# mj129/Tramba

Measured on AMD Instinct MI355X. Metric: images/sec fwd Tramba-V 384x384, higher is better.
Workload: dtype bf16; 1 GPU; Tramba-V (VMamba-B encoder) 384x384 bf16 inference, batch 4 per GPU, random-init weights (seed 1026), randn images; global_batch=4, launch=hipGraph replay, decoder guide branches on a side stream

## Files before the change

### include/tramba_hip.h

```cpp
#ifndef TRAMBA_HIP_H
#define TRAMBA_HIP_H

#include <stddef.h>
#include <stdint.h>

#ifdef __cplusplus
extern "C" {
#endif

typedef enum { TRAMBA_F32 = 0, TRAMBA_F16 = 1, TRAMBA_BF16 = 2 } tramba_dtype;

typedef enum {
    TRAMBA_SCAN_RASTER = 0,
    TRAMBA_SCAN_LINE = 1,
    TRAMBA_SCAN_HELIX = 2,
    TRAMBA_SCAN_WINDOW = 3,
    TRAMBA_SCAN_DILATION = 4
} tramba_scan_family;

typedef enum { TRAMBA_ACT_NONE = 0, TRAMBA_ACT_SILU = 1, TRAMBA_ACT_GELU = 2,
               TRAMBA_ACT_SIGMOID_GATE = 3 ,
               TRAMBA_ACT_GELU_GRAD_MUL = 4
             } tramba_act;

// ... 82 lines not shown
#define TRAMBA_SCAN_BWD_A_LOG 1
#define TRAMBA_SCAN_BWD_BC_PARTIALS 2
int tramba_ss2d_bwd_prep_cl(const float *xdbl, const int32_t *table, const float *bpart, const float *cpart, void *ranks,
                            float *gseq, int batch, int l, int k, int r, int ctiles, int dtype, void *stream);
int tramba_ss2d_bwd_assemble_cl(const float *gseq, const int32_t *inv_ptr, const int32_t *inv_idx, void *out, int batch,
                                int l, int k, int r, int dtype, void *stream);
size_t tramba_ss2d_scan_n_bwd_workspace(int batch, int l, int d, int k, int n, int dtype);
int tramba_ss2d_scan_n_bwd_plan(int batch, int l, int d, int k, int n, int *tiles_per_segment, int *nseg);
int tramba_ss2d_scan_n_bwd_cl(const void *x, const float *xdbl, const int32_t *table, const float *dt_w,
                              const float *dt_bias, const float *A, const float *Ds, const void *gym, void *gu,
                              void *graw, float *bpart, float *cpart, float *gpar, void *workspace,
                              size_t workspace_bytes, int batch, int l, int d, int k, int r, int n, int dtype,
                              int gym_dtype, void *stream);
int tramba_ss2d_bwd_prep_n_cl(const float *xdbl, const int32_t *table, const float *bpart, const float *cpart, void *ranks,
                              float *gseq, int batch, int l, int k, int r, int n, int ctiles, int dtype, void *stream);
int tramba_ss2d_bwd_assemble_n_cl(const float *gseq, const int32_t *inv_ptr, const int32_t *inv_idx, void *out, int batch,
                                  int l, int k, int r, int n, int dtype, void *stream);
int tramba_ss2d_merge_norm_cl(const void *ys, const int32_t *inv_ptr, const int32_t *inv_idx,
                              const float *ln_w, const float *ln_b, void *y, int batch, int l, int d,
                              int k, float eps, int act, int ys_dtype, int dtype, void *stream);
int tramba_ss2d_merge_grad_cl(const void *ys, const int32_t *inv_ptr, const int32_t *inv_idx, const float *ln_w,
                              const float *ln_b, void *y, const void *addend, const void *zpre, int batch, int l, int d,
                              int k, float eps, int act, int ys_dtype, int dtype, void *stream);

int tramba_layernorm_cl(const void *x, const float *w, const float *b, void *y, int64_t rows, int c,
                        float eps, int act, int dtype, void *stream);
int64_t tramba_layernorm_bwd_parts(int64_t rows, int c, int dtype);
int tramba_layernorm_bwd_cl(const void *x, const void *dy, const float *w, void *dx, float *part, int64_t rows,
                            int c, float eps, int dtype, void *stream);
int tramba_layernorm_bwd_res_cl(const void *x, const void *dy, const float *w, void *dx, float *part, const void *gres,
                                const float *mask, int64_t rows_per_sample, void *dxm, int64_t rows, int c, float eps,
                                int dtype, void *stream);
int tramba_layernorm_bwd_any_cl(const void *x, const void *dy, const float *w, void *dx, float *part, const void *gres,
                                const float *mask, int64_t rows_per_sample, void *dxm, int64_t rows, int c, float eps, int P,
                                int H, int W, int dtype, void *stream);
int tramba_shuffle_norm_bwd_cl(const void *x, const void *dy, const float *w, void *dx, float *part, int batch, int h,
                               int wd, int c, int p, float eps, int dtype, void *stream);
int tramba_add_layernorm_cl(const void *x, const void *y, const float *mask, int64_t rows_per_sample, const float *w,
                            const float *b, void *xsum, void *n, void *n_act, int64_t rows, int c, float eps, int act,
                            int dtype, void *stream);
int tramba_shuffle_norm_cl(const void *x, const float *w, const float *b, void *y, int batch, int h,
                           int wd, int c, int p, float eps, int dtype, void *stream);
int tramba_shuffle_norm_head_cl(const void *x, const float *w, const float *b, const float *head_w, float head_b,
                                float *y, int batch, int h, int wd, int c, int p, float eps, int dtype,
                                void *stream);
int64_t tramba_shuffle_norm_head_bwd_parts(int batch, int h, int wd, int c, int p, int dtype);
int tramba_shuffle_norm_head_bwd_cl(const void *x, const float *g, const float *ln_w, const float *head_w, void *dx,
                                    float *part, int batch, int h, int wd, int c, int p, float eps, int dtype, void *stream);
int tramba_rowdot_cl(const void *x, const float *w, float bias, float *y, int64_t rows, int c, int dtype,
                     void *stream);
int64_t tramba_rowdot_bwd_parts(int64_t rows, int c, int dtype);
int tramba_rowdot_bwd_cl(const void *x, const float *gy, const float *w, void *gx, float *part, int64_t rows, int c,
                         int dtype, void *stream);
int tramba_dw_pack(const float *w, const float *bias, const float *w3, const float *b3, const float *w5,
                   const float *b5, float *wt, float *bt, int c, int ks, void *stream);
int tramba_dw_pack_multi(const float *const *w, const float *const *bias, const float *const *w3, const float *const *b3,
                         const float *const *w5, const float *const *b5, float *const *wt, float *const *bt, const int *c,
                         const int *ks, int count, void *stream);
int tramba_im2col3x3_cl(const void *x, void *cols, int batch, int h, int wd, int c, int stride, int pad, int ckp,
                        int dtype, void *stream);
int tramba_col2im3x3_cl(const void *gcols, void *gx, int batch, int h, int wd, int c, int stride, int pad, int ckp,
                        int dtype, void *stream);
int tramba_upsample_bilinear_bwd(const float *gout, float *gin, int planes, int h, int w, int hout, int wout,
                                 void *stream);
int tramba_dwconv_cl(const void *x, const float *wt, const float *bt, void *y, int batch, int h,
                     int wd, int c, int ks, int act, int dtype, void *stream);
int tramba_dwconv_dual_cl(const void *x, const float *wt, const float *bt, void *y_pre, void *y, int batch, int h, int wd,
                          int c, int ks, int act, int flip_taps, int dtype, void *stream);
int tramba_dw_unpack_grad(const float *gwt, float *g7, float *g5, float *g3, float *gb, int nb, int c, int ks,
                          void *stream);
int tramba_dw_unpack_grad_multi(const float *const *gwt, float *const *g7, float *const *g5, float *const *g3,
                                float *const *gb, const int *nb, const int *c, const int *ks, int count, void *stream);
int64_t tramba_dwconv_wgrad_parts(int batch, int h, int wd, int c, int ks);
int tramba_dwconv_wgrad_cl(const void *x, const void *gy, float *part, int batch, int h, int wd, int c, int ks,
                           int dtype, void *stream);
int tramba_dct_split_cl(const void *x, const float *wx, const float *wy, float *tmp, void *high,
                        void *low, int batch, int n, int c, int dtype, void *stream);
int tramba_linear_cl(const void *x, const void *w, const float *bias, const void *residual, void *y,
                     int64_t m, int n, int k, int act, int dtype, int out_dtype, void *stream);
int tramba_linear_ln_cl(const void *x, const void *w_folded, const float *colsum, const float *bias, const void *residual,
                        void *y, int64_t m, int n, int k, float eps, int act, int dtype, int out_dtype, void *stream);
int tramba_linear2_cl(const void *x1, const void *x2, int k1, const void *w, const float *bias, const void *residual,
                      void *y, int64_t m, int n, int k, int act, int dtype, int out_dtype, void *stream);

int tramba_linear_dual_cl(const void *x, const void *w, const float *bias, void *y_pre, void *y_act, int64_t m, int n,
                          int k, int act, int dtype, void *stream);
size_t tramba_wgrad_workspace(int64_t m, int n, int k, int groups, int nbatch);
int tramba_wgrad_cl(const void *gy, const void *x, float *out, void *workspace, size_t workspace_bytes, int64_t m, int n,
                    int k, int groups, int nbatch, int64_t gy_bs, int64_t gy_gs, int gy_ld, int64_t x_bs, int64_t x_gs,
                    int x_ld, int want_bias, int dtype, void *stream);
int tramba_wgrad_parts_cl(const void *gy, const void *x, float *out, void *workspace, size_t workspace_bytes, int64_t m,
                          int n, int k, int groups, int nbatch, int64_t gy_bs, int64_t gy_gs, int gy_ld, int64_t x_bs,
                          int64_t x_gs, int x_ld, int want_bias, int dtype, void *stream, int *nslab);
int tramba_rows_gemm_cl(const void *x, const void *w, float *y, int nz, int64_t m, int n, int k, int groups, int ldy,
                        int dtype, void *stream);
int tramba_shadow_cast_multi(const void *table, int ntensors, int64_t total_tiles, int dtype, void *stream);
int tramba_slab_sum(const float *part, float *out, int64_t n, int nslab, void *stream);
int tramba_multi_sum_strided(const float *const *parts, float *const *outs, const int64_t *n, const int64_t *stride,
                             const int *nslab, int count, void *stream);
int tramba_multi_sum(const float *const *parts, float *const *outs, const int64_t *n, const int *nslab, int count,
                     void *stream);

int tramba_expand_norm_head_cl(const void *x, const void *w, const float *ln_w, const float *ln_b,
                               const float *head_w, float head_b, float *y, int batch, int h, int wd, int cin, int p,
                               float eps, int dtype, void *stream);

int tramba_conv3x3s2_cl(const void *x, const void *w, const float *bias, void *y, int batch, int hin,
                        int win, int cin, int cout, int dtype, void *stream);
int tramba_stem_conv_ln_gelu(const void *img, const float *w, const float *bias, const float *ln_w,
                             const float *ln_b, void *y, int batch, int h, int wd, float eps,
                             int img_dtype, int dtype, void *stream);

#define TRAMBA_EVAL_NINT 520
#define TRAMBA_EVAL_NDBL 48
int tramba_saliency_stats(const float *pred, const unsigned char *gt, long long *ints, double *dbl, int batch, int h,
                          int w, void *stream);
#define TRAMBA_WFM_MAX_DIM 4096
int tramba_feature_transform(const unsigned char *gt, int *idx, int *dist2, int batch, int h, int w, void *stream);
size_t tramba_weighted_f_workspace(int batch, int h, int w);
int tramba_weighted_f_sums(const float *pred, const unsigned char *gt, const int *idx, const int *dist2, const double *gauss,
                           double *sums, void *workspace, size_t workspace_bytes, int batch, int h, int w, void *stream);

#define TRAMBA_FRAME_MAX_DIM 16384
#define TRAMBA_FRAME_MAX_OUT 2048
size_t tramba_resize_table_words(int in_h, int in_w, int out_h, int out_w);
int tramba_resize_table(int in_h, int in_w, int out_h, int out_w, const double *mean, const double *std, int *table,
                        size_t words);
int tramba_frames_to_input(const unsigned char *frames, const int *table, float *out, int batch, int h, int w, int out_h,
                           int out_w, int bgr, void *stream);
int tramba_logits_to_u8(const void *logits, unsigned char *out, int batch, int in_h, int in_w, int h, int w, int dtype,
                        void *stream);
#define TRAMBA_FRAMES_DESC_WORDS 16
#define TRAMBA_RAGGED_IN 1
#define TRAMBA_RAGGED_OUT 2
int tramba_frames_ragged_check(const int64_t *desc_host, int batch, int size, size_t packed_bytes, size_t out_capacity,
                               int parts);
int tramba_frames_to_input_ragged(const unsigned char *packed, const int64_t *desc_host, size_t packed_bytes, float *out,
                                  int batch, int size, int bgr, void *stream);
int tramba_logits_to_u8_ragged(const void *logits, const unsigned char *packed, const int64_t *desc_host, unsigned char *out,
                               size_t out_capacity, int batch, int size, int dtype, void *stream);

#define TRAMBA_AUG_DESC_WORDS 32
#define TRAMBA_AUG_CONTRAST 0
#define TRAMBA_AUG_BRIGHTNESS 1
#define TRAMBA_AUG_SHARPNESS 2
size_t tramba_augment_source_table_words(int h, int w, int size);
int tramba_augment_source_table(int h, int w, int size, int *table, size_t words);
size_t tramba_augment_size_table_words(int size);
int tramba_augment_size_table(int size, const double *mean, const double *std, int *table, size_t words);
int tramba_augment_scale_taps(int size, int r);
int tramba_augment_rotation(int size, int degrees, int *coef);
size_t tramba_augment_workspace(int batch, int size);
int tramba_augment_batch(const unsigned char *packed, const int64_t *desc_host, size_t packed_bytes, const int *size_table,
                         float *image, float *label, void *workspace, size_t workspace_bytes, int batch, int size,
                         void *stream);

int tramba_sod_loss_sums(const float *logits, const float *label, float *part, int planes, int h, int w, int hout, int wout,
                         int nblk, void *stream);
int tramba_sod_loss_finish(const float *const *parts, const int *nblk, const float *weights, float *const *coefs, int nout,
                           int planes, int64_t npix, float *loss, void *stream);
size_t tramba_sod_loss_grad_workspace(int planes, int h, int w, int hout, int wout);
int tramba_sod_loss_grad(const float *logits, const float *label, const float *coef, const float *gscale, float *glogits,
                         void *workspace, size_t workspace_bytes, int planes, int h, int w, int hout, int wout, void *stream);
int tramba_loss_weight_map(const float *label, float *weit, int planes, int h, int w, int k, void *stream);
int tramba_sod_wloss_sums(const float *logits, const float *label, const float *wmap, float *part, int planes, int h, int w,
                          int hout, int wout, int nblk, float eps, int weight_is_raw, void *stream);
// ... 80 lines not shown
```

### tramba_amd/csrc/linear.hip

```cpp
#include <stdlib.h>
#include <string.h>

#include <type_traits>

#include "common.h"

namespace tramba {

typedef __attribute__((ext_vector_type(8))) short frag8_t;
typedef __attribute__((ext_vector_type(8))) _Float16 frag8h_t;
typedef __attribute__((ext_vector_type(16))) float acc16_t;

template <typename T> struct Mfma;
template <> struct Mfma<__hip_bfloat16> {
    static constexpr int KSTEP = 16;
    using frag = frag8_t;
    static __device__ __forceinline__ acc16_t run(frag a, frag b, acc16_t c)
    {
        typedef __attribute__((ext_vector_type(8))) __bf16 bf8;
        return __builtin_amdgcn_mfma_f32_32x32x16_bf16(__builtin_bit_cast(bf8, a), __builtin_bit_cast(bf8, b), c, 0, 0, 0);
    }
};
template <> struct Mfma<__half> {
    static constexpr int KSTEP = 16;
// ... 31 lines not shown
    if (col >= N) return;
    const float bv = bias ? bias[col] : 0.f;
#pragma unroll
    for (int r = 0; r < 16; ++r) {
        const long row = m0 + (r & 3) + 8 * (r >> 2) + 4 * (lane >> 5);
        if (row < M) {
            float v = apply_act(acc[r] + bv, act);
            if (res) v = combine_residual(v, Cvt<T>::to_f(res[row * N + col]), act);
            y[row * N + col] = Cvt<TO>::from_f(v);
        }
    }
}

template <typename T, typename TO>
__global__ __launch_bounds__(256) void linear16_kernel(const T *__restrict__ x, const T *__restrict__ w,
                                                      const float *__restrict__ bias, const T *__restrict__ res,
                                                      TO *__restrict__ y, long M, int N, int K, int act, int vec)
{
    const int lane = threadIdx.x & 63, wave = threadIdx.x >> 6;
    const long m0 = (long)blockIdx.y * 128 + (wave >> 1) * 64;
    const int n0 = blockIdx.x * 128 + (wave & 1) * 64;
    if (m0 >= M || n0 >= N) return;
    acc16_t acc[2][2];
#pragma unroll
    for (int i = 0; i < 2; ++i)
#pragma unroll
        for (int j = 0; j < 2; ++j)
#pragma unroll
            for (int r = 0; r < 16; ++r) acc[i][j][r] = 0.f;
    const int r32 = lane & 31, kh = (lane >> 5) * 8;
    for (int k0 = 0; k0 < K; k0 += 16) {
        frag8_t a[2], b[2];
#pragma unroll
        for (int i = 0; i < 2; ++i) a[i] = load_frag16<T>(x, m0 + i * 32 + r32, M, k0 + kh, K, vec);
#pragma unroll
        for (int j = 0; j < 2; ++j) b[j] = load_frag16<T>(w, n0 + j * 32 + r32, N, k0 + kh, K, vec);
#pragma unroll
        for (int i = 0; i < 2; ++i)
#pragma unroll
            for (int j = 0; j < 2; ++j) acc[i][j] = Mfma<T>::run(a[i], b[j], acc[i][j]);
    }
#pragma unroll
    for (int i = 0; i < 2; ++i)
#pragma unroll
        for (int j = 0; j < 2; ++j)
            store_tile<T, TO>(acc[i][j], y, bias, res, m0 + i * 32, n0 + j * 32, M, N, act, lane);
}


constexpr int kBK = 64;

__device__ __forceinline__ int swz_chunk(int row, int chunk) { return chunk ^ ((row >> 1) & 7); }

struct ConvGeom {
    int hin, win, cin, hout, wout;
};

template <int BM, int BN>
struct WaveLayout {
    static constexpr int WM = BM / 2, WN = BN / 2, TM = WM / 32, TN = WN / 32;
    static_assert(WM % 32 == 0 && WN % 32 == 0, "wave tiles are whole 32x32 MFMA tiles");
};

template <int BM, int BN, typename ACC>
__device__ __forceinline__ void acc_to_lds(ACC &acc, float *ep)
{
    using WL = WaveLayout<BM, BN>;
    constexpr int TM = WL::TM, TN = WL::TN, WM = WL::WM, WN = WL::WN, LDE = BN + 4;
    const int lane = threadIdx.x & 63, wave = threadIdx.x >> 6;
    if (wave >= 4) return;
    const int wm = wave / 2, wn = wave % 2;
    const int r32 = lane & 31, hi = lane >> 5;
#pragma unroll
    for (int i = 0; i < TM; ++i)
#pragma unroll
        for (int j = 0; j < TN; ++j)
#pragma unroll
            for (int g = 0; g < 4; ++g) {
                float *dst = ep + (wm * WM + i * 32 + r32) * LDE + wn * WN + j * 32 + 8 * g + 4 * hi;
                *reinterpret_cast<float4 *>(dst) = make_float4(acc[i][j][4 * g], acc[i][j][4 * g + 1], acc[i][j][4 * g + 2], acc[i][j][4 * g + 3]);
            }
}

template <typename T, typename TO, int BM, int BN, int NT = 256, typename ACC>
__device__ __forceinline__ void tile_epilogue(ACC &acc, unsigned char *lds,
                                              const float *__restrict__ bias, const T *__restrict__ res,
                                              TO *__restrict__ y, long M, int N, int act, long m0, int n0,
                                              const float *__restrict__ colsum = nullptr,
                                              const float2 *__restrict__ rowstat = nullptr,
                                              TO *__restrict__ y_pre = nullptr)
{
    const int tid = threadIdx.x;
    constexpr int LDE = BN + 4;
    float *ep = reinterpret_cast<float *>(lds);
    acc_to_lds<BM, BN>(acc, ep);
    __syncthreads();
    constexpr int CPL = 8;
    constexpr int LPRW = BN / CPL;
    constexpr int RPI = NT / LPRW;
    const int cl = (tid % LPRW) * CPL, rl = tid / LPRW;
    const int gcol = n0 + cl;
#pragma unroll
    for (int it = 0; it < (BM + RPI - 1) / RPI; ++it) {
        const int row = it * RPI + rl;
        const long grow = m0 + row;
        if (grow >= M || gcol >= N) continue;
        float o[CPL];
        {
            const float4 v0 = *reinterpret_cast<const float4 *>(ep + row * LDE + cl);
            const float4 v1 = *reinterpret_cast<const float4 *>(ep + row * LDE + cl + 4);
            o[0] = v0.x; o[1] = v0.y; o[2] = v0.z; o[3] = v0.w; o[4] = v1.x; o[5] = v1.y; o[6] = v1.z; o[7] = v1.w;
        }
        if (gcol + CPL <= N && (N & 7) == 0) {
            if (colsum) {
                const float2 st = rowstat[row];
                float cs[CPL];
                load_pack<float, CPL>(colsum + gcol, cs);
#pragma unroll
                for (int q = 0; q < CPL; ++q) o[q] = st.y * fmaf(-st.x, cs[q], o[q]);
            }
            if (bias) {
                float bv[CPL];
                load_pack<float, CPL>(bias + gcol, bv);
#pragma unroll
                for (int q = 0; q < CPL; ++q) o[q] += bv[q];
            }
            if (y_pre) store_pack<TO, CPL>(y_pre + grow * N + gcol, o);
#pragma unroll
            for (int q = 0; q < CPL; ++q) o[q] = apply_act(o[q], act);
            if (res) {
                float rv[CPL];
                load_pack<T, CPL>(res + grow * N + gcol, rv);
#pragma unroll
                for (int q = 0; q < CPL; ++q) o[q] = combine_residual(o[q], rv[q], act);
            }
            store_pack<TO, CPL>(y + grow * N + gcol, o);
        } else {
#pragma unroll
            for (int q = 0; q < CPL; ++q) {
                if (gcol + q < N) {
                    if (colsum) o[q] = rowstat[row].y * fmaf(-rowstat[row].x, colsum[gcol + q], o[q]);
                    const float pre = o[q] + (bias ? bias[gcol + q] : 0.f);
                    if (y_pre) y_pre[grow * N + gcol + q] = Cvt<TO>::from_f(pre);
                    float t = apply_act(pre, act);
                    if (res) {
                        const float rv = Cvt<T>::to_f(res[grow * N + gcol + q]);
                        t = combine_residual(t, rv, act);
                    }
                    y[grow * N + gcol + q] = Cvt<TO>::from_f(t);
                }
            }
        }
    }
}

template <typename T, typename TO, int BM, int BN, int PF, bool CONV>
__global__ __launch_bounds__(256) void linear_tiled_kernel(const T *__restrict__ x, const T *__restrict__ w,
                                                          const float *__restrict__ bias,
                                                          const T *__restrict__ res, TO *__restrict__ y, long M,
                                                          int N, int K, int act, ConvGeom cg)
{
    constexpr int TM = BM / 64, TN = BN / 64;
    constexpr int A_CHUNKS = BM * (kBK / 8), B_CHUNKS = BN * (kBK / 8);
    constexpr int A_PER_T = A_CHUNKS / 256, B_PER_T = B_CHUNKS / 256;
    constexpr int TILE_BYTES = (BM + BN) * kBK * 2;
    constexpr int EPI_BYTES = BM * (BN + 4) * 4;
    constexpr int LDS_BYTES = 2 * TILE_BYTES > EPI_BYTES ? 2 * TILE_BYTES : EPI_BYTES;
    __shared__ __attribute__((aligned(16))) unsigned char lds[LDS_BYTES];

    const int tid = threadIdx.x, lane = tid & 63, wave = tid >> 6;
    const int wm = wave >> 1, wn = wave & 1;
    long m0;
    int n0;
    {
        const unsigned nblk = gridDim.x * gridDim.y, lin = blockIdx.y * gridDim.x + blockIdx.x;
        const unsigned q = nblk >> 3, r = nblk & 7, xcd = lin & 7, slot = lin >> 3;
        const unsigned t = xcd * q + (xcd < r ? xcd : r) + slot;
        m0 = (long)(t / gridDim.x) * BM;
        n0 = (int)(t % gridDim.x) * BN;
    }
    const int nk = (K + kBK - 1) / kBK;

    acc16_t acc[TM][TN];
#pragma unroll
    for (int i = 0; i < TM; ++i)
#pragma unroll
        for (int j = 0; j < TN; ++j)
#pragma unroll
            for (int r = 0; r < 16; ++r) acc[i][j][r] = 0.f;

    struct Stage { frag8_t a[A_PER_T], b[B_PER_T]; };
    const int kmax = ((K - 1) / 8) * 8;
    int cb[A_PER_T], chi[A_PER_T], cwi[A_PER_T];
    if (CONV) {
#pragma unroll
        for (int i = 0; i < A_PER_T; ++i) {
            const int row = (tid + i * 256) >> 3;
            const long gr = m0 + row < M ? m0 + row : M - 1;
            const int wo = (int)(gr % cg.wout);
            const long t = gr / cg.wout;
            chi[i] = 2 * (int)(t % cg.hout) - 1;
            cwi[i] = 2 * wo - 1;
            cb[i] = (int)(t / cg.hout);
        }
    }
    auto conv_src = [&](int kt, int i, bool &inside) -> long {
        const int k0 = kt * kBK;
        const int tap = k0 / cg.cin, ci = k0 - tap * cg.cin;
        const int hy = chi[i] + tap / 3, wx = cwi[i] + tap % 3;
        inside = hy >= 0 && hy < cg.hin && wx >= 0 && wx < cg.win;
        const int hc = hy < 0 ? 0 : (hy >= cg.hin ? cg.hin - 1 : hy), wc = wx < 0 ? 0 : (wx >= cg.win ? cg.win - 1 : wx);
        return (((long)cb[i] * cg.hin + hc) * cg.win + wc) * cg.cin + ci;
    };
    auto gload = [&](int kt, Stage &st) {
        const int ktc = kt < nk ? kt : nk - 1;
        const int k0 = ktc * kBK;
#pragma unroll
        for (int i = 0; i < A_PER_T; ++i) {
            const int q = tid + i * 256, row = q >> 3, c = q & 7;
            if (CONV) {
                bool inside;
                st.a[i] = *reinterpret_cast<const frag8_t *>(x + conv_src(ktc, i, inside) + c * 8);
            } else {
                const long gr = m0 + row < M ? m0 + row : M - 1;
                const int kc = k0 + c * 8 <= kmax ? k0 + c * 8 : kmax;
                st.a[i] = *reinterpret_cast<const frag8_t *>(x + gr * K + kc);
            }
        }
#pragma unroll
        for (int i = 0; i < B_PER_T; ++i) {
            const int q = tid + i * 256, row = q >> 3, c = q & 7;
            const int gn = n0 + row < N ? n0 + row : N - 1;
            const int kc = k0 + c * 8 <= kmax ? k0 + c * 8 : kmax;
            st.b[i] = *reinterpret_cast<const frag8_t *>(w + (long)gn * K + kc);
        }
    };
    auto lstore = [&](int kt, const Stage &st) {
        const int buf = kt & 1, k0 = kt * kBK;
        unsigned char *As = lds + buf * TILE_BYTES, *Bs = As + BM * kBK * 2;
        const frag8_t zero = {0, 0, 0, 0, 0, 0, 0, 0};
#pragma unroll
        for (int i = 0; i < A_PER_T; ++i) {
            const int q = tid + i * 256, row = q >> 3, c = q & 7;
            bool ok = m0 + row < M && k0 + c * 8 < K;
            if (CONV) {
                bool inside;
                conv_src(kt, i, inside);
                ok = ok && inside;
            }
            *reinterpret_cast<frag8_t *>(As + row * 128 + swz_chunk(row, c) * 16) = ok ? st.a[i] : zero;
        }
#pragma unroll
        for (int i = 0; i < B_PER_T; ++i) {
            const int q = tid + i * 256, row = q >> 3, c = q & 7;
            const bool ok = n0 + row < N && k0 + c * 8 < K;
            *reinterpret_cast<frag8_t *>(Bs + row * 128 + swz_chunk(row, c) * 16) = ok ? st.b[i] : zero;
        }
    };

    constexpr int NS = PF + 1;
    Stage pipe[NS];
    gload(0, pipe[0]);
    lstore(0, pipe[0]);
#pragma unroll
    for (int i = 1; i < NS; ++i) gload(i, pipe[i]);
    __syncthreads();
    const int r32 = lane & 31, hi = lane >> 5;
    auto kstep = [&](int kt, Stage &load_into, const Stage &store_from) {
        gload(kt + NS, load_into);
        const unsigned char *As = lds + (kt & 1) * TILE_BYTES, *Bs = As + BM * kBK * 2;
#pragma unroll
        for (int kk = 0; kk < kBK / 16; ++kk) {
            frag8_t a[TM], b[TN];
            const int c = kk * 2 + hi;
#pragma unroll
            for (int i = 0; i < TM; ++i) {
                const int row = wm * (BM / 2) + i * 32 + r32;
                a[i] = *reinterpret_cast<const frag8_t *>(As + row * 128 + swz_chunk(row, c) * 16);
            }
#pragma unroll
            for (int j = 0; j < TN; ++j) {
                const int row = wn * (BN / 2) + j * 32 + r32;
                b[j] = *reinterpret_cast<const frag8_t *>(Bs + row * 128 + swz_chunk(row, c) * 16);
            }
#pragma unroll
            for (int i = 0; i < TM; ++i)
#pragma unroll
                for (int j = 0; j < TN; ++j) acc[i][j] = Mfma<T>::run(b[j], a[i], acc[i][j]);
        }
        lstore(kt + 1, store_from);
        __syncthreads();
    };
    const int nkp = (nk + NS - 1) / NS * NS;
    constexpr int UNR = 4 * NS;
    int kt0 = 0;
    for (; kt0 + UNR <= nkp; kt0 += UNR) {
#pragma unroll
        for (int ui = 0; ui < UNR; ++ui) kstep(kt0 + ui, pipe[ui % NS], pipe[(ui + 1) % NS]);
    }
    for (; kt0 < nkp; kt0 += NS) {
#pragma unroll
        for (int ui = 0; ui < NS; ++ui) kstep(kt0 + ui, pipe[ui % NS], pipe[(ui + 1) % NS]);
    }

    tile_epilogue<T, TO, BM, BN>(acc, lds, bias, res, y, M, N, act, m0, n0);
}

struct LnIn {
    const float *colsum;
    float eps;
};

struct LnHead {
    const float *ln_w, *ln_b, *head_w;
    float head_b, eps;
    int H, W, P;
    float *out;
};

template <typename T, int BM>
__device__ __forceinline__ void tile_epilogue_ln_head(acc16_t (&acc)[BM / 64][2], unsigned char *lds, const LnHead hd,
                                                      long M, long m0, int n0)
{
    constexpr int BN = 128, TM = BM / 64, TN = 2, WM = BM / 2, WN = BN / 2;
    const int tid = threadIdx.x, lane = tid & 63, wave = tid >> 6;
    const int wm = wave >> 1, wn = wave & 1;
    const int r32 = lane & 31, hi = lane >> 5;
    constexpr int LDE = BN + 4;
    float *ep = reinterpret_cast<float *>(lds);
    acc_to_lds<BM, BN>(acc, ep);
    __syncthreads();
    const int sub = tid & 3;
    float gam[32], bet[32], hw[32];
#pragma unroll
    for (int j = 0; j < 8; ++j) {
        const int c = 16 * j + 4 * sub;
        const float4 a = *reinterpret_cast<const float4 *>(hd.ln_w + c);
        const float4 b = *reinterpret_cast<const float4 *>(hd.ln_b + c);
        const float4 h = *reinterpret_cast<const float4 *>(hd.head_w + c);
        gam[4 * j] = a.x; gam[4 * j + 1] = a.y; gam[4 * j + 2] = a.z; gam[4 * j + 3] = a.w;
        bet[4 * j] = b.x; bet[4 * j + 1] = b.y; bet[4 * j + 2] = b.z; bet[4 * j + 3] = b.w;
        hw[4 * j] = h.x; hw[4 * j + 1] = h.y; hw[4 * j + 2] = h.z; hw[4 * j + 3] = h.w;
    }
    const int g = n0 / BN;
#pragma unroll
    for (int it = 0; it < BM / 64; ++it) {
        const int row = it * 64 + (tid >> 2);
        const long grow = m0 + row;
        float v[32];
#pragma unroll
        for (int j = 0; j < 8; ++j) {
            const float4 t = *reinterpret_cast<const float4 *>(ep + row * LDE + 16 * j + 4 * sub);
            v[4 * j] = t.x; v[4 * j + 1] = t.y; v[4 * j + 2] = t.z; v[4 * j + 3] = t.w;
        }
        float s1 = 0.f;
#pragma unroll
        for (int q = 0; q < 32; ++q) s1 += v[q];
        s1 += __shfl_xor(s1, 1, 64);
        s1 += __shfl_xor(s1, 2, 64);
        const float mean = s1 * (1.f / 128.f);
        float s2 = 0.f;
#pragma unroll
        for (int q = 0; q < 32; ++q) {
            const float d = v[q] - mean;
            s2 = fmaf(d, d, s2);
        }
        s2 += __shfl_xor(s2, 1, 64);
        s2 += __shfl_xor(s2, 2, 64);
        const float rstd = rsqrtf(s2 * (1.f / 128.f) + hd.eps);
        float dot = 0.f;
#pragma unroll
        for (int q = 0; q < 32; ++q) {
            const float yn = (v[q] - mean) * rstd * gam[q] + bet[q];
            dot = fmaf(yn, hw[q], dot);
        }
        dot += __shfl_xor(dot, 1, 64);
        dot += __shfl_xor(dot, 2, 64);
        if (sub == 0 && grow < M) {
            const unsigned pix = (unsigned)grow;
            const unsigned wi = pix % (unsigned)hd.W, bh = pix / (unsigned)hd.W;
            const unsigned hh = bh % (unsigned)hd.H, bb = bh / (unsigned)hd.H;
            const long o = ((long)bb * (hd.H * hd.P) + (hh * hd.P + g / hd.P)) * (long)(hd.W * hd.P) + (wi * hd.P + g % hd.P);
            hd.out[o] = dot + hd.head_b;
        }
    }
}

typedef unsigned v4u_t __attribute__((ext_vector_type(4)));

template <typename T> __device__ __forceinline__ float dot2_ones(unsigned v, float acc);
template <typename T> __device__ __forceinline__ float dot2_self(unsigned v, float acc);
typedef __bf16 bf2_t __attribute__((ext_vector_type(2)));
typedef _Float16 hf2_t __attribute__((ext_vector_type(2)));
template <> __device__ __forceinline__ float dot2_ones<__hip_bfloat16>(unsigned v, float acc)
{
    return __builtin_amdgcn_fdot2_f32_bf16(__builtin_bit_cast(bf2_t, v), __builtin_bit_cast(bf2_t, 0x3f803f80u), acc, false);
}
template <> __device__ __forceinline__ float dot2_self<__hip_bfloat16>(unsigned v, float acc)
{
    return __builtin_amdgcn_fdot2_f32_bf16(__builtin_bit_cast(bf2_t, v), __builtin_bit_cast(bf2_t, v), acc, false);
}
template <> __device__ __forceinline__ float dot2_ones<__half>(unsigned v, float acc)
{
    return __builtin_amdgcn_fdot2(__builtin_bit_cast(hf2_t, v), __builtin_bit_cast(hf2_t, 0x3c003c00u), acc, false);
}
template <> __device__ __forceinline__ float dot2_self<__half>(unsigned v, float acc)
{
    return __builtin_amdgcn_fdot2(__builtin_bit_cast(hf2_t, v), __builtin_bit_cast(hf2_t, v), acc, false);
}
template <> __device__ __forceinline__ float dot2_ones<float>(unsigned, float acc) { return acc; }
template <> __device__ __forceinline__ float dot2_self<float>(unsigned, float acc) { return acc; }

template <typename T, typename TO, int BM, int BN, int PF, bool LNHEAD = false>
__global__ __launch_bounds__(256) void linear_lean_kernel(const T *__restrict__ x, const T *__restrict__ w,
                                                         const float *__restrict__ bias,
                                                         const T *__restrict__ res, TO *__restrict__ y, long M,
                                                         int N, int K, int act, const T *__restrict__ x2, int K1,
                                                         LnHead hd = LnHead{})
{
    using WL = WaveLayout<BM, BN>;
    constexpr int TM = WL::TM, TN = WL::TN;
    constexpr int A_PER_T = BM * (kBK / 8) / 256, B_PER_T = BN * (kBK / 8) / 256;
    constexpr int TILE_BYTES = (BM + BN) * kBK * 2;
    constexpr int EPI_BYTES = BM * (BN + 4) * 4;
    static_assert((BM * (kBK / 8)) % 256 == 0 && (BN * (kBK / 8)) % 256 == 0, "whole 16-byte chunks per thread");
    constexpr int LDS_BYTES = 2 * TILE_BYTES > EPI_BYTES ? 2 * TILE_BYTES : EPI_BYTES;
    constexpr int NS = PF + 1;
    static_assert(NS % 2 == 0, "the LDS buffer parity must be a compile-time constant");
    __shared__ __attribute__((aligned(16))) unsigned char lds[LDS_BYTES];

    const int tid = threadIdx.x, lane = tid & 63, wave = tid >> 6;
    const int wm = wave < 4 ? wave / 2 : 0, wn = wave % 2;
    const int r32 = lane & 31, hi = lane >> 5;
    long m0;
    int n0;
    {
        const unsigned nblk = gridDim.x * gridDim.y, lin = blockIdx.y * gridDim.x + blockIdx.x;
        const unsigned q = nblk >> 3, r = nblk & 7, xcd = lin & 7, slot = lin >> 3;
        const unsigned t = xcd * q + (xcd < r ? xcd : r) + slot;
        m0 = (long)(t / gridDim.x) * BM;
        n0 = (int)(t % gridDim.x) * BN;
    }
    const int nk = K / kBK;
    const unsigned rowb = (unsigned)K * 2u;
    const long mrows = M - m0 < BM ? M - m0 : BM;
    const int nrows = N - n0 < BN ? N - n0 : BN;
    const int ka = x2 ? K1 : K;
    const unsigned rowa = (unsigned)ka * 2u, rowa2 = (unsigned)(K - ka) * 2u;
    const int nk1 = ka / kBK;
    const __amdgpu_buffer_rsrc_t ra = make_rsrc(x + m0 * ka, (unsigned)mrows * rowa);
    const __amdgpu_buffer_rsrc_t ra2 = make_rsrc(x2 ? x2 + m0 * (K - ka) : x, x2 ? (unsigned)mrows * rowa2 : 0u);
    const __amdgpu_buffer_rsrc_t rb = make_rsrc(w + (long)n0 * K, (unsigned)nrows * rowb);

    unsigned ag[A_PER_T], ag2[A_PER_T], bg[B_PER_T], al[A_PER_T], bl[B_PER_T];
#pragma unroll
    for (int i = 0; i < A_PER_T; ++i) {
        const int q = tid + i * 256, row = q >> 3, c = q & 7;
        ag[i] = (unsigned)row * rowa + (unsigned)c * 16u;
        ag2[i] = (unsigned)row * rowa2 + (unsigned)c * 16u;
        al[i] = (unsigned)(row * 128 + swz_chunk(row, c) * 16);
    }
#pragma unroll
    for (int i = 0; i < B_PER_T; ++i) {
        const int q = tid + i * 256, row = q >> 3, c = q & 7;
        bg[i] = (unsigned)row * rowb + (unsigned)c * 16u;
        bl[i] = (unsigned)(BM * kBK * 2 + row * 128 + swz_chunk(row, c) * 16);
    }
    unsigned ard[TM], brd[TN];
#pragma unroll
    for (int i = 0; i < TM; ++i) {
        const int row = wm * WL::WM + i * 32 + r32;
        ard[i] = (unsigned)(row * 128 + swz_chunk(row, hi) * 16);
    }
#pragma unroll
    for (int j = 0; j < TN; ++j) {
        const int row = wn * WL::WN + j * 32 + r32;
        brd[j] = (unsigned)(BM * kBK * 2 + row * 128 + swz_chunk(row, hi) * 16);
    }

    acc16_t acc[TM][TN];
#pragma unroll
    for (int i = 0; i < TM; ++i)
#pragma unroll
        for (int j = 0; j < TN; ++j)
#pragma unroll
            for (int r = 0; r < 16; ++r) acc[i][j][r] = 0.f;

    struct Stage { v4u_t a[A_PER_T], b[B_PER_T]; };
    auto gload = [&](int kt, Stage &st) {
        const unsigned so = (unsigned)kt * (kBK * 2);
        const bool first = kt < nk1;
        const __amdgpu_buffer_rsrc_t rsel = first ? ra : ra2;
        const unsigned soa = first ? so : so - (unsigned)nk1 * (kBK * 2);
#pragma unroll
        for (int i = 0; i < A_PER_T; ++i)
            st.a[i] = __builtin_amdgcn_raw_buffer_load_b128(rsel, first ? ag[i] : ag2[i], soa, 0);
#pragma unroll
        for (int i = 0; i < B_PER_T; ++i) st.b[i] = __builtin_amdgcn_raw_buffer_load_b128(rb, bg[i], so, 0);
    };
    auto lstore = [&](int par, const Stage &st) {
        unsigned char *base = lds + par * TILE_BYTES;
#pragma unroll
        for (int i = 0; i < A_PER_T; ++i) *reinterpret_cast<v4u_t *>(base + al[i]) = st.a[i];
#pragma unroll
        for (int i = 0; i < B_PER_T; ++i) *reinterpret_cast<v4u_t *>(base + bl[i]) = st.b[i];
    };

    Stage pipe[NS];
    gload(0, pipe[0]);
    lstore(0, pipe[0]);
#pragma unroll
    for (int i = 1; i < NS; ++i) gload(i, pipe[i]);
    __syncthreads();
    auto kstep = [&](int kt, int par, Stage &load_into, const Stage &store_from) {
        gload(kt + NS, load_into);
        const unsigned char *base = lds + par * TILE_BYTES;
#pragma unroll
        for (int kk = 0; kk < kBK / 16; ++kk) {
            frag8_t a[TM], b[TN];
#pragma unroll
            for (int i = 0; i < TM; ++i) a[i] = *reinterpret_cast<const frag8_t *>(base + (ard[i] ^ (unsigned)(kk * 32)));
#pragma unroll
            for (int j = 0; j < TN; ++j) b[j] = *reinterpret_cast<const frag8_t *>(base + (brd[j] ^ (unsigned)(kk * 32)));
#pragma unroll
            for (int i = 0; i < TM; ++i)
#pragma unroll
                for (int j = 0; j < TN; ++j) acc[i][j] = Mfma<T>::run(b[j], a[i], acc[i][j]);
        }
        lstore(par ^ 1, store_from);
        __syncthreads();
    };
    constexpr int UNR = 4 * NS;
    int kt0 = 0;
    for (; kt0 + UNR <= nk; kt0 += UNR) {
#pragma unroll
        for (int ui = 0; ui < UNR; ++ui) kstep(kt0 + ui, ui & 1, pipe[ui % NS], pipe[(ui + 1) % NS]);
    }
    for (; kt0 + NS <= nk; kt0 += NS) {
#pragma unroll
        for (int ui = 0; ui < NS; ++ui) kstep(kt0 + ui, ui & 1, pipe[ui % NS], pipe[(ui + 1) % NS]);
    }
#pragma unroll
    for (int ui = 0; ui < NS - 1; ++ui)
        if (kt0 + ui < nk) kstep(kt0 + ui, ui & 1, pipe[ui % NS], pipe[(ui + 1) % NS]);

    if constexpr (LNHEAD) {
        static_assert(BN == 128, "one tile = whole 128-channel groups");
        tile_epilogue_ln_head<T, BM>(acc, lds, hd, M, m0, n0);
    } else {
        tile_epilogue<T, TO, BM, BN>(acc, lds, bias, res, y, M, N, act, m0, n0);
    }
}

#define TRAMBA_DSR128_(OUT, ADDR, OFF) asm volatile("ds_read_b128 %0, %1 offset:" #OFF : "=v"(OUT) : "v"(ADDR) : "memory")

template <typename T, typename TO, int NSTG, bool LNIN = false, bool DUAL = false>
__global__ __launch_bounds__(256) void linear_dma_kernel(const T *__restrict__ x, const T *__restrict__ w,
                                                        const float *__restrict__ bias, const T *__restrict__ res,
                                                        TO *__restrict__ y, long M, int N, int K, int act,
                                                        LnIn li = LnIn{nullptr, 0.f}, TO *__restrict__ y_pre = nullptr)
{
#if defined(__HIP_DEVICE_COMPILE__)
    constexpr int BM = 64, BN = 64;
    constexpr int TILE_BYTES = (BM + BN) * kBK * 2;
    constexpr int EPI_BYTES = BM * (BN + 4) * 4;
    constexpr int LDS_BYTES = NSTG * TILE_BYTES > EPI_BYTES ? NSTG * TILE_BYTES : EPI_BYTES;
    static_assert(NSTG == 2 || NSTG == 3 || NSTG == 4, "stage index = kt % NSTG with the loop unrolled by NSTG (up to 8 stages are coded)");
    __shared__ __attribute__((aligned(1024))) unsigned char lds[LDS_BYTES + (LNIN ? BM * 8 : 0)];
    typedef __attribute__((address_space(3))) void lds_void;

    const int tid = threadIdx.x, lane = tid & 63;
    const int wave = __builtin_amdgcn_readfirstlane(tid >> 6);
    const int wm = wave >> 1, wn = wave & 1;
    const int r32 = lane & 31, hi = lane >> 5;
    long m0;
    int n0;
    {
        const unsigned nblk = gridDim.x * gridDim.y, lin = blockIdx.y * gridDim.x + blockIdx.x;
        const unsigned q = nblk >> 3, r = nblk & 7, xcd = lin & 7, slot = lin >> 3;
        const unsigned t = xcd * q + (xcd < r ? xcd : r) + slot;
        m0 = (long)(t / gridDim.x) * BM;
        n0 = (int)(t % gridDim.x) * BN;
    }
    const int nk = K / kBK;
    const unsigned rowb = (unsigned)K * 2u;
    const long mrows = M - m0 < BM ? M - m0 : BM;
    const int nrows = N - n0 < BN ? N - n0 : BN;
    const bool stage_b = wave >= 2;
    const __amdgpu_buffer_rsrc_t rs = stage_b ? make_rsrc(w + (long)n0 * K, (unsigned)nrows * rowb)
                                              : make_rsrc(x + m0 * K, (unsigned)mrows * rowb);
    unsigned voff[4];
#pragma unroll
    for (int j = 0; j < 4; ++j) {
        const int row = ((wave & 1) * 4 + j) * 8 + (lane >> 3);
        const int c = (lane & 7) ^ ((row >> 1) & 7);
        voff[j] = (unsigned)row * rowb + (unsigned)c * 16u;
    }
    unsigned char *mine = lds + (stage_b ? BM * kBK * 2 : 0) + (wave & 1) * 4096;
    auto issue = [&](int kt, int stg) {
        const unsigned so = (unsigned)kt * (kBK * 2);
#pragma unroll
        for (int j = 0; j < 4; ++j)
            __builtin_amdgcn_raw_ptr_buffer_load_lds(rs, (lds_void *)(mine + stg * TILE_BYTES + j * 1024), 16, voff[j], so, 0,
                                                     0);
    };
    const unsigned lbase = (unsigned)(size_t)(__attribute__((address_space(3))) unsigned char *)lds;
    unsigned aad[4], bad[4];
    {
        const int ra_ = wm * 32 + r32, rb_ = wn * 32 + r32;
        const unsigned a0 = lbase + (unsigned)(ra_ * 128 + ((hi ^ ((ra_ >> 1) & 7)) * 16));
        const unsigned b0 = lbase + (unsigned)(BM * kBK * 2 + rb_ * 128 + ((hi ^ ((rb_ >> 1) & 7)) * 16));
#pragma unroll
        for (int kk = 0; kk < 4; ++kk) {
            aad[kk] = a0 ^ (unsigned)(kk * 32);
            bad[kk] = b0 ^ (unsigned)(kk * 32);
        }
    }
    acc16_t acc[1][1];
#pragma unroll
    for (int r = 0; r < 16; ++r) acc[0][0][r] = 0.f;
    float rs1[2] = {0.f, 0.f}, rs2[2] = {0.f, 0.f};
    const unsigned sad = lbase + (unsigned)((tid >> 3) * 128 + (tid & 7) * 16);

    constexpr int DEPTH = NSTG - 1;
#pragma unroll
    for (int t = 0; t < DEPTH; ++t)
        if (t < nk) issue(t, t);
    unsigned aad_hi[4], bad_hi[4];
#pragma unroll
    for (int kk = 0; kk < 4; ++kk) {
        aad_hi[kk] = aad[kk] + 65536u;
        bad_hi[kk] = bad[kk] + 65536u;
    }
    const unsigned sad_hi = sad + 65536u;
    auto kstep = [&](int kt, auto stg_c) {
        constexpr int STG = decltype(stg_c)::value;
        const int later = nk - 1 - kt;
        if (later >= DEPTH - 1) {
            if constexpr (DEPTH == 1) asm volatile("s_waitcnt vmcnt(0)" ::: "memory");
            else if constexpr (DEPTH == 2) asm volatile("s_waitcnt vmcnt(4)" ::: "memory");
            else if constexpr (DEPTH == 3) asm volatile("s_waitcnt vmcnt(8)" ::: "memory");
            else asm volatile("s_waitcnt vmcnt(24)" ::: "memory");
        } else {
            switch (later) {
            case 0: asm volatile("s_waitcnt vmcnt(0)" ::: "memory"); break;
            case 1: asm volatile("s_waitcnt vmcnt(4)" ::: "memory"); break;
            case 2: asm volatile("s_waitcnt vmcnt(8)" ::: "memory"); break;
            case 3: asm volatile("s_waitcnt vmcnt(12)" ::: "memory"); break;
            case 4: asm volatile("s_waitcnt vmcnt(16)" ::: "memory"); break;
            default: asm volatile("s_waitcnt vmcnt(20)" ::: "memory"); break;
            }
        }
        __builtin_amdgcn_s_barrier();
        asm volatile("" ::: "memory");
        if (kt + DEPTH < nk) issue(kt + DEPTH, (STG + DEPTH) % NSTG);
        frag8_t a[4], b[4];
        v4u_t sv[2];
        const unsigned *aa = STG < 4 ? aad : aad_hi, *ba = STG < 4 ? bad : bad_hi;
        const unsigned sa = STG < 4 ? sad : sad_hi;
#define TRAMBA_RD_STG_(S, S2)                                                                       \
    if constexpr (LNIN) { TRAMBA_DSR128_(sv[0], sa, S); TRAMBA_DSR128_(sv[1], sa, S2); }             \
    TRAMBA_DSR128_(a[0], aa[0], S); TRAMBA_DSR128_(b[0], ba[0], S); TRAMBA_DSR128_(a[1], aa[1], S);  \
    TRAMBA_DSR128_(b[1], ba[1], S); TRAMBA_DSR128_(a[2], aa[2], S); TRAMBA_DSR128_(b[2], ba[2], S);  \
    TRAMBA_DSR128_(a[3], aa[3], S); TRAMBA_DSR128_(b[3], ba[3], S)
        if constexpr ((STG & 3) == 0) { TRAMBA_RD_STG_(0, 4096); }
        else if constexpr ((STG & 3) == 1) { TRAMBA_RD_STG_(16384, 20480); }
        else if constexpr ((STG & 3) == 2) { TRAMBA_RD_STG_(32768, 36864); }
        else { TRAMBA_RD_STG_(49152, 53248); }
#undef TRAMBA_RD_STG_
        if constexpr (LNIN) {
            asm volatile("s_waitcnt lgkmcnt(8)" : "+v"(sv[0]), "+v"(sv[1]) : : "memory");
#pragma unroll
            for (int i = 0; i < 2; ++i)
#pragma unroll
                for (int e = 0; e < 4; ++e) {
                    rs1[i] = dot2_ones<T>(sv[i][e], rs1[i]);
                    rs2[i] = dot2_self<T>(sv[i][e], rs2[i]);
                }
        }
        asm volatile("s_waitcnt lgkmcnt(6)" : "+v"(a[0]), "+v"(b[0]) : : "memory");
        acc[0][0] = Mfma<T>::run(b[0], a[0], acc[0][0]);
        asm volatile("s_waitcnt lgkmcnt(4)" : "+v"(a[1]), "+v"(b[1]) : : "memory");
        acc[0][0] = Mfma<T>::run(b[1], a[1], acc[0][0]);
        asm volatile("s_waitcnt lgkmcnt(2)" : "+v"(a[2]), "+v"(b[2]) : : "memory");
        acc[0][0] = Mfma<T>::run(b[2], a[2], acc[0][0]);
        asm volatile("s_waitcnt lgkmcnt(0)" : "+v"(a[3]), "+v"(b[3]) : : "memory");
        acc[0][0] = Mfma<T>::run(b[3], a[3], acc[0][0]);
    };
    int kt0 = 0;
    for (; kt0 + NSTG <= nk; kt0 += NSTG) {
        kstep(kt0, std::integral_constant<int, 0>{});
        kstep(kt0 + 1, std::integral_constant<int, 1>{});
        if constexpr (NSTG > 2) kstep(kt0 + 2, std::integral_constant<int, 2>{});
        if constexpr (NSTG > 3) kstep(kt0 + 3, std::integral_constant<int, 3>{});
        if constexpr (NSTG > 4) {
            kstep(kt0 + 4, std::integral_constant<int, 4>{});
            kstep(kt0 + 5, std::integral_constant<int, 5>{});
            kstep(kt0 + 6, std::integral_constant<int, 6>{});
            kstep(kt0 + 7, std::integral_constant<int, 7>{});
        }
    }
    if (kt0 < nk) kstep(kt0, std::integral_constant<int, 0>{});
    if constexpr (NSTG > 2) {
        if (kt0 + 1 < nk) kstep(kt0 + 1, std::integral_constant<int, 1>{});
    }
    if constexpr (NSTG > 3) {
        if (kt0 + 2 < nk) kstep(kt0 + 2, std::integral_constant<int, 2>{});
    }
    if constexpr (NSTG > 4) {
        if (kt0 + 3 < nk) kstep(kt0 + 3, std::integral_constant<int, 3>{});
        if (kt0 + 4 < nk) kstep(kt0 + 4, std::integral_constant<int, 4>{});
        if (kt0 + 5 < nk) kstep(kt0 + 5, std::integral_constant<int, 5>{});
        if (kt0 + 6 < nk) kstep(kt0 + 6, std::integral_constant<int, 6>{});
    }
    __syncthreads();
    if constexpr (LNIN) {
        float2 *rowstat = reinterpret_cast<float2 *>(lds + LDS_BYTES);
#pragma unroll
        for (int i = 0; i < 2; ++i) {
            float s1 = rs1[i], s2 = rs2[i];
#pragma unroll
            for (int m = 1; m < 8; m <<= 1) {
                s1 += __shfl_xor(s1, m, 64);
                s2 += __shfl_xor(s2, m, 64);
            }
            const float mean = s1 / (float)K;
            const float var = fmaxf(s2 / (float)K - mean * mean, 0.f);
            if ((tid & 7) == 0) rowstat[(tid >> 3) + 32 * i] = make_float2(mean, rsqrtf(var + li.eps));
        }
        tile_epilogue<T, TO, BM, BN>(acc, lds, bias, res, y, M, N, act, m0, n0, li.colsum,
                                     reinterpret_cast<const float2 *>(lds + LDS_BYTES));
    } else {
        tile_epilogue<T, TO, BM, BN>(acc, lds, bias, res, y, M, N, act, m0, n0, nullptr, nullptr, DUAL ? y_pre : nullptr);
    }
#endif
}

enum { A_PLAIN = 0, A_TWO = 1, A_CONV = 2 };
struct ASrc {
    const void *x2;
    int k1;
    ConvGeom cg;
    unsigned abytes;
};

#define TRAMBA_DSR128_(OUT, ADDR, OFF) asm volatile("ds_read_b128 %0, %1 offset:" #OFF : "=v"(OUT) : "v"(ADDR) : "memory")
template <typename T, typename TO, int NSTG, bool LNIN = false, bool DUAL = false, int ASRC = A_PLAIN>
__global__ __launch_bounds__(512, ASRC == A_CONV && NSTG == 3 ? 6 : 1) void linear_pc_kernel(const T *__restrict__ x, const T *__restrict__ w,
                                                       const float *__restrict__ bias, const T *__restrict__ res,
                                                       TO *__restrict__ y, long M, int N, int K, int act,
                                                       LnIn li = LnIn{nullptr, 0.f}, TO *__restrict__ y_pre = nullptr,
                                                       ASrc as = ASrc{nullptr, 0, ConvGeom{0, 0, 0, 0, 0}, 0u})
{
#if defined(__HIP_DEVICE_COMPILE__)
    constexpr int BM = 64, BN = 64;
    constexpr int TILE_BYTES = (BM + BN) * kBK * 2;
    constexpr int EPI_BYTES = BM * (BN + 4) * 4;
    constexpr int LDS_BYTES = NSTG * TILE_BYTES > EPI_BYTES ? NSTG * TILE_BYTES : EPI_BYTES;
    static_assert(NSTG == 3 || NSTG == 4, "stage index = kt % NSTG with the loop unrolled by NSTG");
    __shared__ __attribute__((aligned(1024))) unsigned char lds[LDS_BYTES + (LNIN ? BM * 8 : 0)];
    typedef __attribute__((address_space(3))) void lds_void;

    const int tid = threadIdx.x, lane = tid & 63;
    const int wave = __builtin_amdgcn_readfirstlane(tid >> 6);
    const bool loader = wave >= 4;
    const int cw = wave & 3;
    const int wm = cw >> 1, wn = cw & 1;
    const int r32 = lane & 31, hi = lane >> 5;
    long m0;
    int n0;
    {
        const unsigned nblk = gridDim.x * gridDim.y, lin = blockIdx.y * gridDim.x + blockIdx.x;
        const unsigned q = nblk >> 3, r = nblk & 7, xcd = lin & 7, slot = lin >> 3;
        const unsigned t = xcd * q + (xcd < r ? xcd : r) + slot;
        m0 = (long)(t / gridDim.x) * BM;
        n0 = (int)(t % gridDim.x) * BN;
    }
    const int nk = K / kBK;
    const unsigned rowb = (unsigned)K * 2u;
    const long mrows = M - m0 < BM ? M - m0 : BM;
    const int nrows = N - n0 < BN ? N - n0 : BN;
    const bool stage_b = cw >= 2;
    __amdgpu_buffer_rsrc_t rs, rsx;
    unsigned voff[4];
    unsigned lx[4] = {0u, 0u, 0u, 0u}, ly[4] = {0u, 0u, 0u, 0u};
    unsigned(&voff2)[4] = lx;
    unsigned(&chy)[4] = lx, (&cwx)[4] = ly;
    int nsw = nk;
    unsigned hlim = 0xffffffffu, wlim = 0xffffffffu;
    int ccs = 0, cdy = 0, cdx = 0;
    if constexpr (ASRC == A_TWO) {
        const int ka = as.k1;
        const unsigned rowa = (unsigned)ka * 2u, rowa2 = (unsigned)(K - ka) * 2u;
        rs = stage_b ? make_rsrc(w + (long)n0 * K, (unsigned)nrows * rowb) : make_rsrc(x + m0 * ka, (unsigned)mrows * rowa);
        rsx = stage_b ? rs : make_rsrc((const T *)as.x2 + m0 * (K - ka), (unsigned)mrows * rowa2);
        if (!stage_b) nsw = ka / kBK;
#pragma unroll
        for (int j = 0; j < 4; ++j) {
            const int row = ((cw & 1) * 4 + j) * 8 + (lane >> 3);
            const int c = (lane & 7) ^ ((row >> 1) & 7);
            voff[j] = (unsigned)row * (stage_b ? rowb : rowa) + (unsigned)c * 16u;
            voff2[j] = (unsigned)row * (stage_b ? rowb : rowa2) + (unsigned)c * 16u;
        }
    } else if constexpr (ASRC == A_CONV) {
        rs = stage_b ? make_rsrc(w + (long)n0 * K, (unsigned)nrows * rowb) : make_rsrc(x, as.abytes);
        if (!stage_b) {
            hlim = (unsigned)as.cg.hin;
            wlim = (unsigned)as.cg.win;
        }
#pragma unroll
        for (int j = 0; j < 4; ++j) {
            const int row = ((cw & 1) * 4 + j) * 8 + (lane >> 3);
            const int c = (lane & 7) ^ ((row >> 1) & 7);
            if (stage_b) {
                voff[j] = (unsigned)row * rowb + (unsigned)c * 16u;
                chy[j] = cwx[j] = 0u;
            } else {
                const long gr = m0 + row;
                const bool ok = gr < M;
                const unsigned pix = ok ? (unsigned)gr : 0u;
                const unsigned wo = pix % (unsigned)as.cg.wout, t = pix / (unsigned)as.cg.wout;
                const unsigned ho = t % (unsigned)as.cg.hout, b = t / (unsigned)as.cg.hout;
                chy[j] = (unsigned)(ok ? 2 * (int)ho - 1 : -4);
                cwx[j] = (unsigned)(2 * (int)wo - 1);
                voff[j] = ((b * (unsigned)as.cg.hin + chy[j]) * (unsigned)as.cg.win + cwx[j]) * ((unsigned)as.cg.cin * 2u) +
                          (unsigned)c * 16u;
            }
        }
    } else {
        rs = stage_b ? make_rsrc(w + (long)n0 * K, (unsigned)nrows * rowb) : make_rsrc(x + m0 * K, (unsigned)mrows * rowb);
#pragma unroll
        for (int j = 0; j < 4; ++j) {
            const int row = ((cw & 1) * 4 + j) * 8 + (lane >> 3);
            const int c = (lane & 7) ^ ((row >> 1) & 7);
            voff[j] = (unsigned)row * rowb + (unsigned)c * 16u;
        }
    }
    unsigned char *mine = lds + (stage_b ? BM * kBK * 2 : 0) + (cw & 1) * 4096;
    auto issue = [&](int kt, int stg) {
        if constexpr (ASRC == A_TWO) {
            const bool first = kt < nsw;
            const __amdgpu_buffer_rsrc_t rsel = first ? rs : rsx;
            const unsigned so = (unsigned)(first ? kt : kt - nsw) * (kBK * 2);
#pragma unroll
            for (int j = 0; j < 4; ++j)
                __builtin_amdgcn_raw_ptr_buffer_load_lds(rsel, (lds_void *)(mine + stg * TILE_BYTES + j * 1024), 16,
                                                         first ? voff[j] : voff2[j], so, 0, 0);
        } else if constexpr (ASRC == A_CONV) {
            const unsigned so = stage_b ? (unsigned)kt * (kBK * 2)
                                        : (unsigned)((cdy * as.cg.win + cdx) * as.cg.cin + ccs * kBK) * 2u;
#pragma unroll
            for (int j = 0; j < 4; ++j) {
                const unsigned hy = chy[j] + (unsigned)cdy, wx = cwx[j] + (unsigned)cdx;
                unsigned out = (hy < hlim && wx < wlim) ? 0u : 1u;
                asm volatile("" : "+v"(out));
                __builtin_amdgcn_raw_ptr_buffer_load_lds(rs, (lds_void *)(mine + stg * TILE_BYTES + j * 1024), 16,
                                                         (voff[j] + so) | (out << 31), 0, 0, 0);
            }
            if (++ccs == as.cg.cin / kBK) {
                ccs = 0;
                if (++cdx == 3) { cdx = 0; ++cdy; }
            }
        } else {
            const unsigned so = (unsigned)kt * (kBK * 2);
#pragma unroll
            for (int j = 0; j < 4; ++j)
                __builtin_amdgcn_raw_ptr_buffer_load_lds(rs, (lds_void *)(mine + stg * TILE_BYTES + j * 1024), 16, voff[j], so,
                                                         0, 0);
        }
    };
    const unsigned lbase = (unsigned)(size_t)(__attribute__((address_space(3))) unsigned char *)lds;
    unsigned(&aad)[4] = lx, (&bad)[4] = ly;
    if (ASRC == A_PLAIN || !loader) {
        const int ra_ = wm * 32 + r32, rb_ = wn * 32 + r32;
        const unsigned a0 = lbase + (unsigned)(ra_ * 128 + ((hi ^ ((ra_ >> 1) & 7)) * 16));
        const unsigned b0 = lbase + (unsigned)(BM * kBK * 2 + rb_ * 128 + ((hi ^ ((rb_ >> 1) & 7)) * 16));
#pragma unroll
        for (int kk = 0; kk < 4; ++kk) {
            aad[kk] = a0 ^ (unsigned)(kk * 32);
            bad[kk] = b0 ^ (unsigned)(kk * 32);
        }
    }
    acc16_t acc[1][1];
#pragma unroll
    for (int r = 0; r < 16; ++r) acc[0][0][r] = 0.f;
    const int lt = tid & 255;
    float rs1[2] = {0.f, 0.f}, rs2[2] = {0.f, 0.f};
    const unsigned sad = lbase + (unsigned)((lt >> 3) * 128 + (lt & 7) * 16);

    constexpr int DEPTH = NSTG - 1;
    if (loader) {
#pragma unroll
        for (int t = 0; t < DEPTH; ++t)
            if (t < nk) issue(t, t);
    }
    auto kstep = [&](int kt, auto stg_c) {
        constexpr int STG = decltype(stg_c)::value;
        if (loader) {
            const int later = nk - 1 - kt;
            if (later >= DEPTH - 1) {
                if constexpr (DEPTH == 2) asm volatile("s_waitcnt vmcnt(4)" ::: "memory");
                else asm volatile("s_waitcnt vmcnt(8)" ::: "memory");
            } else {
                switch (later) {
                case 0: asm volatile("s_waitcnt vmcnt(0)" ::: "memory"); break;
                default: asm volatile("s_waitcnt vmcnt(4)" ::: "memory"); break;
                }
            }
        }
        __builtin_amdgcn_s_barrier();
        asm volatile("" ::: "memory");
        if (loader) {
            if (kt + DEPTH < nk) issue(kt + DEPTH, (STG + DEPTH) % NSTG);
        } else {
            frag8_t a[4], b[4];
            v4u_t sv[2];
            if constexpr (LNIN) {
                if constexpr (STG == 0) { TRAMBA_DSR128_(sv[0], sad, 0); TRAMBA_DSR128_(sv[1], sad, 4096); }
                else if constexpr (STG == 1) { TRAMBA_DSR128_(sv[0], sad, 16384); TRAMBA_DSR128_(sv[1], sad, 20480); }
                else if constexpr (STG == 2) { TRAMBA_DSR128_(sv[0], sad, 32768); TRAMBA_DSR128_(sv[1], sad, 36864); }
                else { TRAMBA_DSR128_(sv[0], sad, 49152); TRAMBA_DSR128_(sv[1], sad, 53248); }
            }
#define TRAMBA_RD_STG_(S)                                                                            \
    TRAMBA_DSR128_(a[0], aad[0], S); TRAMBA_DSR128_(b[0], bad[0], S); TRAMBA_DSR128_(a[1], aad[1], S); \
    TRAMBA_DSR128_(b[1], bad[1], S); TRAMBA_DSR128_(a[2], aad[2], S); TRAMBA_DSR128_(b[2], bad[2], S); \
    TRAMBA_DSR128_(a[3], aad[3], S); TRAMBA_DSR128_(b[3], bad[3], S)
            if constexpr (STG == 0) { TRAMBA_RD_STG_(0); }
            else if constexpr (STG == 1) { TRAMBA_RD_STG_(16384); }
            else if constexpr (STG == 2) { TRAMBA_RD_STG_(32768); }
            else { TRAMBA_RD_STG_(49152); }
#undef TRAMBA_RD_STG_
            if constexpr (LNIN) {
                asm volatile("s_waitcnt lgkmcnt(8)" : "+v"(sv[0]), "+v"(sv[1]) : : "memory");
#pragma unroll
                for (int i = 0; i < 2; ++i)
#pragma unroll
                    for (int e = 0; e < 4; ++e) {
                        rs1[i] = dot2_ones<T>(sv[i][e], rs1[i]);
                        rs2[i] = dot2_self<T>(sv[i][e], rs2[i]);
                    }
            }
            asm volatile("s_waitcnt lgkmcnt(6)" : "+v"(a[0]), "+v"(b[0]) : : "memory");
            acc[0][0] = Mfma<T>::run(b[0], a[0], acc[0][0]);
            __builtin_amdgcn_sched_barrier(0);
            asm volatile("s_waitcnt lgkmcnt(4)" : "+v"(a[1]), "+v"(b[1]) : : "memory");
            acc[0][0] = Mfma<T>::run(b[1], a[1], acc[0][0]);
            __builtin_amdgcn_sched_barrier(0);
            asm volatile("s_waitcnt lgkmcnt(2)" : "+v"(a[2]), "+v"(b[2]) : : "memory");
            acc[0][0] = Mfma<T>::run(b[2], a[2], acc[0][0]);
            __builtin_amdgcn_sched_barrier(0);
            asm volatile("s_waitcnt lgkmcnt(0)" : "+v"(a[3]), "+v"(b[3]) : : "memory");
            acc[0][0] = Mfma<T>::run(b[3], a[3], acc[0][0]);
        }
    };
    int kt0 = 0;
    for (; kt0 + NSTG <= nk; kt0 += NSTG) {
        kstep(kt0, std::integral_constant<int, 0>{});
        kstep(kt0 + 1, std::integral_constant<int, 1>{});
        kstep(kt0 + 2, std::integral_constant<int, 2>{});
        if constexpr (NSTG > 3) kstep(kt0 + 3, std::integral_constant<int, 3>{});
    }
    if (kt0 < nk) kstep(kt0, std::integral_constant<int, 0>{});
    if (kt0 + 1 < nk) kstep(kt0 + 1, std::integral_constant<int, 1>{});
    if constexpr (NSTG > 3) {
        if (kt0 + 2 < nk) kstep(kt0 + 2, std::integral_constant<int, 2>{});
    }
    __syncthreads();
    if constexpr (LNIN) {
        float2 *rowstat = reinterpret_cast<float2 *>(lds + LDS_BYTES);
        if (!loader) {
#pragma unroll
            for (int i = 0; i < 2; ++i) {
                float s1 = rs1[i], s2 = rs2[i];
#pragma unroll
                for (int m = 1; m < 8; m <<= 1) {
                    s1 += __shfl_xor(s1, m, 64);
                    s2 += __shfl_xor(s2, m, 64);
                }
                const float mean = s1 / (float)K;
                const float var = fmaxf(s2 / (float)K - mean * mean, 0.f);
                if ((lt & 7) == 0) rowstat[(lt >> 3) + 32 * i] = make_float2(mean, rsqrtf(var + li.eps));
            }
        }
        tile_epilogue<T, TO, BM, BN, 512>(acc, lds, bias, res, y, M, N, act, m0, n0, li.colsum,
                                          reinterpret_cast<const float2 *>(lds + LDS_BYTES));
    } else {
        tile_epilogue<T, TO, BM, BN, 512>(acc, lds, bias, res, y, M, N, act, m0, n0, nullptr, nullptr, DUAL ? y_pre : nullptr);
    }
#endif
}
#undef TRAMBA_DSR128_

template <typename T> __device__ __forceinline__ unsigned pack2_(float a, float b);
template <> __device__ __forceinline__ unsigned pack2_<__hip_bfloat16>(float a, float b)
{
    unsigned pk = 0u;
#if defined(__HIP_DEVICE_COMPILE__)
    asm("v_cvt_pk_bf16_f32 %0, %1, %2" : "=v"(pk) : "v"(a), "v"(b));
#endif
    return pk;
}
template <> __device__ __forceinline__ unsigned pack2_<__half>(float a, float b)
{
    unsigned pk = 0u;
#if defined(__HIP_DEVICE_COMPILE__)
    asm("v_cvt_pk_f16_f32 %0, %1, %2" : "=v"(pk) : "v"(a), "v"(b));
#endif
    return pk;
}
template <typename T> __device__ __forceinline__ float unpack_lo_(unsigned v);
template <typename T> __device__ __forceinline__ float unpack_hi_(unsigned v);
template <> __device__ __forceinline__ float unpack_lo_<__hip_bfloat16>(unsigned v) { return __builtin_bit_cast(float, v << 16); }
template <> __device__ __forceinline__ float unpack_hi_<__hip_bfloat16>(unsigned v) { return __builtin_bit_cast(float, v & 0xffff0000u); }
template <> __device__ __forceinline__ float unpack_lo_<__half>(unsigned v) { return (float)__builtin_bit_cast(_Float16, (unsigned short)(v & 0xffffu)); }
template <> __device__ __forceinline__ float unpack_hi_<__half>(unsigned v) { return (float)__builtin_bit_cast(_Float16, (unsigned short)(v >> 16)); }

typedef unsigned v2u_t __attribute__((ext_vector_type(2)));

#define TRAMBA_DSR128I_(OUT, ADDR, OFF) asm volatile("ds_read_b128 %0, %1 offset:%2" : "=v"(OUT) : "v"(ADDR), "i"(OFF) : "memory")
#define TRAMBA_VMCNT_(N) asm volatile("s_waitcnt vmcnt(%0)" ::"n"(N) : "memory")

template <typename T, int K, int NCW, bool LNIN, bool DUAL, bool RES>
__global__ __launch_bounds__(256, 2) void linear_ws_kernel(const T *__restrict__ x, const T *__restrict__ w,
                                                          const float *__restrict__ bias, const T *__restrict__ res,
                                                          T *__restrict__ y, long M, int N, int act, LnIn li,
                                                          T *__restrict__ y_pre, int npanel, int gt)
{
#if defined(__HIP_DEVICE_COMPILE__)
    static_assert(K == 128 || K == 256, "row = one or two 256-byte bank rows");
    static_assert(NCW * K <= 512, "the wave's B fragments stay in <= 128 registers");
    static_assert((((K == 128 && NCW <= 2) ? 6 : 4) - 1) * 32 * K * 2 + 512 <= 65535, "the last ring stage inside ds_read's 16-bit offset");
    static_assert((((K == 128 && NCW <= 2) ? 6 : 4) - 1) * (NCW * 2 * (DUAL ? 2 : 1)) +
                          (((K == 128 && NCW <= 2) ? 6 : 4) - 2) * ((RES ? NCW * 4 : 0) + K / 64) <= 63,
                  "the counted vmcnt fits its 6-bit field");
    static_assert(!(DUAL && RES), "a dual-output launch has no residual");
    static_assert(!RES || NCW <= 2, "residual rows are prefetched into registers");
    constexpr int KB = K / 16;
    constexpr int RB = K * 2;
    constexpr int TILE_BYTES = 32 * RB;
    constexpr int NSTG = (K == 128 && NCW <= 2) ? 6 : 4;
    constexpr int PPW = K / 64;
    constexpr int PANEL = 128 * NCW;
    constexpr int S = NCW * 2 * (DUAL ? 2 : 1);
    constexpr int RL = RES ? NCW * 4 : 0;
    __shared__ __attribute__((aligned(1024))) unsigned char lds[NSTG * TILE_BYTES + PANEL * 8];
    typedef __attribute__((address_space(3))) void lds_void;
    float *lbias = reinterpret_cast<float *>(lds + NSTG * TILE_BYTES);
    float *lcs = lbias + PANEL;

    const int tid = threadIdx.x, lane = tid & 63;
    const int wv = __builtin_amdgcn_readfirstlane(tid >> 6);
    const int r32 = lane & 31, hi = lane >> 5;
    const int pn = blockIdx.x % npanel, g0 = blockIdx.x / npanel;
    const int n0 = pn * PANEL, n0w = n0 + wv * (NCW * 32);
    const long T32 = (M + 31) / 32;
    const int nt = g0 < T32 ? (int)((T32 - g0 + gt - 1) / gt) : 0;

    frag8_t bf[NCW][KB];
#pragma unroll
    for (int cb = 0; cb < NCW; ++cb)
#pragma unroll
        for (int kb = 0; kb < KB; ++kb)
            bf[cb][kb] = *reinterpret_cast<const frag8_t *>(w + (long)(n0w + cb * 32 + r32) * K + kb * 16 + hi * 8);
    for (int i = tid; i < PANEL; i += 256) {
        lbias[i] = bias ? bias[n0 + i] : 0.f;
        lcs[i] = LNIN ? li.colsum[n0 + i] : 0.f;
    }
    __syncthreads();

    const __amdgpu_buffer_rsrc_t rsx = make_rsrc(x, (unsigned)(M * RB));
// ... 133 lines not shown
                v4f_t cf4 = {0.f, 0.f, 0.f, 0.f};
                if constexpr (LNIN) cf4 = __builtin_bit_cast(v4f_t, cq[g]);
#pragma unroll
                for (int q = 0; q < 4; ++q) {
                    float v = acc[cb][4 * g + q];
                    if constexpr (LNIN) v = rstd * fmaf(-mean, cf4[q], v);
                    o[4 * g + q] = v + bf4[q];
                }
            }
            if constexpr (DUAL) {
#pragma unroll
                for (int g = 0; g < 4; ++g) {
                    pp[g][0] = pack2_<T>(o[4 * g], o[4 * g + 1]);
                    pp[g][1] = pack2_<T>(o[4 * g + 2], o[4 * g + 3]);
                }
            }
            if (act == TRAMBA_ACT_GELU) {
#pragma unroll
                for (int e = 0; e < 16; ++e) o[e] = geluf_(o[e]);
            } else if (act == TRAMBA_ACT_SILU) {
#pragma unroll
                for (int e = 0; e < 16; ++e) o[e] = siluf_(o[e]);
            }
#pragma unroll
            for (int g = 0; g < 4; ++g) {
                if constexpr (RES) {
                    const v2u_t r2 = rv[cb * 4 + g];
                    o[4 * g + 0] += unpack_lo_<T>(r2[0]);
                    o[4 * g + 1] += unpack_hi_<T>(r2[0]);
                    o[4 * g + 2] += unpack_lo_<T>(r2[1]);
                    o[4 * g + 3] += unpack_hi_<T>(r2[1]);
                }
                pk[g][0] = pack2_<T>(o[4 * g], o[4 * g + 1]);
                pk[g][1] = pack2_<T>(o[4 * g + 2], o[4 * g + 3]);
            }
#pragma unroll
            for (int pr = 0; pr < 2; ++pr) {
                const auto w0 = __builtin_amdgcn_permlane32_swap(pk[2 * pr][0], pk[2 * pr + 1][0], false, false);
                const auto w1 = __builtin_amdgcn_permlane32_swap(pk[2 * pr][1], pk[2 * pr + 1][1], false, false);
                const unsigned a0 = w0[0], b0 = w0[1], a1 = w1[0], b1 = w1[1];
                const v4u_t out = {a0, a1, b0, b1};
                __builtin_amdgcn_raw_buffer_store_b128(out, rsy, yoff + (unsigned)((cb * 32 + pr * 16) * 2), so_y, 0);
                if constexpr (DUAL) {
                    const auto u0 = __builtin_amdgcn_permlane32_swap(pp[2 * pr][0], pp[2 * pr + 1][0], false, false);
                    const auto u1 = __builtin_amdgcn_permlane32_swap(pp[2 * pr][1], pp[2 * pr + 1][1], false, false);
                    const unsigned c0 = u0[0], d0 = u0[1], c1 = u1[0], d1 = u1[1];
                    const v4u_t outp = {c0, c1, d0, d1};
                    __builtin_amdgcn_raw_buffer_store_b128(outp, rsp, yoff + (unsigned)((cb * 32 + pr * 16) * 2), so_y, 0);
                }
            }
        }
    };
    for (int t0 = 0; t0 < nt; t0 += NSTG) {
        tile_step(t0, std::integral_constant<int, 0>{});
        if (t0 + 1 < nt) tile_step(t0 + 1, std::integral_constant<int, 1>{});
        if (t0 + 2 < nt) tile_step(t0 + 2, std::integral_constant<int, 2>{});
        if (t0 + 3 < nt) tile_step(t0 + 3, std::integral_constant<int, 3>{});
        if constexpr (NSTG > 4) {
            if (t0 + 4 < nt) tile_step(t0 + 4, std::integral_constant<int, 4>{});
            if (t0 + 5 < nt) tile_step(t0 + 5, std::integral_constant<int, 5>{});
        }
    }
    asm volatile("s_waitcnt vmcnt(0)" ::: "memory");
#endif
}
#undef TRAMBA_DSR128I_
#undef TRAMBA_VMCNT_

static bool ws_rule(long m, int n, int k, int kind )
{
    if (k != 128 || n < 256) return false;
    return kind == 1 ? m >= 16384 : m >= 65536;
}

static int pc_rule(long tiles64, int k, int kind)
{
    if (kind == 1) return tiles64 <= 320 ? 3 : 0;
    if (kind == 2) return (k <= 256 && tiles64 >= 4096) ? 0 : 3;
    if (k >= 2048 && tiles64 <= 256) return 4;
    if (k >= 2048 && tiles64 <= 320) return 0;
    return 3;
}

static int ws_ncw(long m, int n, int k)
{
    if (k != 128 && k != 256) return 0;
    if ((double)m * n * 2.0 >= 2147483648.0 || (double)(m + 32) * k * 2.0 >= 2147483648.0) return 0;
    int ncw = 256 / k;
    while (ncw >= 1 && n % (128 * ncw)) ncw >>= 1;
    return ncw;
}

template <typename T, int K, bool LNIN, bool DUAL, bool RES>
static void launch_ws(int ncw, const void *x, const void *w, const float *bias, const void *res, void *y, long m, int n, int act,
                      LnIn li, void *y_pre, hipStream_t s)
{
    const int npanel = n / (128 * ncw);
    const long t32 = (m + 31) / 32;
    const long resident = 256L * (K == 128 ? 3 : 2);
    long gt = resident / npanel;
    if (gt > t32) gt = t32;
    if (gt < 1) gt = 1;
    dim3 grid((unsigned)(gt * npanel)), block(256);
#define WS_(NCW_)                                                                                                      \
    hipLaunchKernelGGL((linear_ws_kernel<T, K, NCW_, LNIN, DUAL, RES>), grid, block, 0, s, (const T *)x, (const T *)w, bias, \
                       (const T *)res, (T *)y, m, n, act, li, (T *)y_pre, npanel, (int)gt)
    if constexpr (K == 128) {
        if (ncw == 2) { WS_(2); } else { WS_(1); }
    } else {
        WS_(1);
    }
#undef WS_
}

template <typename T, bool LNIN, bool DUAL>
static void launch_ws_k(int ncw, const void *x, const void *w, const float *bias, const void *res, void *y, long m, int n, int k,
                        int act, LnIn li, void *y_pre, hipStream_t s)
{
    if (k == 128) {
        if (res) { if constexpr (!DUAL) launch_ws<T, 128, LNIN, false, true>(ncw, x, w, bias, res, y, m, n, act, li, y_pre, s); }
        else launch_ws<T, 128, LNIN, DUAL, false>(ncw, x, w, bias, res, y, m, n, act, li, y_pre, s);
    } else {
        if (res) { if constexpr (!DUAL) launch_ws<T, 256, LNIN, false, true>(ncw, x, w, bias, res, y, m, n, act, li, y_pre, s); }
        else launch_ws<T, 256, LNIN, DUAL, false>(ncw, x, w, bias, res, y, m, n, act, li, y_pre, s);
    }
}

constexpr int DMA_SHORT_K = 256;

enum GemmKind { GEMM_PLAIN = 0, GEMM_LN = 1, GEMM_DUAL = 2, GEMM_TWO_SRC, GEMM_CONV };
enum class GemmForm {
    WS,
    PC3, PC4,
    DMA2, DMA3, DMA4,
    LEAN,
    TILED128, TILED64, TILED64_PF3
};
struct GemmPlan {
    GemmForm form;
    int ncw;
};

static GemmPlan gemm_plan(GemmKind kind, long m, int n, int k, int act, bool same_dtype, bool a_dma = true)
{
    int tune = tramba_tune_get(TRAMBA_TUNE_GEMM_TILE);
    if ((kind == GEMM_TWO_SRC || kind == GEMM_CONV) && a_dma && tune != 18 && k % 64 == 0 &&
        (double)k * 2.0 * 128.0 < 2147483648.0) {
        const long tiles64 = ((m + 63) / 64) * ((n + 63) / 64);
        return {pc_rule(tiles64, k, GEMM_PLAIN) == 4 ? GemmForm::PC4 : GemmForm::PC3, 0};
    }
    if (kind == GEMM_TWO_SRC) return {GemmForm::LEAN, 0};
    if (kind == GEMM_CONV || k % 64 != 0 || (double)k * 2.0 * 128.0 >= 2147483648.0) {
        const long big = ((m + 127) / 128) * ((n + 127) / 128);
        if (big >= 2048 && k >= 1024) return {GemmForm::TILED128, 0};
        return {k <= 128 ? GemmForm::TILED64 : GemmForm::TILED64_PF3, 0};
    }
    if (tune == 7 && kind != GEMM_PLAIN) tune = 0;
    if (tune == 0 || tune == 19) {
        const bool ws_act = act == TRAMBA_ACT_NONE || act == TRAMBA_ACT_GELU || act == TRAMBA_ACT_SILU;
        const int ncw = same_dtype && ws_act ? ws_ncw(m, n, k) : 0;
        if (ncw && (tune == 19 ? m >= 64 : ws_rule(m, n, k, kind))) return {GemmForm::WS, ncw};
    }
    switch (tune) {
    case 7: return {GemmForm::DMA4, 0};
    case 13: return {GemmForm::DMA2, 0};
    case 14: return {GemmForm::DMA3, 0};
    case 16: return {GemmForm::PC3, 0};
    case 17: return {GemmForm::PC4, 0};
    }
    const long tiles64 = ((m + 63) / 64) * ((n + 63) / 64);
    const int pc = tune == 18 ? 0 : pc_rule(tiles64, k, kind);
    if (pc) return {pc == 4 ? GemmForm::PC4 : GemmForm::PC3, 0};
    if (k <= DMA_SHORT_K && tiles64 >= 1024) return {GemmForm::DMA2, 0};
    if (kind == GEMM_PLAIN && tiles64 <= 256 && k >= 1024) return {GemmForm::DMA4, 0};
    return {GemmForm::DMA3, 0};
}

struct GemmArgs {
    const void *x, *w;
    const float *bias;
    const void *res;
    void *y;
    long m;
    int n, k, act;
    LnIn li{nullptr, 0.f};
    void *y_pre = nullptr;
    const void *x2 = nullptr;
    int k1 = 0;
    ConvGeom cg{0, 0, 0, 0, 0};
    unsigned abytes = 0;
};

template <typename T, typename TO, bool LNIN = false, bool DUAL = false, bool CONV = false>
static void launch_gemm(const GemmPlan &p, const GemmArgs &a, hipStream_t s)
{
    const T *x = (const T *)a.x, *w = (const T *)a.w, *res = (const T *)a.res;
    TO *y = (TO *)a.y, *y_pre = (TO *)a.y_pre;
    const long m = a.m;
    const int n = a.n, k = a.k, act = a.act;
    const dim3 g64((n + 63) / 64, (unsigned)((m + 63) / 64)), g128((n + 127) / 128, (unsigned)((m + 127) / 128));
    switch (p.form) {
    case GemmForm::WS:
        launch_ws_k<T, LNIN, DUAL>(p.ncw, a.x, a.w, a.bias, a.res, a.y, m, n, k, act, a.li, a.y_pre, s);
        break;
    case GemmForm::PC3:
    case GemmForm::PC4: {
        const bool four = p.form == GemmForm::PC4;
        if constexpr (CONV) {
            const ASrc as{nullptr, 0, a.cg, a.abytes};
            if (four) hipLaunchKernelGGL((linear_pc_kernel<T, TO, 4, false, false, A_CONV>), g64, dim3(512), 0, s, x, w, a.bias, res, y, m, n, k, act, a.li, y_pre, as);
            else hipLaunchKernelGGL((linear_pc_kernel<T, TO, 3, false, false, A_CONV>), g64, dim3(512), 0, s, x, w, a.bias, res, y, m, n, k, act, a.li, y_pre, as);
            break;
        }
        if constexpr (!LNIN && !DUAL) {
            if (a.x2) {
                const ASrc as{a.x2, a.k1, a.cg, 0u};
                if (four) hipLaunchKernelGGL((linear_pc_kernel<T, TO, 4, false, false, A_TWO>), g64, dim3(512), 0, s, x, w, a.bias, res, y, m, n, k, act, a.li, y_pre, as);
                else hipLaunchKernelGGL((linear_pc_kernel<T, TO, 3, false, false, A_TWO>), g64, dim3(512), 0, s, x, w, a.bias, res, y, m, n, k, act, a.li, y_pre, as);
                break;
            }
        }
        if (four) hipLaunchKernelGGL((linear_pc_kernel<T, TO, 4, LNIN, DUAL>), g64, dim3(512), 0, s, x, w, a.bias, res, y, m, n, k, act, a.li, y_pre);
        else hipLaunchKernelGGL((linear_pc_kernel<T, TO, 3, LNIN, DUAL>), g64, dim3(512), 0, s, x, w, a.bias, res, y, m, n, k, act, a.li, y_pre);
        break;
    }
    case GemmForm::DMA2:
        hipLaunchKernelGGL((linear_dma_kernel<T, TO, 2, LNIN, DUAL>), g64, dim3(256), 0, s, x, w, a.bias, res, y, m, n, k, act, a.li, y_pre);
        break;
    case GemmForm::DMA3:
        hipLaunchKernelGGL((linear_dma_kernel<T, TO, 3, LNIN, DUAL>), g64, dim3(256), 0, s, x, w, a.bias, res, y, m, n, k, act, a.li, y_pre);
        break;
    case GemmForm::DMA4:
        if constexpr (!LNIN && !DUAL)
            hipLaunchKernelGGL((linear_dma_kernel<T, TO, 4>), g64, dim3(256), 0, s, x, w, a.bias, res, y, m, n, k, act, a.li, y_pre);
        break;
    case GemmForm::LEAN:
        hipLaunchKernelGGL((linear_lean_kernel<T, TO, 64, 64, 1>), g64, dim3(256), 0, s, x, w, a.bias, res, y, m, n, k, act,
                           (const T *)a.x2, a.k1);
        break;
    case GemmForm::TILED128:
        hipLaunchKernelGGL((linear_tiled_kernel<T, TO, 128, 128, 2, CONV>), g128, dim3(256), 0, s, x, w, a.bias, res, y, m, n, k, act, a.cg);
        break;
    case GemmForm::TILED64:
        hipLaunchKernelGGL((linear_tiled_kernel<T, TO, 64, 64, 1, CONV>), g64, dim3(256), 0, s, x, w, a.bias, res, y, m, n, k, act, a.cg);
        break;
    case GemmForm::TILED64_PF3:
        hipLaunchKernelGGL((linear_tiled_kernel<T, TO, 64, 64, 3, CONV>), g64, dim3(256), 0, s, x, w, a.bias, res, y, m, n, k, act, a.cg);
        break;
    }
}

template <bool LNIN = false>
static void launch_gemm16(const GemmPlan &p, const GemmArgs &a, int dtype, int out_dtype, hipStream_t s)
{
    if (dtype == TRAMBA_BF16) {
        if (out_dtype == TRAMBA_F32) launch_gemm<__hip_bfloat16, float, LNIN>(p, a, s);
        else launch_gemm<__hip_bfloat16, __hip_bfloat16, LNIN>(p, a, s);
    } else {
        if (out_dtype == TRAMBA_F32) launch_gemm<__half, float, LNIN>(p, a, s);
        else launch_gemm<__half, __half, LNIN>(p, a, s);
    }
}

template <typename TO>
__global__ __launch_bounds__(256) void linear32_kernel(const float *__restrict__ x, const float *__restrict__ w,
                                                      const float *__restrict__ bias, const float *__restrict__ res,
                                                      TO *__restrict__ y, long M, int N, int K, int act)
{
    const int lane = threadIdx.x & 63, wave = threadIdx.x >> 6;
    const long m0 = (long)blockIdx.y * 128 + (wave >> 1) * 64;
    const int n0 = blockIdx.x * 128 + (wave & 1) * 64;
    if (m0 >= M || n0 >= N) return;
    acc16_t acc[2][2];
#pragma unroll
    for (int i = 0; i < 2; ++i)
#pragma unroll
        for (int j = 0; j < 2; ++j)
#pragma unroll
            for (int r = 0; r < 16; ++r) acc[i][j][r] = 0.f;
    const int r32 = lane & 31, kh = lane >> 5;
    for (int k0 = 0; k0 < K; k0 += 2) {
        const int k = k0 + kh;
        float a[2], b[2];
#pragma unroll
        for (int i = 0; i < 2; ++i) {
            const long row = m0 + i * 32 + r32;
            a[i] = (row < M && k < K) ? x[row * K + k] : 0.f;
        }
#pragma unroll
        for (int j = 0; j < 2; ++j) {
            const int col = n0 + j * 32 + r32;
            b[j] = (col < N && k < K) ? w[(long)col * K + k] : 0.f;
        }
#pragma unroll
        for (int i = 0; i < 2; ++i)
#pragma unroll
            for (int j = 0; j < 2; ++j)
                acc[i][j] = __builtin_amdgcn_mfma_f32_32x32x2f32(a[i], b[j], acc[i][j], 0, 0, 0);
    }
#pragma unroll
    for (int i = 0; i < 2; ++i)
#pragma unroll
        for (int j = 0; j < 2; ++j)
            store_tile<float, TO>(acc[i][j], y, bias, res, m0 + i * 32, n0 + j * 32, M, N, act, lane);
}

}

using namespace tramba;

extern "C" int tramba_linear_cl(const void *x, const void *w, const float *bias, const void *residual,
                                void *y, int64_t m, int n, int k, int act, int dtype, int out_dtype,
                                void *stream)
{
    TRAMBA_CHECK(x && w && y, "linear_cl: null tensor");
    TRAMBA_CHECK(m > 0 && n > 0 && k > 0, "linear_cl: empty shape");
    TRAMBA_CHECK(out_dtype == dtype || out_dtype == TRAMBA_F32, "linear_cl: out dtype must be dtype or f32");
    TRAMBA_CHECK(act >= TRAMBA_ACT_NONE && act <= TRAMBA_ACT_GELU_GRAD_MUL, "linear_cl: unknown activation %d", act);
    TRAMBA_CHECK(residual || (act != TRAMBA_ACT_SIGMOID_GATE && act != TRAMBA_ACT_GELU_GRAD_MUL),
                 "linear_cl: activation %d combines with a `residual` operand, none given", act);
    const long gy = (m + 127) / 128, gx = (n + 127) / 128;
    TRAMBA_CHECK(gy <= 65535, "linear_cl: M=%ld exceeds grid limits", (long)m);
    hipStream_t s = (hipStream_t)stream;
    ProfScope prof(TRAMBA_PROF_GEMM, s, 2.0 * (double)m * n * k);
    dim3 grid((unsigned)gx, (unsigned)gy), block(256);
    const int vec = (k % 8 == 0) && aligned16(x) && aligned16(w);
    const bool tiled = vec && dtype != TRAMBA_F32 && aligned16(y) && (residual == nullptr || aligned16(residual)) &&
                       (m + 63) / 64 <= 65535;
    if (tiled) {
        launch_gemm16(gemm_plan(GEMM_PLAIN, m, n, k, act, out_dtype == dtype), GemmArgs{x, w, bias, residual, y, m, n, k, act},
                      dtype, out_dtype, s);
        TRAMBA_LAUNCH_CHECK();
        return TRAMBA_OK;
    }
    if (dtype == TRAMBA_F32) {
        hipLaunchKernelGGL(linear32_kernel<float>, grid, block, 0, s, (const float *)x, (const float *)w, bias,
                           (const float *)residual, (float *)y, (long)m, n, k, act);
    } else if (dtype == TRAMBA_BF16) {
        using T = __hip_bfloat16;
        if (out_dtype == TRAMBA_F32)
            hipLaunchKernelGGL((linear16_kernel<T, float>), grid, block, 0, s, (const T *)x, (const T *)w, bias,
                               (const T *)residual, (float *)y, (long)m, n, k, act, vec);
        else
            hipLaunchKernelGGL((linear16_kernel<T, T>), grid, block, 0, s, (const T *)x, (const T *)w, bias,
                               (const T *)residual, (T *)y, (long)m, n, k, act, vec);
    } else if (dtype == TRAMBA_F16) {
        using T = __half;
        if (out_dtype == TRAMBA_F32)
            hipLaunchKernelGGL((linear16_kernel<T, float>), grid, block, 0, s, (const T *)x, (const T *)w, bias,
                               (const T *)residual, (float *)y, (long)m, n, k, act, vec);
        else
            hipLaunchKernelGGL((linear16_kernel<T, T>), grid, block, 0, s, (const T *)x, (const T *)w, bias,
                               (const T *)residual, (T *)y, (long)m, n, k, act, vec);
    } else {
        set_error("linear_cl: bad dtype %d", dtype);
        return TRAMBA_ERR_ARG;
    }
    TRAMBA_LAUNCH_CHECK();
    return TRAMBA_OK;
}

extern "C" int tramba_linear_ln_cl(const void *x, const void *w_folded, const float *colsum, const float *bias,
                                   const void *residual, void *y, int64_t m, int n, int k, float eps, int act, int dtype,
                                   int out_dtype, void *stream)
{
    TRAMBA_CHECK(x && w_folded && colsum && y, "linear_ln_cl: null tensor");
    TRAMBA_CHECK(m > 0 && n > 0 && k > 0, "linear_ln_cl: empty shape");
    TRAMBA_CHECK(dtype == TRAMBA_BF16 || dtype == TRAMBA_F16, "linear_ln_cl: 16-bit activations only");
    TRAMBA_CHECK(out_dtype == dtype || out_dtype == TRAMBA_F32, "linear_ln_cl: output must be the input dtype or f32");
    TRAMBA_CHECK(k % 64 == 0 && k <= 2048 && n % 8 == 0, "linear_ln_cl: needs K %% 64 == 0, K <= 2048, N %% 8 == 0");
    TRAMBA_CHECK(aligned16(x) && aligned16(w_folded) && aligned16(y) && aligned16(colsum) && (!bias || aligned16(bias)) &&
                     (!residual || aligned16(residual)),
                 "linear_ln_cl: tensors must be 16-byte aligned");
    hipStream_t s = (hipStream_t)stream;
    ProfScope prof(TRAMBA_PROF_GEMM, s, 2.0 * (double)m * n * k);
    GemmArgs a{x, w_folded, bias, residual, y, m, n, k, act};
    a.li = LnIn{colsum, eps};
    launch_gemm16<true>(gemm_plan(GEMM_LN, m, n, k, act, out_dtype == dtype), a, dtype, out_dtype, s);
    TRAMBA_LAUNCH_CHECK();
    return TRAMBA_OK;
}

extern "C" int tramba_linear2_cl(const void *x1, const void *x2, int k1, const void *w, const float *bias,
                                 const void *residual, void *y, int64_t m, int n, int k, int act, int dtype,
                                 int out_dtype, void *stream)
{
    TRAMBA_CHECK(x1 && x2 && w && y, "linear2_cl: null tensor");
    TRAMBA_CHECK(m > 0 && n > 0 && k > 0 && k1 > 0 && k1 < k, "linear2_cl: empty shape");
    TRAMBA_CHECK(dtype == TRAMBA_BF16 || dtype == TRAMBA_F16, "linear2_cl: 16-bit dtypes only");
    TRAMBA_CHECK(out_dtype == dtype || out_dtype == TRAMBA_F32, "linear2_cl: out dtype must be dtype or f32");
    TRAMBA_CHECK(k1 % 64 == 0 && (k - k1) % 64 == 0, "linear2_cl: both K parts must be multiples of 64 (%d + %d)", k1, k - k1);
    TRAMBA_CHECK(aligned16(x1) && aligned16(x2) && aligned16(w) && aligned16(y) && (residual == nullptr || aligned16(residual)),
                 "linear2_cl: tensors must be 16-byte aligned");
    TRAMBA_CHECK((m + 63) / 64 <= 65535 && (double)k * 2.0 * 128.0 < 2147483648.0, "linear2_cl: shape exceeds this build's limits");
    hipStream_t s = (hipStream_t)stream;
    ProfScope prof(TRAMBA_PROF_GEMM, s, 2.0 * (double)m * n * k);
    GemmArgs a{x1, w, bias, residual, y, m, n, k, act};
    a.x2 = x2;
    a.k1 = k1;
    launch_gemm16(gemm_plan(GEMM_TWO_SRC, m, n, k, act, out_dtype == dtype), a, dtype, out_dtype, s);
    TRAMBA_LAUNCH_CHECK();
    return TRAMBA_OK;
}

extern "C" int tramba_expand_norm_head_cl(const void *x, const void *w, const float *ln_w, const float *ln_b,
                                          const float *head_w, float head_b, float *y, int batch, int h, int wd, int cin,
                                          int p, float eps, int dtype, void *stream)
{
    TRAMBA_CHECK(x && w && ln_w && ln_b && head_w && y, "expand_norm_head_cl: null tensor");
    TRAMBA_CHECK(batch > 0 && h > 0 && wd > 0 && cin > 0 && p > 0, "expand_norm_head_cl: empty shape");
    TRAMBA_CHECK(dtype == TRAMBA_BF16 || dtype == TRAMBA_F16, "expand_norm_head_cl: 16-bit dtypes only");
    TRAMBA_CHECK(cin % 64 == 0, "expand_norm_head_cl: Cin=%d must be a multiple of 64", cin);
    TRAMBA_CHECK(aligned16(x) && aligned16(w), "expand_norm_head_cl: tensors must be 16-byte aligned");
    const long m = (long)batch * h * wd;
    const int n = p * p * 128;
    TRAMBA_CHECK(m < 2147483647L && (m + 63) / 64 <= 65535, "expand_norm_head_cl: too many pixels");
    hipStream_t s = (hipStream_t)stream;
    ProfScope prof(TRAMBA_PROF_GEMM, s, 2.0 * (double)m * n * cin);
    const LnHead hd{ln_w, ln_b, head_w, head_b, eps, h, wd, p, y};
    dim3 grid((unsigned)(n / 128), (unsigned)((m + 63) / 64)), block(256);
    if (dtype == TRAMBA_BF16) {
        using T = __hip_bfloat16;
        hipLaunchKernelGGL((linear_lean_kernel<T, T, 64, 128, 1, true>), grid, block, 0, s, (const T *)x, (const T *)w,
                           (const float *)nullptr, (const T *)nullptr, (T *)nullptr, m, n, cin, 0, (const T *)nullptr, 0, hd);
    } else {
        using T = __half;
        hipLaunchKernelGGL((linear_lean_kernel<T, T, 64, 128, 1, true>), grid, block, 0, s, (const T *)x, (const T *)w,
                           (const float *)nullptr, (const T *)nullptr, (T *)nullptr, m, n, cin, 0, (const T *)nullptr, 0, hd);
    }
    TRAMBA_LAUNCH_CHECK();
    return TRAMBA_OK;
}

extern "C" int tramba_conv3x3s2_cl(const void *x, const void *w, const float *bias, void *y, int batch, int hin,
                                   int win, int cin, int cout, int dtype, void *stream)
{
    TRAMBA_CHECK(x && w && y, "conv3x3s2_cl: null tensor");
    TRAMBA_CHECK(batch > 0 && hin > 0 && win > 0 && cin > 0 && cout > 0, "conv3x3s2_cl: empty shape");
    TRAMBA_CHECK(cin % 64 == 0, "conv3x3s2_cl: Cin=%d must be a multiple of 64", cin);
    TRAMBA_CHECK(dtype == TRAMBA_BF16 || dtype == TRAMBA_F16, "conv3x3s2_cl: bf16/f16 only (fp32 convs run on MIOpen)");
    TRAMBA_CHECK(aligned16(x) && aligned16(w) && aligned16(y), "conv3x3s2_cl: tensors must be 16-byte aligned");
    ConvGeom cg{hin, win, cin, (hin + 1) / 2, (win + 1) / 2};
    const long m = (long)batch * cg.hout * cg.wout;
    TRAMBA_CHECK((m + 63) / 64 <= 65535, "conv3x3s2_cl: too many output pixels");
    hipStream_t s = (hipStream_t)stream;
    const double xbytes = (double)batch * hin * win * cin * 2.0;
    const GemmPlan p = gemm_plan(GEMM_CONV, m, cout, 9 * cin, TRAMBA_ACT_NONE, true, xbytes < 2147483648.0);
    GemmArgs a{x, w, bias, nullptr, y, m, cout, 9 * cin, TRAMBA_ACT_NONE};
    a.cg = cg;
    a.abytes = (unsigned)xbytes;
    if (dtype == TRAMBA_BF16) launch_gemm<__hip_bfloat16, __hip_bfloat16, false, false, true>(p, a, s);
    else launch_gemm<__half, __half, false, false, true>(p, a, s);
    TRAMBA_LAUNCH_CHECK();
    return TRAMBA_OK;
}

extern "C" int tramba_linear_dual_cl(const void *x, const void *w, const float *bias, void *y_pre, void *y_act, int64_t m,
                                     int n, int k, int act, int dtype, void *stream)
{
    TRAMBA_CHECK(x && w && y_pre && y_act, "linear_dual_cl: null tensor");
    TRAMBA_CHECK(m > 0 && n > 0 && k > 0, "linear_dual_cl: empty shape");
    TRAMBA_CHECK(dtype == TRAMBA_BF16 || dtype == TRAMBA_F16, "linear_dual_cl: 16-bit activations only");
    TRAMBA_CHECK(act == TRAMBA_ACT_GELU || act == TRAMBA_ACT_SILU, "linear_dual_cl: act must be GELU or SiLU");
    TRAMBA_CHECK(k % 64 == 0 && n % 8 == 0 && (double)k * 2.0 * 128.0 < 2147483648.0 && (m + 63) / 64 <= 65535,
                 "linear_dual_cl: needs K %% 64 == 0, N %% 8 == 0");
    TRAMBA_CHECK(aligned16(x) && aligned16(w) && aligned16(y_pre) && aligned16(y_act), "linear_dual_cl: 16-byte alignment");
    hipStream_t s = (hipStream_t)stream;
    ProfScope prof(TRAMBA_PROF_GEMM, s, 2.0 * (double)m * n * k);
    const GemmPlan p = gemm_plan(GEMM_DUAL, m, n, k, act, true);
    GemmArgs a{x, w, bias, nullptr, y_act, m, n, k, act};
    a.y_pre = y_pre;
    if (dtype == TRAMBA_BF16) launch_gemm<__hip_bfloat16, __hip_bfloat16, false, true>(p, a, s);
    else launch_gemm<__half, __half, false, true>(p, a, s);
    TRAMBA_LAUNCH_CHECK();
    return TRAMBA_OK;
}
```

### tramba_amd/hip.py

```python
import ctypes
import os
import threading
import weakref

import numpy as np
import torch

_HERE = os.path.dirname(os.path.abspath(__file__))
LIB_PATH = os.path.join(_HERE, "_lib", "libtramba_hip.so")

F32, F16, BF16 = 0, 1, 2
ACT_NONE, ACT_SILU, ACT_GELU, ACT_SIGMOID_GATE, ACT_GELU_GRAD_MUL = 0, 1, 2, 3, 4
SCAN_RASTER, SCAN_LINE, SCAN_HELIX, SCAN_WINDOW, SCAN_DILATION = range(5)
FAMILY = {"raster": SCAN_RASTER, "line": SCAN_LINE, "helix": SCAN_HELIX, "window": SCAN_WINDOW,
          "dilation": SCAN_DILATION}
PROF_SCAN_BOUNDARY, PROF_SCAN_FUSED, PROF_GEMM, PROF_MERGE, PROF_SCAN_BWD, PROF_WGRAD, PROF_LAYERNORM, PROF_DW = 0, 1, 2, 3, 4, 5, 6, 7

_DT = {torch.float32: F32, torch.float16: F16, torch.bfloat16: BF16}

c_int, c_i64, c_f, c_vp = ctypes.c_int, ctypes.c_int64, ctypes.c_float, ctypes.c_void_p

SIGNATURES = {
    "tramba_last_error": (ctypes.c_char_p, []),
    "tramba_abi_version": (c_int, []),
# ... 2 lines not shown
    "tramba_tune_get": (c_int, [c_int]),
    "tramba_profile_enable": (c_int, [c_int, c_int]),
    "tramba_profile_read": (c_int, [c_int, ctypes.POINTER(ctypes.c_double), ctypes.POINTER(ctypes.c_double)]),
    "tramba_profile_min_units": (c_int, [c_int, ctypes.c_double]),
    "tramba_scan_family_k": (c_int, [c_int]),
    "tramba_default_window": (c_int, [c_int]),
    "tramba_scan_table": (c_int, [c_int, c_int, c_int, c_int, c_vp]),
    "tramba_scan_table_inverse": (c_int, [c_vp, c_int, c_int, c_vp, c_vp]),
    "tramba_selective_scan_nchunk": (c_int, [c_int, c_int]),
    "tramba_selective_scan_max_dstate": (c_int, []),
    "tramba_selective_scan_fwd": (c_int, [c_vp] * 9 + [c_int] * 8 + [c_vp]),
    "tramba_selective_scan_bwd": (c_int, [c_vp] * 16 + [c_int] * 8 + [c_vp]),
    "tramba_selective_scan_bwd_det_work": (c_i64, [c_int] * 6),
    "tramba_selective_scan_bwd_det": (c_int, [c_vp] * 17 + [ctypes.c_size_t] + [c_int] * 7 + [c_vp]),
    "tramba_cross_scan": (c_int, [c_vp, c_vp, c_vp, c_int, c_int, c_int, c_int, c_int, c_vp]),
    "tramba_cross_merge": (c_int, [c_vp, c_vp, c_vp, c_vp, c_int, c_int, c_int, c_int, c_int, c_vp]),
    "tramba_ss2d_group_stride": (c_int, [c_int]),
    "tramba_ss2d_scan_workspace": (ctypes.c_size_t, [c_int] * 4),
    "tramba_ss2d_scan_cl": (c_int, [c_vp] * 9 + [ctypes.c_size_t] + [c_int] * 7 + [c_vp, c_int, c_vp]),
    "tramba_ss2d_group_stride_n": (c_int, [c_int] * 2),
    "tramba_ss2d_scan_n_workspace": (ctypes.c_size_t, [c_int] * 5),
    "tramba_ss2d_scan_n_plan": (c_int, [c_int] * 5 + [c_vp] * 2),
    "tramba_ss2d_scan_n_cl": (c_int, [c_vp] * 9 + [ctypes.c_size_t] + [c_int] * 8 + [c_vp]),
    "tramba_ss2d_scan_bwd_workspace": (ctypes.c_size_t, [c_int] * 4),
    "tramba_ss2d_scan_bwd_cl": (c_int, [c_vp] * 12 + [c_int, c_vp, c_vp, ctypes.c_size_t] + [c_int] * 9 + [c_vp]),
    "tramba_ss2d_bwd_prep_cl": (c_int, [c_vp] * 6 + [c_int] * 6 + [c_vp]),
    "tramba_ss2d_bwd_assemble_cl": (c_int, [c_vp] * 4 + [c_int] * 5 + [c_vp]),
    "tramba_ss2d_scan_n_bwd_workspace": (ctypes.c_size_t, [c_int] * 6),
    "tramba_ss2d_scan_n_bwd_plan": (c_int, [c_int] * 5 + [c_vp] * 2),
    "tramba_ss2d_scan_n_bwd_cl": (c_int, [c_vp] * 14 + [ctypes.c_size_t] + [c_int] * 8 + [c_vp]),
    "tramba_ss2d_bwd_prep_n_cl": (c_int, [c_vp] * 6 + [c_int] * 7 + [c_vp]),
    "tramba_ss2d_bwd_assemble_n_cl": (c_int, [c_vp] * 4 + [c_int] * 6 + [c_vp]),
    "tramba_ss2d_merge_grad_cl": (c_int, [c_vp] * 8 + [c_int] * 4 + [c_f, c_int, c_int, c_int, c_vp]),
    "tramba_ss2d_merge_norm_cl": (c_int, [c_vp] * 6 + [c_int] * 4 + [c_f, c_int, c_int, c_int, c_vp]),
    "tramba_layernorm_cl": (c_int, [c_vp] * 4 + [c_i64, c_int, c_f, c_int, c_int, c_vp]),
    "tramba_layernorm_bwd_parts": (c_i64, [c_i64, c_int, c_int]),
    "tramba_layernorm_bwd_cl": (c_int, [c_vp] * 5 + [c_i64, c_int, c_f, c_int, c_vp]),
    "tramba_layernorm_bwd_res_cl": (c_int, [c_vp] * 7 + [c_i64, c_vp, c_i64, c_int, c_f, c_int, c_vp]),
    "tramba_layernorm_bwd_any_cl": (c_int, [c_vp] * 7 + [c_i64, c_vp, c_i64, c_int, c_f, c_int, c_int, c_int, c_int, c_vp]),
    "tramba_shuffle_norm_bwd_cl": (c_int, [c_vp] * 5 + [c_int] * 5 + [c_f, c_int, c_vp]),
    "tramba_add_layernorm_cl": (c_int, [c_vp] * 3 + [c_i64] + [c_vp] * 5 + [c_i64, c_int, c_f, c_int, c_int, c_vp]),
    "tramba_shuffle_norm_cl": (c_int, [c_vp] * 4 + [c_int] * 5 + [c_f, c_int, c_vp]),
    "tramba_shuffle_norm_head_cl": (c_int, [c_vp] * 4 + [c_f, c_vp] + [c_int] * 5 + [c_f, c_int, c_vp]),
    "tramba_shuffle_norm_head_bwd_parts": (c_i64, [c_int] * 6),
    "tramba_shuffle_norm_head_bwd_cl": (c_int, [c_vp] * 6 + [c_int] * 5 + [c_f, c_int, c_vp]),
    "tramba_rowdot_cl": (c_int, [c_vp, c_vp, c_f, c_vp, c_i64, c_int, c_int, c_vp]),
    "tramba_rowdot_bwd_parts": (c_i64, [c_i64, c_int, c_int]),
    "tramba_rowdot_bwd_cl": (c_int, [c_vp] * 5 + [c_i64, c_int, c_int, c_vp]),
    "tramba_saliency_stats": (c_int, [c_vp] * 4 + [c_int] * 3 + [c_vp]),
    "tramba_feature_transform": (c_int, [c_vp] * 3 + [c_int] * 3 + [c_vp]),
    "tramba_weighted_f_workspace": (ctypes.c_size_t, [c_int] * 3),
    "tramba_weighted_f_sums": (c_int, [c_vp] * 7 + [ctypes.c_size_t] + [c_int] * 3 + [c_vp]),
    "tramba_resize_table_words": (ctypes.c_size_t, [c_int] * 4),
    "tramba_resize_table": (c_int, [c_int] * 4 + [c_vp] * 3 + [ctypes.c_size_t]),
    "tramba_frames_to_input": (c_int, [c_vp] * 3 + [c_int] * 6 + [c_vp]),
    "tramba_logits_to_u8": (c_int, [c_vp] * 2 + [c_int] * 6 + [c_vp]),
    "tramba_frames_ragged_check": (c_int, [c_vp, c_int, c_int, ctypes.c_size_t, ctypes.c_size_t, c_int]),
    "tramba_frames_to_input_ragged": (c_int, [c_vp, c_vp, ctypes.c_size_t, c_vp, c_int, c_int, c_int, c_vp]),
    "tramba_logits_to_u8_ragged": (c_int, [c_vp] * 4 + [ctypes.c_size_t] + [c_int] * 3 + [c_vp]),
    "tramba_augment_source_table_words": (ctypes.c_size_t, [c_int] * 3),
    "tramba_augment_source_table": (c_int, [c_int] * 3 + [c_vp, ctypes.c_size_t]),
    "tramba_augment_size_table_words": (ctypes.c_size_t, [c_int]),
    "tramba_augment_size_table": (c_int, [c_int] + [c_vp] * 3 + [ctypes.c_size_t]),
    "tramba_augment_scale_taps": (c_int, [c_int] * 2),
    "tramba_augment_rotation": (c_int, [c_int] * 2 + [c_vp]),
    "tramba_augment_workspace": (ctypes.c_size_t, [c_int] * 2),
    "tramba_augment_batch": (c_int, [c_vp] * 2 + [ctypes.c_size_t] + [c_vp] * 4 + [ctypes.c_size_t] + [c_int] * 2 + [c_vp]),
    "tramba_dw_pack": (c_int, [c_vp] * 8 + [c_int] * 2 + [c_vp]),
    "tramba_dwconv_cl": (c_int, [c_vp] * 4 + [c_int] * 7 + [c_vp]),
    "tramba_dwconv_dual_cl": (c_int, [c_vp] * 5 + [c_int] * 8 + [c_vp]),
    "tramba_dw_unpack_grad": (c_int, [c_vp] * 5 + [c_int] * 3 + [c_vp]),
    "tramba_dw_pack_multi": (c_int, [c_vp] * 10 + [c_int, c_vp]),
    "tramba_dw_unpack_grad_multi": (c_int, [c_vp] * 8 + [c_int, c_vp]),
    "tramba_im2col3x3_cl": (c_int, [c_vp] * 2 + [c_int] * 8 + [c_vp]),
    "tramba_upsample_bilinear_bwd": (c_int, [c_vp] * 2 + [c_int] * 5 + [c_vp]),
    "tramba_col2im3x3_cl": (c_int, [c_vp] * 2 + [c_int] * 8 + [c_vp]),
    "tramba_dwconv_wgrad_parts": (c_i64, [c_int, c_int, c_int, c_int, c_int]),
    "tramba_dwconv_wgrad_cl": (c_int, [c_vp] * 3 + [c_int] * 6 + [c_vp]),
    "tramba_dct_split_cl": (c_int, [c_vp] * 6 + [c_int] * 4 + [c_vp]),
    "tramba_linear_cl": (c_int, [c_vp] * 5 + [c_i64, c_int, c_int, c_int, c_int, c_int, c_vp]),
    "tramba_linear_dual_cl": (c_int, [c_vp] * 5 + [c_i64, c_int, c_int, c_int, c_int, c_vp]),
    "tramba_linear_ln_cl": (c_int, [c_vp] * 6 + [c_i64, c_int, c_int, c_f, c_int, c_int, c_int, c_vp]),
    "tramba_linear2_cl": (c_int, [c_vp, c_vp, c_int] + [c_vp] * 4 + [c_i64, c_int, c_int, c_int, c_int, c_int, c_vp]),
    "tramba_wgrad_workspace": (ctypes.c_size_t, [c_i64, c_int, c_int, c_int, c_int]),
    "tramba_wgrad_cl": (c_int, [c_vp] * 4 + [ctypes.c_size_t, c_i64, c_int, c_int, c_int, c_int, c_i64, c_i64, c_int, c_i64,
                                             c_i64, c_int, c_int, c_int, c_vp]),
    "tramba_rows_gemm_cl": (c_int, [c_vp] * 3 + [c_int, c_i64, c_int, c_int, c_int, c_int, c_int, c_vp]),
    "tramba_shadow_cast_multi": (c_int, [c_vp, c_int, c_i64, c_int, c_vp]),
    "tramba_slab_sum": (c_int, [c_vp, c_vp, c_i64, c_int, c_vp]),
    "tramba_multi_sum": (c_int, [c_vp, c_vp, c_vp, c_vp, c_int, c_vp]),
    "tramba_multi_sum_strided": (c_int, [c_vp, c_vp, c_vp, c_vp, c_vp, c_int, c_vp]),
    "tramba_wgrad_parts_cl": (c_int, [c_vp] * 4 + [ctypes.c_size_t, c_i64, c_int, c_int, c_int, c_int, c_i64, c_i64, c_int, c_i64,
                                                   c_i64, c_int, c_int, c_int, c_vp, c_vp]),
    "tramba_expand_norm_head_cl": (c_int, [c_vp] * 5 + [c_f, c_vp] + [c_int] * 5 + [c_f, c_int, c_vp]),
    "tramba_conv3x3s2_cl": (c_int, [c_vp] * 4 + [c_int] * 6 + [c_vp]),
    "tramba_stem_conv_ln_gelu": (c_int, [c_vp] * 6 + [c_int] * 3 + [c_f, c_int, c_int, c_vp]),
    "tramba_sod_loss_sums": (c_int, [c_vp] * 3 + [c_int] * 6 + [c_vp]),
    "tramba_sod_loss_finish": (c_int, [c_vp] * 4 + [c_int, c_int, c_i64, c_vp, c_vp]),
    "tramba_sod_loss_grad_workspace": (ctypes.c_size_t, [c_int] * 5),
    "tramba_sod_loss_grad": (c_int, [c_vp] * 6 + [ctypes.c_size_t] + [c_int] * 5 + [c_vp]),
    "tramba_loss_weight_map": (c_int, [c_vp] * 2 + [c_int] * 4 + [c_vp]),
    "tramba_sod_wloss_sums": (c_int, [c_vp] * 4 + [c_int] * 6 + [c_f, c_int, c_vp]),
    "tramba_sod_wloss_finish": (c_int, [c_vp] * 4 + [c_int, c_int, c_i64, c_int, c_int, c_vp, c_vp]),
    "tramba_sod_wloss_grad_workspace": (ctypes.c_size_t, [c_int] * 5),
    "tramba_sod_wloss_grad": (c_int, [c_vp] * 7 + [ctypes.c_size_t] + [c_int] * 5 + [c_f, c_int, c_vp]),
    "tramba_adam_step": (c_int, [c_vp] * 6 + [c_int] + [ctypes.c_double] * 5 + [c_vp]),
    "tramba_grad_accumulate": (c_int, [c_vp] * 3 + [c_int, c_vp, c_vp]),
    "tramba_grad_norm_workspace": (ctypes.c_size_t, [c_vp, c_int]),
    "tramba_grad_norm": (c_int, [c_vp] * 2 + [c_int, ctypes.c_double, ctypes.c_double, c_int, c_vp, c_vp, ctypes.c_size_t, c_vp]),
    "tramba_adam_step_ctl": (c_int, [c_vp] * 6 + [c_int] + [ctypes.c_double] * 5 + [c_vp] * 3),
    "tramba_window_attn_cl": (c_int, [c_vp] * 3 + [c_int] * 8 + [c_vp]),
    "tramba_kv_attn_cl": (c_int, [c_vp] * 3 + [c_int, c_i64] + [c_int] * 4 + [c_vp]),
    "tramba_window_attn_bwd_work": (ctypes.c_size_t, [c_int] * 6),
    "tramba_window_attn_bwd_cl": (c_int, [c_vp] * 6 + [ctypes.c_size_t] + [c_int] * 8 + [c_vp]),
    "tramba_kv_attn_bwd_work": (ctypes.c_size_t, [c_int, c_i64, c_int, c_int, c_int]),
    "tramba_kv_attn_bwd_cl": (c_int, [c_vp] * 6 + [ctypes.c_size_t, c_int, c_i64] + [c_int] * 4 + [c_vp]),
    "tramba_patch_conv_cl": (c_int, [c_vp] * 4 + [c_int] * 7 + [c_vp]),
    "tramba_patch_conv_dgrad_cl": (c_int, [c_vp] * 3 + [c_int] * 7 + [c_vp]),
    "tramba_patch_conv_wgrad_split": (c_int, [c_int] * 6),
    "tramba_patch_conv_wgrad_work": (ctypes.c_size_t, [c_int] * 6),
    "tramba_patch_conv_wgrad_cl": (c_int, [c_vp] * 3 + [ctypes.c_size_t] + [c_int] * 8 + [c_vp]),
    "tramba_patch_embed_ln": (c_int, [c_vp] * 6 + [c_int] * 7 + [c_f, c_int, c_int, c_vp]),
    "tramba_conv_affine_cl": (c_int, [c_vp] * 6 + [c_int] * 9 + [c_vp]),
    "tramba_stem7_affine_relu_pool": (c_int, [c_vp] * 5 + [c_int] * 5 + [c_vp]),
    "tramba_conv_dgrad_cl": (c_int, [c_vp] * 3 + [c_int] * 8 + [c_vp]),
    "tramba_conv_wgrad_split": (c_int, [c_int] * 7),
    "tramba_conv_wgrad_work": (ctypes.c_size_t, [c_int] * 7),
    "tramba_conv_wgrad_cl": (c_int, [c_vp] * 3 + [ctypes.c_size_t] + [c_int] * 8 + [c_vp]),
    "tramba_bn_parts": (c_int, [c_i64, c_int]),
    "tramba_bn_work": (ctypes.c_size_t, [c_i64, c_int]),
    "tramba_bn_stats_cl": (c_int, [c_vp] * 6 + [ctypes.c_size_t, c_i64, c_int, c_f, c_f, c_int, c_vp]),
    "tramba_bn_act_cl": (c_int, [c_vp] * 7 + [c_i64, c_int, c_int, c_int, c_vp]),
    "tramba_bn_act_bwd_cl": (c_int, [c_vp] * 11 + [ctypes.c_size_t, c_i64, c_int, c_int, c_int, c_vp]),
    "tramba_maxpool3s2_cl": (c_int, [c_vp] * 2 + [c_int] * 5 + [c_vp]),
    "tramba_maxpool3s2_bwd_cl": (c_int, [c_vp] * 3 + [c_int] * 5 + [c_vp]),
}

_lib = None
_lock = threading.Lock()


def lib():
    global _lib
    if _lib is None:
        with _lock:
            if _lib is None:
                if not os.path.exists(LIB_PATH):
                    raise RuntimeError(
                        f"{LIB_PATH} is missing: build it with `python -m tramba_amd.buildlib` "
                        "(hipcc, gfx950).  tramba_amd has no CPU or PyTorch fallback.")
                l = ctypes.CDLL(LIB_PATH)
                for name, (res, args) in SIGNATURES.items():
                    fn = getattr(l, name)
                    fn.restype, fn.argtypes = res, args
                _lib = l
    return _lib


class TrambaHipError(RuntimeError):
    pass


def _check(rc, what):
    if rc < 0:
        raise TrambaHipError(f"{what}: {lib().tramba_last_error().decode()} (code {rc})")
    return rc
# ... 1064 lines not shown

def step_ctl_record(device):
    rec = torch.zeros(STEP_CTL_BYTES // 8, dtype=torch.int64, device=device)
    f, i = rec.view(torch.float32), rec.view(torch.int32)
    return rec, {"norm": f[0], "scale": f[1], "skip": i[2], "micro": i[3], "skipped_steps": rec[2]}


def grad_accumulate_raw(accs, grads, numel, n, ctl):
    _check(lib().tramba_grad_accumulate(accs, grads, numel, n, ctl.data_ptr(), _stream()), "grad_accumulate")


def grad_norm_workspace(numel, n):
    return lib().tramba_grad_norm_workspace(numel, n)


def grad_norm_raw(grads, numel, n, mean_scale, max_norm, skip_nonfinite, ctl, workspace):
    _check(lib().tramba_grad_norm(grads, numel, n, float(mean_scale), float(max_norm or 0.0), int(bool(skip_nonfinite)),
                                  ctl.data_ptr(), workspace.data_ptr(), workspace.numel() * workspace.element_size(), _stream()),
           "grad_norm")


def im2col3x3_cl(x, stride, pad, ckp):
    _dev(x)
    bb, h, wd, c = x.shape
    ho, wo = (h + 2 * pad - 3) // stride + 1, (wd + 2 * pad - 3) // stride + 1
    cols = torch.empty((bb * ho * wo, ckp), dtype=x.dtype, device=x.device)
    _check(lib().tramba_im2col3x3_cl(_ptr(x), _ptr(cols), bb, h, wd, c, stride, pad, ckp, dt(x), _stream()), "im2col3x3_cl")
    return cols


def col2im3x3_cl(gcols, shape, stride, pad):
    _dev(gcols)
    bb, h, wd, c = shape
    gx = torch.empty(shape, dtype=gcols.dtype, device=gcols.device)
    _check(lib().tramba_col2im3x3_cl(_ptr(gcols), _ptr(gx), bb, h, wd, c, stride, pad, gcols.shape[1], dt(gcols), _stream()),
           "col2im3x3_cl")
    return gx


def dwconv_wgrad_cl(x, gy, ks):
    _dev(x, gy)
    bb, h, wd, c = x.shape
    if gy.shape != x.shape or gy.dtype != x.dtype:
        raise TrambaHipError("dwconv_wgrad_cl: x / gy mismatch")
    part = torch.empty((lib().tramba_dwconv_wgrad_parts(bb, h, wd, c, ks), ks * ks + 1, c), dtype=torch.float32, device=x.device)
    _check(lib().tramba_dwconv_wgrad_cl(_ptr(x), _ptr(gy), _ptr(part), bb, h, wd, c, ks, dt(x), _stream()),
           "dwconv_wgrad_cl")
    s = slab_sum(part)
    return s[:ks * ks], s[ks * ks]


def dwconv_wgrad_table(x, gy, ks, defer=False):
    _dev(x, gy)
    bb, h, wd, c = x.shape
    if gy.shape != x.shape or gy.dtype != x.dtype:
        raise TrambaHipError("dwconv_wgrad_cl: x / gy mismatch")
    part = torch.empty((lib().tramba_dwconv_wgrad_parts(bb, h, wd, c, ks), ks * ks + 1, c), dtype=torch.float32, device=x.device)
    _check(lib().tramba_dwconv_wgrad_cl(_ptr(x), _ptr(gy), _ptr(part), bb, h, wd, c, ks, dt(x), _stream()),
           "dwconv_wgrad_cl")
    return slab_sum(part, defer=defer)


def dct_split_cl(x, wx, wy):
    _dev(x, wx, wy)
    bb, n, n2, c = x.shape
    if n != n2 or n % 2:
        raise TrambaHipError(f"dct_split_cl: need an even square map, got {n}x{n2}")
    tmp = torch.empty((bb, n, n, c), dtype=torch.float32, device=x.device)
    high = torch.empty((bb, n // 2, n // 2, c), dtype=x.dtype, device=x.device)
    low = torch.empty_like(high)
    _check(lib().tramba_dct_split_cl(_ptr(x), _ptr(wx), _ptr(wy), _ptr(tmp), _ptr(high), _ptr(low), bb, n, c,
                                     dt(x), _stream()), "dct_split_cl")
    return high, low


def _check_epilogue(what, bias, residual, dtype, m, n):
    if bias is not None and (bias.dtype != torch.float32 or bias.numel() != n):
        raise TrambaHipError(f"{what}: bias must be float32 with {n} elements, got {bias.dtype} x {bias.numel()}")
    if residual is not None and (residual.dtype != dtype or residual.numel() != m * n):
        raise TrambaHipError(f"{what}: residual must be {dtype} with {m} x {n} elements, got {residual.dtype} x "
                             f"{residual.numel()}")


def linear_cl(x, w, bias=None, residual=None, act=ACT_NONE, out_dtype=None):
    _dev(x, w, bias, residual)
    k = x.shape[-1]
    n = w.shape[0]
    m = x.numel() // k
    out_dtype = x.dtype if out_dtype is None else out_dtype
    y = torch.empty(x.shape[:-1] + (n,), dtype=out_dtype, device=x.device)
    if w.dtype != x.dtype or w.shape[1] != k:
        raise TrambaHipError("linear_cl: weight dtype/shape mismatch")
    _check_epilogue("linear_cl", bias, residual, x.dtype, m, n)
    _check(lib().tramba_linear_cl(_ptr(x), _ptr(w), _ptr(bias), _ptr(residual), _ptr(y), m, n, k, act, dt(x),
                                  dt(y), _stream()), "linear_cl")
    return y


_ATTN_DTYPES = (torch.bfloat16, torch.float16)


def window_attention_supported(dtype, h, w, c, heads, ws, shift):
    return (dtype in _ATTN_DTYPES and heads > 0 and c % heads == 0 and c // heads in (32, 64) and h > 0 and w > 0
            and 1 <= ws and ws * ws <= 256 and h % ws == 0 and w % ws == 0 and 0 <= shift < ws)


def kv_attention_supported(dtype, m, c, heads):
    return dtype in _ATTN_DTYPES and heads > 0 and c % heads == 0 and c // heads in (32, 64) and 1 <= m <= 256


def window_attention_cl(qkv, table, ws, shift, heads):
    _dev(qkv, table)
    if heads <= 0 or qkv.dim() != 4 or qkv.shape[-1] % (3 * heads):
        raise TrambaHipError(f"window_attention_cl: qkv must be (B, H, W, 3 * heads * hd), got {tuple(qkv.shape)}")
    b, h, w, c3 = qkv.shape
    if table.dtype != torch.float32 or tuple(table.shape) != ((2 * ws - 1) ** 2, heads):
        raise TrambaHipError(f"window_attention_cl: table must be float32 ({(2 * ws - 1) ** 2}, {heads}), got {table.dtype} "
                             f"{tuple(table.shape)}")
    y = torch.empty((b, h, w, c3 // 3), dtype=qkv.dtype, device=qkv.device)
    _check(lib().tramba_window_attn_cl(_ptr(qkv), _ptr(table), _ptr(y), b, h, w, heads, c3 // (3 * heads), ws, shift, dt(qkv),
                                       _stream()), "window_attention_cl")
    return y


def kv_attention_cl(q, kv, heads):
    _dev(q, kv)
    if heads <= 0 or q.dim() != 3 or kv.dim() != 3 or kv.shape[0] != q.shape[0] or kv.shape[2] != 2 * q.shape[2] or kv.dtype != q.dtype \
            or q.shape[2] % heads:
        raise TrambaHipError(f"kv_attention_cl: need q (B, N, C) and kv (B, M, 2 C) of one dtype, got {tuple(q.shape)} "
                             f"{tuple(kv.shape)}")
    b, n, c = q.shape
    y = torch.empty_like(q)
    _check(lib().tramba_kv_attn_cl(_ptr(q), _ptr(kv), _ptr(y), b, n, kv.shape[1], heads, c // heads, dt(q), _stream()),
           "kv_attention_cl")
    return y


def window_attention_train_supported(dtype, h, w, c, heads, ws, shift):
    return window_attention_supported(dtype, h, w, c, heads, ws, shift)


def kv_attention_train_supported(dtype, m, c, heads):
    return kv_attention_supported(dtype, m, c, heads)


def _attn_out(name, what, out, shape, dtype, device):
    if out is None:
        return torch.empty(shape, dtype=dtype, device=device)
    _dev(out)
    if tuple(out.shape) != tuple(shape) or out.dtype != dtype:
        raise TrambaHipError(f"{name}: {what} must be {dtype} {tuple(shape)}, got {out.dtype} {tuple(out.shape)}")
    return out


def window_attention_bwd_cl(qkv, table, dy, ws, shift, heads, need_table=True, out=None):
    _dev(qkv, table, dy)
    if heads <= 0 or qkv.dim() != 4 or qkv.shape[-1] % (3 * heads):
        raise TrambaHipError(f"window_attention_bwd_cl: qkv must be (B, H, W, 3 * heads * hd), got {tuple(qkv.shape)}")
    b, h, w, c3 = qkv.shape
    if table.dtype != torch.float32 or tuple(table.shape) != ((2 * ws - 1) ** 2, heads):
        raise TrambaHipError(f"window_attention_bwd_cl: table must be float32 ({(2 * ws - 1) ** 2}, {heads}), got "
                             f"{table.dtype} {tuple(table.shape)}")
    if dy.dtype != qkv.dtype or tuple(dy.shape) != (b, h, w, c3 // 3):
        raise TrambaHipError(f"window_attention_bwd_cl: dy must be {qkv.dtype} {(b, h, w, c3 // 3)}, got {dy.dtype} "
                             f"{tuple(dy.shape)}")
    o_qkv, o_table = out if out is not None else (None, None)
    dqkv = _attn_out("window_attention_bwd_cl", "dqkv", o_qkv, qkv.shape, qkv.dtype, qkv.device)
    dtable = _attn_out("window_attention_bwd_cl", "dtable", o_table, table.shape, torch.float32, qkv.device) if need_table else None
    hd = c3 // (3 * heads)
    nbytes = lib().tramba_window_attn_bwd_work(b, h, w, heads, hd, ws) if need_table else 0
    work = torch.empty(nbytes, dtype=torch.uint8, device=qkv.device) if nbytes else None
    _check(lib().tramba_window_attn_bwd_cl(_ptr(qkv), _ptr(table), _ptr(dy), _ptr(dqkv), _ptr(dtable), _ptr(work), nbytes, b, h,
                                           w, heads, hd, ws, shift, dt(qkv), _stream()), "window_attention_bwd_cl")
    return dqkv, dtable


def kv_attention_bwd_cl(q, kv, dy, heads, out=None):
    _dev(q, kv, dy)
    if heads <= 0 or q.dim() != 3 or kv.dim() != 3 or kv.shape[0] != q.shape[0] or kv.shape[2] != 2 * q.shape[2] or kv.dtype != q.dtype \
            or q.shape[2] % heads or dy.shape != q.shape or dy.dtype != q.dtype:
        raise TrambaHipError(f"kv_attention_bwd_cl: need q, dy (B, N, C) and kv (B, M, 2 C) of one dtype, got {tuple(q.shape)} "
                             f"{tuple(dy.shape)} {tuple(kv.shape)}")
    b, n, c = q.shape
    m = kv.shape[1]
    o_q, o_kv = out if out is not None else (None, None)
    dq = _attn_out("kv_attention_bwd_cl", "dq", o_q, q.shape, q.dtype, q.device)
    dkv = _attn_out("kv_attention_bwd_cl", "dkv", o_kv, kv.shape, q.dtype, q.device)
    nbytes = lib().tramba_kv_attn_bwd_work(b, n, m, heads, c // heads)
    work = torch.empty(max(nbytes, 16), dtype=torch.uint8, device=q.device)
    _check(lib().tramba_kv_attn_bwd_cl(_ptr(q), _ptr(kv), _ptr(dy), _ptr(dq), _ptr(dkv), _ptr(work), nbytes, b, n, m, heads,
                                       c // heads, dt(q), _stream()), "kv_attention_bwd_cl")
    return dq, dkv


def linear_dual_ok(x, w):
    return (x.is_cuda and x.dtype in (torch.bfloat16, torch.float16) and w.dtype == x.dtype and x.shape[-1] % 64 == 0
            and w.shape[0] % 8 == 0 and x.is_contiguous() and w.is_contiguous())


def linear_dual_cl(x, w, bias, act):
    _dev(x, w, bias)
    k, n = x.shape[-1], w.shape[0]
    m = x.numel() // k
    if not linear_dual_ok(x, w) or w.shape[1] != k:
        raise TrambaHipError("linear_dual_cl: needs 16-bit contiguous operands with K % 64 == 0 and N % 8 == 0")
    _check_epilogue("linear_dual_cl", bias, None, x.dtype, m, n)
    y_pre = torch.empty(x.shape[:-1] + (n,), dtype=x.dtype, device=x.device)
    y_act = torch.empty_like(y_pre)
    _check(lib().tramba_linear_dual_cl(_ptr(x), _ptr(w), _ptr(bias), _ptr(y_pre), _ptr(y_act), m, n, k, act, dt(x), _stream()),
           "linear_dual_cl")
    return y_pre, y_act


def linear_ln_cl(x, w_folded, colsum, bias, eps, residual=None, act=ACT_NONE, out_dtype=None):
    _dev(x, w_folded, colsum, bias, residual)
    k = x.shape[-1]
    n = w_folded.shape[0]
    m = x.numel() // k
    if w_folded.dtype != x.dtype or w_folded.shape[1] != k or colsum.dtype != torch.float32 or colsum.numel() != n:
        raise TrambaHipError("linear_ln_cl: operand shapes / dtypes do not match")
    _check_epilogue("linear_ln_cl", bias, residual, x.dtype, m, n)
    out_dtype = x.dtype if out_dtype is None else out_dtype
    y = torch.empty(x.shape[:-1] + (n,), dtype=out_dtype, device=x.device)
    _check(lib().tramba_linear_ln_cl(_ptr(x), _ptr(w_folded), _ptr(colsum), _ptr(bias), _ptr(residual), _ptr(y), m, n, k,
                                     float(eps), act, dt(x), dt(y), _stream()), "linear_ln_cl")
    return y


def linear2_cl(x1, x2, w, bias=None, residual=None, act=ACT_NONE, out_dtype=None):
    _dev(x1, x2, w, bias, residual)
    k1, k2 = x1.shape[-1], x2.shape[-1]
    n = w.shape[0]
    m = x1.numel() // k1
    if x2.shape[:-1] != x1.shape[:-1] or w.shape[1] != k1 + k2 or w.dtype != x1.dtype or x2.dtype != x1.dtype:
        raise TrambaHipError("linear2_cl: operand shapes / dtypes do not match")
    _check_epilogue("linear2_cl", bias, residual, x1.dtype, m, n)
    out_dtype = x1.dtype if out_dtype is None else out_dtype
    y = torch.empty(x1.shape[:-1] + (n,), dtype=out_dtype, device=x1.device)
    _check(lib().tramba_linear2_cl(_ptr(x1), _ptr(x2), k1, _ptr(w), _ptr(bias), _ptr(residual), _ptr(y), m, n, k1 + k2,
                                   act, dt(x1), dt(y), _stream()), "linear2_cl")
    return y


def wgrad_cl(gy, x, want_bias=False, defer=False):
    n, k = gy.shape[-1], x.shape[-1]
    gy2, x2 = gy.reshape(-1, n), x.reshape(-1, k)
    if gy2.stride(-1) != 1 or x2.stride(-1) != 1:
        gy2, x2 = gy2.contiguous(), x2.contiguous()
    m = gy2.shape[0]
    if x2.shape[0] != m or gy2.dtype != x2.dtype:
        raise TrambaHipError("wgrad_cl: gy / x mismatch")
    return _wgrad(gy2, x2, m, n, k, 1, 1, 0, 0, gy2.stride(0), 0, 0, x2.stride(0), want_bias, defer)


def wgrad_rows_cl(gy, x, segments, defer=False):
    _dev(gy, x)
    m, n = gy.shape
    k = x.shape[-1]
    if x.shape[0] != m or gy.dtype != x.dtype:
        raise TrambaHipError("wgrad_rows_cl: gy / x mismatch")
    if any(a < 0 or c <= 0 or a + c > n for a, c in segments):
        raise TrambaHipError("wgrad_rows_cl: a row range outside the gradient")
    total = sum(c for _, c in segments)
    if defer and _sumq.enabled:
        ws_bytes = lib().tramba_wgrad_workspace(m, n, k, 1, 1)
        ws = torch.empty(ws_bytes, dtype=torch.uint8, device=gy.device)
        full = torch.empty((1, n * k + n), dtype=torch.float32, device=gy.device)
        nslab = ctypes.c_int(0)
        _check(lib().tramba_wgrad_parts_cl(_ptr(gy), _ptr(x), _ptr(full), _ptr(ws), ws_bytes, m, n, k, 1, 1, 0, 0, n, 0, 0, k, 0,
                                           dt(gy), _stream(), ctypes.byref(nslab)), "wgrad_parts_cl")
        if nslab.value > 0:
            out = torch.empty((total, k), dtype=torch.float32, device=gy.device)
            if _sumq.poison:
                out.fill_(float("nan"))
            row = 0
            for a, c in segments:
                _enqueue_sum(_ptr(ws) + a * k * 4, _ptr(out) + row * k * 4, c * k, nslab.value, (ws, out), stride=n * k + n)
                row += c
            return out.view(total, k)
        gw = full[0, :n * k].view(n, k)
    else:
        gw = wgrad_cl(gy, x)[0]
    return torch.cat([gw[a:a + c] for a, c in segments], dim=0)


def wgrad_grouped_cl(gy, x, defer=False):
    _dev(gy, x)
    b, g, l, n = gy.shape
    k = x.shape[-1]
    if x.shape[:3] != gy.shape[:3] or gy.dtype != x.dtype:
        raise TrambaHipError("wgrad_grouped_cl: gy / x mismatch")
    out, _ = _wgrad(gy, x, l, n, k, g, b, g * l * n, l * n, n, g * l * k, l * k, k, False, defer)
    return out


def tn_shared_cl(a, x):
    _dev(a, x)
    nb = a.shape[0] if a.dim() == 3 else 1
    t, n = a.shape[-2:]
    g, t2, k = x.shape
    if t2 != t or a.dtype != x.dtype:
        raise TrambaHipError("tn_shared_cl: operand shapes / dtypes do not match")
    out, _ = _wgrad(a, x, t, n, k, g, nb, t * n, 0, n, 0, t * k, k, False)
    return out if g > 1 else out.view(1, n, k)


def _wgrad(gy, x, m, n, k, groups, nbatch, gy_bs, gy_gs, gy_ld, x_bs, x_gs, x_ld, want_bias, defer=False):
    for t in (gy, x):
        if not t.is_cuda:
            raise TrambaHipError("tramba_amd kernels need tensors on a HIP device (no CPU fallback)")
    ws_bytes = lib().tramba_wgrad_workspace(m, n, k, groups, nbatch)
    ws = torch.empty(ws_bytes, dtype=torch.uint8, device=gy.device)
    out = torch.empty((groups, n * k + n), dtype=torch.float32, device=gy.device)
    if defer and _sumq.enabled:
        nslab = ctypes.c_int(0)
        _check(lib().tramba_wgrad_parts_cl(_ptr(gy), _ptr(x), _ptr(out), _ptr(ws), ws_bytes, m, n, k, groups, nbatch, gy_bs,
                                           gy_gs, gy_ld, x_bs, x_gs, x_ld, int(want_bias), dt(gy), _stream(),
                                           ctypes.byref(nslab)), "wgrad_parts_cl")
        if nslab.value > 0:
            slab = n * k + n
            if groups > 1 and not want_bias:
# ... 466 lines not shown
```

### tramba_amd/modules.py

```python
import math
from collections import OrderedDict

import torch
import torch.nn as nn
import torch.nn.functional as F

from . import hip
from .ops import (CrossMerge, CrossMerge_Dilation, CrossMerge_Line, CrossMerge_Window, CrossScan,
                  CrossScan_Dilation, CrossScan_Line, CrossScan_Window, SelectiveScanOflex)



FOLD_LAYERNORM = True


def to_cl(x: torch.Tensor) -> torch.Tensor:
    return x.permute(0, 2, 3, 1).contiguous()


def from_cl(x: torch.Tensor) -> torch.Tensor:
    return x.permute(0, 3, 1, 2)


def _need_device(x):
    if not x.is_cuda:
        raise RuntimeError("tramba_amd runs on a HIP device only (MI355X); got a CPU tensor. "
                           "There is deliberately no CPU fallback.")


def _infer(*tensors) -> bool:
    if not torch.is_grad_enabled():
        return True
    return not any(t is not None and t.requires_grad for t in tensors)


def _f32(p):
    return hip._f32(p)


class _PackCache:

    def __init__(self):
        self._store = {}

    def get(self, name, params, builder):
        key = tuple((p._version, p.data_ptr(), p.dtype, str(p.device)) for p in params if p is not None)
        hit = self._store.get(name)
        if hit is None or hit[0] != key:
            with torch.no_grad():
                hit = (key, builder())
            self._store[name] = hit
        return hit[1]


def _cache(module) -> _PackCache:
    c = module.__dict__.get("_tramba_cache")
    if c is None:
        c = module.__dict__["_tramba_cache"] = _PackCache()
    return c


def _act_torch(x, act):
    if act == hip.ACT_GELU:
        return F.gelu(x)
    if act == hip.ACT_SILU:
        return F.silu(x)
    return x


def _split16(t):
    hi = t.to(torch.bfloat16)
    return hi, (t - hi.float()).to(torch.bfloat16)


def _wgrad(gy2, x2, want_bias=False, defer=False):
    if gy2.dtype != torch.float32:
        return hip.wgrad_cl(gy2, x2, want_bias, defer)
    gh, gl = _split16(gy2)
    xh, xl = _split16(x2)
    gw = hip.wgrad_cl(gh, xh)[0] + hip.wgrad_cl(gh, xl)[0] + hip.wgrad_cl(gl, xh)[0]
    return gw, (gy2.sum(0) if want_bias else None)


def _dgrad(gy2, wa, wa_t=None):
    return hip.linear_cl(gy2, wa.t().contiguous() if wa_t is None else wa_t)


class _ConvIm2colCL(torch.autograd.Function):

    @staticmethod
    def forward(ctx, x, w, b, stride, padding):
        bsz, h, wd, cin = x.shape
        cout, _, kh, kw = w.shape
        if (kh, kw) != (3, 3) or stride[0] != stride[1] or padding[0] != padding[1]:
            raise NotImplementedError("the training path of a dense convolution is built for 3x3 kernels with one stride / padding")
        st, pd = int(stride[0]), int(padding[0])
# ... 360 lines not shown

    @staticmethod
    def forward(ctx, x1, x2, w, b):
        wa = _lowp(w, x1.dtype).detach().contiguous()
        k1, k2 = x1.shape[-1], x2.shape[-1]
        a1, a2 = x1.reshape(-1, k1).contiguous(), x2.reshape(-1, k2).contiguous()
        ctx.save_for_backward(a1, a2, wa)
        ctx.wa_t = _lowp_t(w, x1.dtype)
        ctx.wdtype, ctx.has_bias, ctx.shapes = w.dtype, b is not None, (x1.shape, x2.shape)
        y = hip.linear2_cl(a1, a2, wa, None if b is None else b.detach().float().contiguous())
        return y.view(x1.shape[:-1] + (wa.shape[0],))

    @staticmethod
    def backward(ctx, gy):
        a1, a2, wa = ctx.saved_tensors
        k1 = a1.shape[1]
        gy2 = gy.reshape(-1, gy.shape[-1])
        gy2 = gy2 if gy2.is_contiguous() and gy2.dtype == a1.dtype else gy2.to(a1.dtype).contiguous()
        wt = wa.t().contiguous() if ctx.wa_t is None else ctx.wa_t
        g1 = hip.linear_cl(gy2, wt[:k1]).view(ctx.shapes[0]) if ctx.needs_input_grad[0] else None
        g2 = hip.linear_cl(gy2, wt[k1:]).view(ctx.shapes[1]) if ctx.needs_input_grad[1] else None
        gw = gb = None
        if ctx.needs_input_grad[2] or (ctx.has_bias and ctx.needs_input_grad[3]):
            gw1, gb = _wgrad(gy2, a1, ctx.has_bias)
            gw = torch.cat((gw1, _wgrad(gy2, a2)[0]), dim=1).to(ctx.wdtype)
        return g1, g2, gw, gb


class _ShuffleNormHeadCL(torch.autograd.Function):

    @staticmethod
    def forward(ctx, x, ln_w, ln_b, head_w, p, eps):
        x = x.contiguous()
        y = hip.shuffle_norm_head_cl(x, hip._f32(ln_w), hip._f32(ln_b), hip._f32(head_w).reshape(-1), 0.0, p, eps)
        ctx.save_for_backward(x, ln_w, ln_b, head_w)
        ctx.p, ctx.eps = p, eps
        return y

    @staticmethod
    def backward(ctx, g):
        x, ln_w, ln_b, head_w = ctx.saved_tensors
        gam, bet, hw = ln_w.detach().float(), ln_b.detach().float(), head_w.detach().float().reshape(-1)
        dx, part = hip.shuffle_norm_head_bwd_cl(x, g.contiguous().float(), gam, hw, ctx.p, ctx.eps)
        s_ = hip.slab_sum(part)
        c = gam.numel()
        a, gs = s_[:c], s_[c]
        return (dx if ctx.needs_input_grad[0] else None, (hw * a).to(ln_w.dtype), (hw * gs).to(ln_b.dtype),
                (gam * a + bet * gs).reshape(head_w.shape).to(head_w.dtype), None, None)


class _RowDotCL(torch.autograd.Function):

    @staticmethod
    def forward(ctx, x, w, b):
        x = x.contiguous()
        wf = w.detach().float().reshape(-1).contiguous()
        ctx.save_for_backward(x, wf)
        ctx.wshape, ctx.wdtype = w.shape, w.dtype
        return hip.rowdot_cl(x, wf, 0.0) + b.detach().float()

    @staticmethod
    def backward(ctx, gy):
        x, wf = ctx.saved_tensors
        gx = gw = gb = None
        if hip.rowdot_bwd_ok(x):
            gx, gw, gb = hip.rowdot_bwd_cl(x, gy.float().contiguous(), wf)
            return gx, gw.reshape(ctx.wshape).to(ctx.wdtype), gb.reshape(1)
        if ctx.needs_input_grad[0]:
            gx = (gy.unsqueeze(-1) * wf).to(x.dtype)
        if ctx.needs_input_grad[1]:
            g8 = torch.zeros((gy.numel(), 8), dtype=x.dtype, device=x.device)
            g8[:, 0] = gy.reshape(-1)
            gw = _wgrad(g8, x.view(-1, x.shape[-1]))[0][0].reshape(ctx.wshape).to(ctx.wdtype)
        if ctx.needs_input_grad[2]:
            gb = gy.sum().reshape(1)
        return gx, gw, gb


class Linear2d(nn.Linear):

    def _forward_cl(self, x, act=hip.ACT_NONE, residual=None, out_dtype=None, gelu_in=False, gelu_ready=None):
        if _infer(x, self.weight):
            w = self.weight if self.weight.dtype == x.dtype else self.weight.to(x.dtype)
            return hip.linear_cl(F.gelu(x) if gelu_in else x, w.detach(), _f32(self.bias), residual, act, out_dtype)
        if gelu_in:
            y = _act_torch(_GeluLinearTrainCL.apply(x, self.weight, self.bias, gelu_ready), act)
        else:
            y = _act_torch(_LinearTrainCL.apply(x, self.weight, self.bias), act)
        if residual is not None:
            y = y + residual
        return y if out_dtype is None else y.to(out_dtype)

    def _forward_gelu_pair_cl(self, x):
        if (not _infer(x, self.weight) and x.is_cuda and x.dtype in (torch.bfloat16, torch.float16) and x.shape[-1] % 64 == 0
                and self.weight.shape[0] % 8 == 0):
            return _LinearGeluPairTrainCL.apply(x, self.weight, self.bias)
        return self._forward_cl(x), None

    def _forward_norm_cl(self, x, norm, act=hip.ACT_NONE, residual=None, out_dtype=None):
        k = x.shape[-1]
        if (FOLD_LAYERNORM and _infer(x, self.weight, norm.weight) and x.dtype != torch.float32 and k % 64 == 0 and k <= 2048
                and self.weight.shape[0] % 8 == 0):
            wf, cs, tb = _cache(self).get(("lnfold", x.dtype, id(norm)), (self.weight, self.bias, norm.weight, norm.bias),
                                          lambda: _fold_layernorm(self, norm, x.dtype))
            return hip.linear_ln_cl(x, wf, cs, tb, norm.eps, residual, act, out_dtype)
        return self._forward_cl(norm._forward_cl(x), act=act, residual=residual, out_dtype=out_dtype)

    def _forward_cat_cl(self, x1, x2, act=hip.ACT_NONE, residual=None, out_dtype=None):
        if (_infer(x1, x2, self.weight) and x1.dtype != torch.float32
                and x1.dtype == x2.dtype
                and x1.shape[-1] % 64 == 0 and x2.shape[-1] % 64 == 0):
            w = self.weight if self.weight.dtype == x1.dtype else self.weight.to(x1.dtype)
            return hip.linear2_cl(x1.contiguous(), x2.contiguous(), w.detach(), _f32(self.bias), residual, act, out_dtype)
        gate = act == hip.ACT_SIGMOID_GATE
        if (x1.is_cuda and x1.dtype in (torch.bfloat16, torch.float16) and x2.dtype == x1.dtype and out_dtype is None
                and x1.shape[-1] % 64 == 0 and x2.shape[-1] % 64 == 0 and self.weight.shape[0] % 8 == 0):
            y = _act_torch(_Linear2TrainCL.apply(x1, x2, self.weight, self.bias), hip.ACT_NONE if gate else act)
            if gate:
                return torch.sigmoid(y) * residual
            return y if residual is None else y + residual
        y = self._forward_cl(torch.cat((x1, x2), dim=-1), act=hip.ACT_NONE if gate else act,
                             residual=None if gate else residual, out_dtype=out_dtype)
        return torch.sigmoid(y) * residual if gate else y

    def forward(self, x):
        _need_device(x)
        return from_cl(self._forward_cl(to_cl(x)))

    def _load_from_state_dict(self, state_dict, prefix, local_metadata, strict, missing_keys, unexpected_keys,
                              error_msgs):
        key = prefix + "weight"
        if key in state_dict:
            state_dict[key] = state_dict[key].view(self.weight.shape)
        return super()._load_from_state_dict(state_dict, prefix, local_metadata, strict, missing_keys,
                                             unexpected_keys, error_msgs)


def _fold_layernorm(lin, norm, dtype):
    w = lin.weight.detach().float()
    wf = (w * norm.weight.detach().float()[None, :]).to(dtype).contiguous()
    colsum = wf.float().sum(dim=1).contiguous()
    t = (w * norm.bias.detach().float()[None, :]).sum(dim=1)
    if lin.bias is not None:
        t = t + lin.bias.detach().float()
    return wf, colsum, t.contiguous()


class _LayerNormCL(torch.autograd.Function):

    @staticmethod
    def forward(ctx, x, w, b, eps):
        x = x.contiguous()
        wf = w.detach().float().contiguous()
        ctx.save_for_backward(x, wf)
        ctx.eps = eps
        ctx.defer = w.dtype == torch.float32 and b.dtype == torch.float32
        return hip.layernorm_cl(x, wf, b.detach().float().contiguous(), eps, hip.ACT_NONE)

    @staticmethod
    def backward(ctx, gy):
        x, wf = ctx.saved_tensors
        dx, dw, db = hip.layernorm_bwd_cl(x, gy.contiguous().to(x.dtype), wf, ctx.eps, defer=ctx.defer)
        return dx, dw, db, None


class LayerNorm2d(nn.LayerNorm):

    def _forward_cl(self, x, act=hip.ACT_NONE):
        if _infer(x, self.weight):
            return hip.layernorm_cl(x, _f32(self.weight), _f32(self.bias), self.eps, act)
        _need_device(x)
        return _act_torch(_LayerNormCL.apply(x, self.weight, self.bias, self.eps), act)

    def forward(self, x):
        _need_device(x)
        return from_cl(self._forward_cl(to_cl(x)))


class Permute(nn.Module):
    def __init__(self, *args):
        super().__init__()
        self.args = args

    def forward(self, x):
        return x.permute(*self.args).contiguous()


class Mlp(nn.Module):
# ... 363 lines not shown
            order._flat_inverse = inv
        if inv is not False:
            g_xd = g_seq.view(b, k * l, rg)[:, inv]
        else:
            g_xd = torch.zeros_like(xdf)
            g_xd.index_add_(1, flat, g_seq.view(b, k * l, rg))
        gp = hip.slab_sum(gpar)
        return (gx, g_xd.view(b, l, k * rg), g_dtw, gp[2].reshape(-1), gp[0].reshape(-1), gp[1].reshape(-1), None)


class _Deferred:
    __slots__ = ("x", "y", "mask")

    def __init__(self, x, y, mask):
        self.x, self.y, self.mask = x, y, mask


class _AddMaskedF32(torch.autograd.Function):

    @staticmethod
    def forward(ctx, x, y, mask):
        m = mask.to(y.dtype).view((-1,) + (1,) * (y.dim() - 1))
        ctx.save_for_backward(m)
        return torch.addcmul(x, y, m)

    @staticmethod
    def backward(ctx, g):
        (m,) = ctx.saved_tensors
        return (g if ctx.needs_input_grad[0] else None), (g * m if ctx.needs_input_grad[1] else None), None


def _resolve(v):
    if not isinstance(v, _Deferred):
        return v
    return v.x + v.y if v.mask is None else _AddMaskedF32.apply(v.x, v.y, v.mask)


class _AddLayerNormCL(torch.autograd.Function):

    @staticmethod
    def forward(ctx, x, y, mask, w, b, eps, act, passthrough):
        x = x.contiguous()
        wf = w.detach().float().contiguous()
        xs, n, na = hip.add_layernorm_cl(x, None if y is None else y.contiguous(), mask, wf, b.detach().float().contiguous(),
                                         eps, act, dual=act != hip.ACT_NONE)
        ctx.save_for_backward(x if xs is None else xs, wf, mask)
        ctx.eps, ctx.has_y = eps, y is not None
        ctx.defer = w.dtype == torch.float32 and b.dtype == torch.float32
        if na is not None:
            ctx.mark_non_differentiable(na)
        ctx.set_materialize_grads(False)
        if xs is None:
            xs = x if passthrough else None
        return xs, n, na

    @staticmethod
    def backward(ctx, g_xs, g_n, _g_na):
        xs, wf, mask = ctx.saved_tensors
        if g_n is None:
            gy = None
            if ctx.has_y and g_xs is not None:
                gy = g_xs if mask is None else g_xs * mask.to(g_xs.dtype).view((-1,) + (1,) * (g_xs.dim() - 1))
            return g_xs, gy, None, None, None, None, None, None
        g_n = g_n.contiguous()
        if g_n.dtype != xs.dtype:
            g_n = g_n.to(xs.dtype)
        if g_xs is not None:
            g_xs = g_xs.contiguous()
            if g_xs.dtype != xs.dtype:
                g_xs = g_xs.to(xs.dtype)
        want_m = ctx.has_y and mask is not None and ctx.needs_input_grad[1]
        dx, dxm, dw, db = hip.layernorm_bwd_res_cl(xs, g_n, wf, ctx.eps, gres=g_xs, mask=mask if want_m else None,
                                                   want_masked=want_m, defer=ctx.defer)
        gy = (dxm if want_m else dx) if ctx.has_y else None
        return dx, gy, None, dw, db, None, None, None


def _add_ln(v, norm, act=hip.ACT_NONE):
    if isinstance(v, _Deferred):
        return _AddLayerNormCL.apply(v.x, v.y, v.mask, norm.weight, norm.bias, norm.eps, act, True)
    return _AddLayerNormCL.apply(v, None, None, norm.weight, norm.bias, norm.eps, act, True)


_dw_pack_store = {}
_dw_plans = None


def _dw_versions(srcs):
    return tuple(-1 if t is None else t._version for t in srcs)


def _dw_packed(w, b, w3=None, b3=None, w5=None, b5=None):
    ent = _dw_pack_store.get(w.data_ptr())
    if ent is not None and ent[2] == _dw_versions((w, b, w3, b3, w5, b5)):
        p = ent[3]()
        if p is not None and p.data_ptr() == w.data_ptr() and p.shape == w.shape:
            return ent[0], ent[1]
    return hip.dw_pack(*[None if t is None else t.detach() for t in (w, b, w3, b3, w5, b5)])


def _dw_pack_sources(model):
    out, folded = [], set()
    for m in model.modules():
        if isinstance(m, DWMSMlp):
            c3, c5, c7 = m.dwc3.dw_conv, m.dwc5.dw_conv, m.dwc7.dw_conv
            if all(c.bias is not None for c in (c3, c5, c7)):
                out.append((c7.weight, c7.bias, c3.weight, c3.bias, c5.weight, c5.bias))
                folded.update(id(c) for c in (c3, c5, c7))
    for m in model.modules():
        if isinstance(m, SS2D) and getattr(m, "with_dconv", False):
            out.append((m.conv2d.weight, m.conv2d.bias, None, None, None, None))
    return [g for g in out if all(t is None or (t.is_cuda and t.dtype == torch.float32) for t in g)]


@torch.no_grad()
def refresh_dw_packs(model):
    import weakref
    global _dw_plans
    if _dw_plans is None:
        _dw_plans = weakref.WeakKeyDictionary()
    plan = _dw_plans.get(model)
    srcs = plan[2] if plan is not None else _dw_pack_sources(model)
    if not srcs:
        return 0
    sig = tuple(g[0].data_ptr() for g in srcs)
    if plan is None or plan[0] != sig:
        srcs = _dw_pack_sources(model)
        sig = tuple(g[0].data_ptr() for g in srcs)
        for key in [k for k, ent in _dw_pack_store.items() if ent[3]() is None]:
            del _dw_pack_store[key]
        items = []
        for g in srcs:
            w = g[0]
            c, ks = w.shape[0], w.shape[-1]
            ent = _dw_pack_store.get(w.data_ptr())
            if ent is None or ent[3]() is not w or tuple(ent[0].shape) != (ks * ks, c) or ent[0].device != w.device:
                ent = [torch.empty((ks * ks, c), dtype=torch.float32, device=w.device),
                       torch.empty((c,), dtype=torch.float32, device=w.device), None, weakref.ref(w)]
                _dw_pack_store[w.data_ptr()] = ent
            items.append(tuple(None if t is None else t.detach() for t in g) + (ent[0], ent[1]))
        plan = (sig, hip.dw_pack_multi_prepare(items), srcs)
        _dw_plans[model] = plan
    hip.dw_pack_multi_run(plan[1])
    packs = []
    for g in srcs:
        ent = _dw_pack_store.get(g[0].data_ptr())
        if ent is not None:
            packs += [ent[0], ent[1]]
    if packs:
        torch.autograd.graph.increment_version(packs)
    restamp_dw_packs(model)
    return len(srcs)


def restamp_dw_packs(model):
    plan = None if _dw_plans is None else _dw_plans.get(model)
    if plan is None:
        return
    for g in plan[2]:
        ent = _dw_pack_store.get(g[0].data_ptr())
        if ent is not None and ent[3]() is g[0]:
            ent[2] = _dw_versions(g)


class _DwConvActCL(torch.autograd.Function):

# ... 738 lines not shown
```

Baseline: 875.4 img/s.

## Emit per-row partial LayerNorm statistics from residual GEMM epilogues for the next folded-LN GEMM

GEMM epilogues that write a residual-added output can now also write per-64-column partial sums and sums of squares for each row. The stats are computed from the rounded bf16 values, reduced with DPP, and stored in a slab appended to the output allocation. A later LayerNorm-folded GEMM that reads this tensor loads the slab and folds it into mean and rstd up front. This replaces the in-loop row-statistic accumulation, which issued extra LDS reads of the A tile and shuffles in every k-step. In exchange the producer epilogue does more work and writes more, and the stats are tied to the tensor through a version tag.

```diff
diff --git a/include/tramba_hip.h b/include/tramba_hip.h
--- a/include/tramba_hip.h
+++ b/include/tramba_hip.h
@@ -188,6 +188,14 @@
                         void *y, int64_t m, int n, int k, float eps, int act, int dtype, int out_dtype, void *stream);
 int tramba_linear2_cl(const void *x1, const void *x2, int k1, const void *w, const float *bias, const void *residual,
                       void *y, int64_t m, int n, int k, int act, int dtype, int out_dtype, void *stream);
+int tramba_linear_rowstat_cl(const void *x, const void *w, const float *bias, const void *residual, void *y, int64_t m,
+                             int n, int k, int act, int dtype, int out_dtype, float *rowstat_out, int *emitted, void *stream);
+int tramba_linear2_rowstat_cl(const void *x1, const void *x2, int k1, const void *w, const float *bias, const void *residual,
+                              void *y, int64_t m, int n, int k, int act, int dtype, int out_dtype, float *rowstat_out,
+                              int *emitted, void *stream);
+int tramba_linear_ln_rowstat_cl(const void *x, const void *w_folded, const float *colsum, const float *bias,
+                                const void *residual, void *y, int64_t m, int n, int k, float eps, int act, int dtype,
+                                int out_dtype, const float *rowstat_in, int p, void *stream);
 
 int tramba_linear_dual_cl(const void *x, const void *w, const float *bias, void *y_pre, void *y_act, int64_t m, int n,
                           int k, int act, int dtype, void *stream);
diff --git a/tramba_amd/csrc/linear.hip b/tramba_amd/csrc/linear.hip
--- a/tramba_amd/csrc/linear.hip
+++ b/tramba_amd/csrc/linear.hip
@@ -137,14 +137,24 @@
             }
 }
 
+__device__ __forceinline__ float sum8_dpp(float v)
+{
+    v += __builtin_bit_cast(float, __builtin_amdgcn_update_dpp(0, __builtin_bit_cast(int, v), 0xB1, 0xf, 0xf, true));
+    v += __builtin_bit_cast(float, __builtin_amdgcn_update_dpp(0, __builtin_bit_cast(int, v), 0x4E, 0xf, 0xf, true));
+    v += __builtin_bit_cast(float, __builtin_amdgcn_update_dpp(0, __builtin_bit_cast(int, v), 0x141, 0xf, 0xf, true));
+    return v;
+}
+
 template <typename T, typename TO, int BM, int BN, int NT = 256, typename ACC>
 __device__ __forceinline__ void tile_epilogue(ACC &acc, unsigned char *lds,
                                               const float *__restrict__ bias, const T *__restrict__ res,
                                               TO *__restrict__ y, long M, int N, int act, long m0, int n0,
                                               const float *__restrict__ colsum = nullptr,
                                               const float2 *__restrict__ rowstat = nullptr,
-                                              TO *__restrict__ y_pre = nullptr)
-{
+                                              TO *__restrict__ y_pre = nullptr,
+                                              float2 *__restrict__ stat_out = nullptr)
+{
+    constexpr bool STAT_OK = BN == 64 && sizeof(TO) == 2;
     const int tid = threadIdx.x;
     constexpr int LDE = BN + 4;
     float *ep = reinterpret_cast<float *>(lds);
@@ -159,51 +169,75 @@
     for (int it = 0; it < (BM + RPI - 1) / RPI; ++it) {
         const int row = it * RPI + rl;
         const long grow = m0 + row;
-        if (grow >= M || gcol >= N) continue;
-        float o[CPL];
-        {
-            const float4 v0 = *reinterpret_cast<const float4 *>(ep + row * LDE + cl);
-            const float4 v1 = *reinterpret_cast<const float4 *>(ep + row * LDE + cl + 4);
-            o[0] = v0.x; o[1] = v0.y; o[2] = v0.z; o[3] = v0.w; o[4] = v1.x; o[5] = v1.y; o[6] = v1.z; o[7] = v1.w;
-        }
-        if (gcol + CPL <= N && (N & 7) == 0) {
-            if (colsum) {
-                const float2 st = rowstat[row];
-                float cs[CPL];
-                load_pack<float, CPL>(colsum + gcol, cs);
-#pragma unroll
-                for (int q = 0; q < CPL; ++q) o[q] = st.y * fmaf(-st.x, cs[q], o[q]);
-            }
-            if (bias) {
-                float bv[CPL];
-                load_pack<float, CPL>(bias + gcol, bv);
-#pragma unroll
-                for (int q = 0; q < CPL; ++q) o[q] += bv[q];
-            }
-            if (y_pre) store_pack<TO, CPL>(y_pre + grow * N + gcol, o);
-#pragma unroll
-            for (int q = 0; q < CPL; ++q) o[q] = apply_act(o[q], act);
-            if (res) {
-                float rv[CPL];
-                load_pack<T, CPL>(res + grow * N + gcol, rv);
-#pragma unroll
-                for (int q = 0; q < CPL; ++q) o[q] = combine_residual(o[q], rv[q], act);
-            }
-            store_pack<TO, CPL>(y + grow * N + gcol, o);
-        } else {
-#pragma unroll
-            for (int q = 0; q < CPL; ++q) {
-                if (gcol + q < N) {
-                    if (colsum) o[q] = rowstat[row].y * fmaf(-rowstat[row].x, colsum[gcol + q], o[q]);
-                    const float pre = o[q] + (bias ? bias[gcol + q] : 0.f);
-                    if (y_pre) y_pre[grow * N + gcol + q] = Cvt<TO>::from_f(pre);
-                    float t = apply_act(pre, act);
-                    if (res) {
-                        const float rv = Cvt<T>::to_f(res[grow * N + gcol + q]);
-                        t = combine_residual(t, rv, act);
+        float s1 = 0.f, s2 = 0.f;
+        if (grow < M && gcol < N) {
+            float o[CPL];
+            {
+                const float4 v0 = *reinterpret_cast<const float4 *>(ep + row * LDE + cl);
+                const float4 v1 = *reinterpret_cast<const float4 *>(ep + row * LDE + cl + 4);
+                o[0] = v0.x; o[1] = v0.y; o[2] = v0.z; o[3] = v0.w; o[4] = v1.x; o[5] = v1.y; o[6] = v1.z; o[7] = v1.w;
+            }
+            if (gcol + CPL <= N && (N & 7) == 0) {
+                if (colsum) {
+                    const float2 st = rowstat[row];
+                    float cs[CPL];
+                    load_pack<float, CPL>(colsum + gcol, cs);
+#pragma unroll
+                    for (int q = 0; q < CPL; ++q) o[q] = st.y * fmaf(-st.x, cs[q], o[q]);
+                }
+                if (bias) {
+                    float bv[CPL];
+                    load_pack<float, CPL>(bias + gcol, bv);
+#pragma unroll
+                    for (int q = 0; q < CPL; ++q) o[q] += bv[q];
+                }
+                if (y_pre) store_pack<TO, CPL>(y_pre + grow * N + gcol, o);
+#pragma unroll
+                for (int q = 0; q < CPL; ++q) o[q] = apply_act(o[q], act);
+                if (res) {
+                    float rv[CPL];
+                    load_pack<T, CPL>(res + grow * N + gcol, rv);
+#pragma unroll
+                    for (int q = 0; q < CPL; ++q) o[q] = combine_residual(o[q], rv[q], act);
+                }
+                store_pack<TO, CPL>(y + grow * N + gcol, o);
+                if constexpr (STAT_OK) {
+                    if (stat_out) {
+#pragma unroll
+                        for (int q = 0; q < CPL; ++q) {
+                            const float r = Cvt<TO>::to_f(Cvt<TO>::from_f(o[q]));
+                            s1 += r;
+                            s2 = fmaf(r, r, s2);
+                        }
                     }
-                    y[grow * N + gcol + q] = Cvt<TO>::from_f(t);
                 }
+            } else {
+#pragma unroll
+                for (int q = 0; q < CPL; ++q) {
+                    if (gcol + q < N) {
+                        if (colsum) o[q] = rowstat[row].y * fmaf(-rowstat[row].x, colsum[gcol + q], o[q]);
+                        const float pre = o[q] + (bias ? bias[gcol + q] : 0.f);
+                        if (y_pre) y_pre[grow * N + gcol + q] = Cvt<TO>::from_f(pre);
+                        float t = apply_act(pre, act);
+                        if (res) {
+                            const float rv = Cvt<T>::to_f(res[grow * N + gcol + q]);
+                            t = combine_residual(t, rv, act);
+                        }
+                        y[grow * N + gcol + q] = Cvt<TO>::from_f(t);
+                        if constexpr (STAT_OK) {
+                            const float r = Cvt<TO>::to_f(Cvt<TO>::from_f(t));
+                            s1 += r;
+                            s2 = fmaf(r, r, s2);
+                        }
+                    }
+                }
+            }
+        }
+        if constexpr (STAT_OK) {
+            if (stat_out) {
+                s1 = sum8_dpp(s1);
+                s2 = sum8_dpp(s2);
+                if (cl == 0 && grow < M) stat_out[grow * ((N + BN - 1) / BN) + n0 / BN] = make_float2(s1, s2);
             }
         }
     }
@@ -364,7 +398,40 @@
 struct LnIn {
     const float *colsum;
     float eps;
+    float2 *stat = nullptr;
 };
+
+struct StatIn {
+    float2 v[8];
+};
+__device__ __forceinline__ StatIn statin_load(const float2 *__restrict__ stat, long m0, long M, int nk, int t)
+{
+    StatIn s;
+    const long row = m0 + (t >> 2);
+    const int p0 = (t & 3) * 8;
+#pragma unroll
+    for (int j = 0; j < 8; ++j) {
+        s.v[j] = make_float2(0.f, 0.f);
+        if (row < M && p0 + j < nk) s.v[j] = stat[row * nk + p0 + j];
+    }
+    return s;
+}
+__device__ __forceinline__ void statin_fold(const StatIn &s, float2 *rowstat, int K, float eps, int t)
+{
+    float s1 = 0.f, s2 = 0.f;
+#pragma unroll
+    for (int j = 0; j < 8; ++j) {
+        s1 += s.v[j].x;
+        s2 += s.v[j].y;
+    }
+    s1 += __shfl_xor(s1, 1, 64);
+    s2 += __shfl_xor(s2, 1, 64);
+    s1 += __shfl_xor(s1, 2, 64);
+    s2 += __shfl_xor(s2, 2, 64);
+    const float mean = s1 / (float)K;
+    const float var = fmaxf(s2 / (float)K - mean * mean, 0.f);
+    if ((t & 3) == 0) rowstat[t >> 2] = make_float2(mean, rsqrtf(var + eps));
+}
 
 struct LnHead {
     const float *ln_w, *ln_b, *head_w;
@@ -471,7 +538,7 @@
                                                          const float *__restrict__ bias,
                                                          const T *__restrict__ res, TO *__restrict__ y, long M,
                                                          int N, int K, int act, const T *__restrict__ x2, int K1,
-                                                         LnHead hd = LnHead{})
+                                                         LnHead hd = LnHead{}, float2 *__restrict__ stat_out = nullptr)
 {
     using WL = WaveLayout<BM, BN>;
     constexpr int TM = WL::TM, TN = WL::TN;
@@ -603,13 +670,13 @@
         static_assert(BN == 128, "one tile = whole 128-channel groups");
         tile_epilogue_ln_head<T, BM>(acc, lds, hd, M, m0, n0);
     } else {
-        tile_epilogue<T, TO, BM, BN>(acc, lds, bias, res, y, M, N, act, m0, n0);
+        tile_epilogue<T, TO, BM, BN>(acc, lds, bias, res, y, M, N, act, m0, n0, nullptr, nullptr, nullptr, stat_out);
     }
 }
 
 #define TRAMBA_DSR128_(OUT, ADDR, OFF) asm volatile("ds_read_b128 %0, %1 offset:" #OFF : "=v"(OUT) : "v"(ADDR) : "memory")
 
-template <typename T, typename TO, int NSTG, bool LNIN = false, bool DUAL = false>
+template <typename T, typename TO, int NSTG, bool LNIN = false, bool DUAL = false, bool STATIN = false>
 __global__ __launch_bounds__(256) void linear_dma_kernel(const T *__restrict__ x, const T *__restrict__ w,
                                                         const float *__restrict__ bias, const T *__restrict__ res,
                                                         TO *__restrict__ y, long M, int N, int K, int act,
@@ -621,6 +688,7 @@
     constexpr int EPI_BYTES = BM * (BN + 4) * 4;
     constexpr int LDS_BYTES = NSTG * TILE_BYTES > EPI_BYTES ? NSTG * TILE_BYTES : EPI_BYTES;
     static_assert(NSTG == 2 || NSTG == 3 || NSTG == 4, "stage index = kt % NSTG with the loop unrolled by NSTG (up to 8 stages are coded)");
+    static_assert(LNIN || !STATIN, "supplied row statistics belong to the LayerNorm-folded GEMM");
     __shared__ __attribute__((aligned(1024))) unsigned char lds[LDS_BYTES + (LNIN ? BM * 8 : 0)];
     typedef __attribute__((address_space(3))) void lds_void;
 
@@ -678,9 +746,12 @@
     const unsigned sad = lbase + (unsigned)((tid >> 3) * 128 + (tid & 7) * 16);
 
     constexpr int DEPTH = NSTG - 1;
+    StatIn spart;
+    if constexpr (STATIN) spart = statin_load(li.stat, m0, M, nk, tid);
 #pragma unroll
     for (int t = 0; t < DEPTH; ++t)
         if (t < nk) issue(t, t);
+    if constexpr (STATIN) statin_fold(spart, reinterpret_cast<float2 *>(lds + LDS_BYTES), K, li.eps, tid);
     unsigned aad_hi[4], bad_hi[4];
 #pragma unroll
     for (int kk = 0; kk < 4; ++kk) {
@@ -714,7 +785,7 @@
         const unsigned *aa = STG < 4 ? aad : aad_hi, *ba = STG < 4 ? bad : bad_hi;
         const unsigned sa = STG < 4 ? sad : sad_hi;
 #define TRAMBA_RD_STG_(S, S2)                                                                       \
-    if constexpr (LNIN) { TRAMBA_DSR128_(sv[0], sa, S); TRAMBA_DSR128_(sv[1], sa, S2); }             \
+    if constexpr (LNIN && !STATIN) { TRAMBA_DSR128_(sv[0], sa, S); TRAMBA_DSR128_(sv[1], sa, S2); }  \
     TRAMBA_DSR128_(a[0], aa[0], S); TRAMBA_DSR128_(b[0], ba[0], S); TRAMBA_DSR128_(a[1], aa[1], S);  \
     TRAMBA_DSR128_(b[1], ba[1], S); TRAMBA_DSR128_(a[2], aa[2], S); TRAMBA_DSR128_(b[2], ba[2], S);  \
     TRAMBA_DSR128_(a[3], aa[3], S); TRAMBA_DSR128_(b[3], ba[3], S)
@@ -723,7 +794,7 @@
         else if constexpr ((STG & 3) == 2) { TRAMBA_RD_STG_(32768, 36864); }
         else { TRAMBA_RD_STG_(49152, 53248); }
 #undef TRAMBA_RD_STG_
-        if constexpr (LNIN) {
+        if constexpr (LNIN && !STATIN) {
             asm volatile("s_waitcnt lgkmcnt(8)" : "+v"(sv[0]), "+v"(sv[1]) : : "memory");
 #pragma unroll
             for (int i = 0; i < 2; ++i)
@@ -771,22 +842,25 @@
     __syncthreads();
     if constexpr (LNIN) {
         float2 *rowstat = reinterpret_cast<float2 *>(lds + LDS_BYTES);
-#pragma unroll
-        for (int i = 0; i < 2; ++i) {
-            float s1 = rs1[i], s2 = rs2[i];
-#pragma unroll
-            for (int m = 1; m < 8; m <<= 1) {
-                s1 += __shfl_xor(s1, m, 64);
-                s2 += __shfl_xor(s2, m, 64);
-            }
-            const float mean = s1 / (float)K;
-            const float var = fmaxf(s2 / (float)K - mean * mean, 0.f);
-            if ((tid & 7) == 0) rowstat[(tid >> 3) + 32 * i] = make_float2(mean, rsqrtf(var + li.eps));
+        if constexpr (!STATIN) {
+#pragma unroll
+            for (int i = 0; i < 2; ++i) {
+                float s1 = rs1[i], s2 = rs2[i];
+#pragma unroll
+                for (int m = 1; m < 8; m <<= 1) {
+                    s1 += __shfl_xor(s1, m, 64);
+                    s2 += __shfl_xor(s2, m, 64);
+                }
+                const float mean = s1 / (float)K;
+                const float var = fmaxf(s2 / (float)K - mean * mean, 0.f);
+                if ((tid & 7) == 0) rowstat[(tid >> 3) + 32 * i] = make_float2(mean, rsqrtf(var + li.eps));
+            }
         }
         tile_epilogue<T, TO, BM, BN>(acc, lds, bias, res, y, M, N, act, m0, n0, li.colsum,
                                      reinterpret_cast<const float2 *>(lds + LDS_BYTES));
     } else {
-        tile_epilogue<T, TO, BM, BN>(acc, lds, bias, res, y, M, N, act, m0, n0, nullptr, nullptr, DUAL ? y_pre : nullptr);
+        tile_epilogue<T, TO, BM, BN>(acc, lds, bias, res, y, M, N, act, m0, n0, nullptr, nullptr, DUAL ? y_pre : nullptr,
+                                     DUAL ? nullptr : li.stat);
     }
 #endif
 }
@@ -800,7 +874,7 @@
 };
 
 #define TRAMBA_DSR128_(OUT, ADDR, OFF) asm volatile("ds_read_b128 %0, %1 offset:" #OFF : "=v"(OUT) : "v"(ADDR) : "memory")
-template <typename T, typename TO, int NSTG, bool LNIN = false, bool DUAL = false, int ASRC = A_PLAIN>
+template <typename T, typename TO, int NSTG, bool LNIN = false, bool DUAL = false, int ASRC = A_PLAIN, bool STATIN = false>
 __global__ __launch_bounds__(512, ASRC == A_CONV && NSTG == 3 ? 6 : 1) void linear_pc_kernel(const T *__restrict__ x, const T *__restrict__ w,
                                                        const float *__restrict__ bias, const T *__restrict__ res,
                                                        TO *__restrict__ y, long M, int N, int K, int act,
@@ -813,6 +887,7 @@
     constexpr int EPI_BYTES = BM * (BN + 4) * 4;
     constexpr int LDS_BYTES = NSTG * TILE_BYTES > EPI_BYTES ? NSTG * TILE_BYTES : EPI_BYTES;
     static_assert(NSTG == 3 || NSTG == 4, "stage index = kt % NSTG with the loop unrolled by NSTG");
+    static_assert(LNIN || !STATIN, "supplied row statistics belong to the LayerNorm-folded GEMM");
     __shared__ __attribute__((aligned(1024))) unsigned char lds[LDS_BYTES + (LNIN ? BM * 8 : 0)];
     typedef __attribute__((address_space(3))) void lds_void;
 
@@ -948,6 +1023,9 @@
 #pragma unroll
         for (int t = 0; t < DEPTH; ++t)
             if (t < nk) issue(t, t);
+    } else if constexpr (STATIN) {
+        const StatIn spart = statin_load(li.stat, m0, M, nk, lt);
+        statin_fold(spart, reinterpret_cast<float2 *>(lds + LDS_BYTES), K, li.eps, lt);
     }
     auto kstep = [&](int kt, auto stg_c) {
         constexpr int STG = decltype(stg_c)::value;
@@ -970,7 +1048,7 @@
         } else {
             frag8_t a[4], b[4];
             v4u_t sv[2];
-            if constexpr (LNIN) {
+            if constexpr (LNIN && !STATIN) {
                 if constexpr (STG == 0) { TRAMBA_DSR128_(sv[0], sad, 0); TRAMBA_DSR128_(sv[1], sad, 4096); }
                 else if constexpr (STG == 1) { TRAMBA_DSR128_(sv[0], sad, 16384); TRAMBA_DSR128_(sv[1], sad, 20480); }
                 else if constexpr (STG == 2) { TRAMBA_DSR128_(sv[0], sad, 32768); TRAMBA_DSR128_(sv[1], sad, 36864); }
@@ -985,7 +1063,7 @@
             else if constexpr (STG == 2) { TRAMBA_RD_STG_(32768); }
             else { TRAMBA_RD_STG_(49152); }
 #undef TRAMBA_RD_STG_
-            if constexpr (LNIN) {
+            if constexpr (LNIN && !STATIN) {
                 asm volatile("s_waitcnt lgkmcnt(8)" : "+v"(sv[0]), "+v"(sv[1]) : : "memory");
 #pragma unroll
                 for (int i = 0; i < 2; ++i)
@@ -1023,7 +1101,7 @@
     __syncthreads();
     if constexpr (LNIN) {
         float2 *rowstat = reinterpret_cast<float2 *>(lds + LDS_BYTES);
-        if (!loader) {
+        if (!STATIN && !loader) {
 #pragma unroll
             for (int i = 0; i < 2; ++i) {
                 float s1 = rs1[i], s2 = rs2[i];
@@ -1040,7 +1118,8 @@
         tile_epilogue<T, TO, BM, BN, 512>(acc, lds, bias, res, y, M, N, act, m0, n0, li.colsum,
                                           reinterpret_cast<const float2 *>(lds + LDS_BYTES));
     } else {
-        tile_epilogue<T, TO, BM, BN, 512>(acc, lds, bias, res, y, M, N, act, m0, n0, nullptr, nullptr, DUAL ? y_pre : nullptr);
+        tile_epilogue<T, TO, BM, BN, 512>(acc, lds, bias, res, y, M, N, act, m0, n0, nullptr, nullptr, DUAL ? y_pre : nullptr,
+                                          DUAL ? nullptr : li.stat);
     }
 #endif
 }
@@ -1340,6 +1419,8 @@
     return 3;
 }
 
+static int ln_stat_rule(long tiles64, int k) { return pc_rule(tiles64, k, 0); }
+
 static int ws_ncw(long m, int n, int k)
 {
     if (k != 128 && k != 256) return 0;
@@ -1399,7 +1480,7 @@
     int ncw;
 };
 
-static GemmPlan gemm_plan(GemmKind kind, long m, int n, int k, int act, bool same_dtype, bool a_dma = true)
+static GemmPlan gemm_plan(GemmKind kind, long m, int n, int k, int act, bool same_dtype, bool a_dma = true, bool ln_stat = false)
 {
     int tune = tramba_tune_get(TRAMBA_TUNE_GEMM_TILE);
     if ((kind == GEMM_TWO_SRC || kind == GEMM_CONV) && a_dma && tune != 18 && k % 64 == 0 &&
@@ -1427,7 +1508,7 @@
     case 17: return {GemmForm::PC4, 0};
     }
     const long tiles64 = ((m + 63) / 64) * ((n + 63) / 64);
-    const int pc = tune == 18 ? 0 : pc_rule(tiles64, k, kind);
+    const int pc = tune == 18 ? 0 : (kind == GEMM_LN && ln_stat) ? ln_stat_rule(tiles64, k) : pc_rule(tiles64, k, kind);
     if (pc) return {pc == 4 ? GemmForm::PC4 : GemmForm::PC3, 0};
     if (k <= DMA_SHORT_K && tiles64 >= 1024) return {GemmForm::DMA2, 0};
     if (kind == GEMM_PLAIN && tiles64 <= 256 && k >= 1024) return {GemmForm::DMA4, 0};
@@ -1478,14 +1559,33 @@
                 break;
             }
         }
+        if constexpr (LNIN) {
+            if (a.li.stat) {
+                if (four) hipLaunchKernelGGL((linear_pc_kernel<T, TO, 4, true, false, A_PLAIN, true>), g64, dim3(512), 0, s, x, w, a.bias, res, y, m, n, k, act, a.li, y_pre);
+                else hipLaunchKernelGGL((linear_pc_kernel<T, TO, 3, true, false, A_PLAIN, true>), g64, dim3(512), 0, s, x, w, a.bias, res, y, m, n, k, act, a.li, y_pre);
+                break;
+            }
+        }
         if (four) hipLaunchKernelGGL((linear_pc_kernel<T, TO, 4, LNIN, DUAL>), g64, dim3(512), 0, s, x, w, a.bias, res, y, m, n, k, act, a.li, y_pre);
         else hipLaunchKernelGGL((linear_pc_kernel<T, TO, 3, LNIN, DUAL>), g64, dim3(512), 0, s, x, w, a.bias, res, y, m, n, k, act, a.li, y_pre);
         break;
     }
     case GemmForm::DMA2:
+        if constexpr (LNIN) {
+            if (a.li.stat) {
+                hipLaunchKernelGGL((linear_dma_kernel<T, TO, 2, true, false, true>), g64, dim3(256), 0, s, x, w, a.bias, res, y, m, n, k, act, a.li, y_pre);
+                break;
+            }
+        }
         hipLaunchKernelGGL((linear_dma_kernel<T, TO, 2, LNIN, DUAL>), g64, dim3(256), 0, s, x, w, a.bias, res, y, m, n, k, act, a.li, y_pre);
         break;
     case GemmForm::DMA3:
+        if constexpr (LNIN) {
+            if (a.li.stat) {
+                hipLaunchKernelGGL((linear_dma_kernel<T, TO, 3, true, false, true>), g64, dim3(256), 0, s, x, w, a.bias, res, y, m, n, k, act, a.li, y_pre);
+                break;
+            }
+        }
         hipLaunchKernelGGL((linear_dma_kernel<T, TO, 3, LNIN, DUAL>), g64, dim3(256), 0, s, x, w, a.bias, res, y, m, n, k, act, a.li, y_pre);
         break;
     case GemmForm::DMA4:
@@ -1494,7 +1594,7 @@
         break;
     case GemmForm::LEAN:
         hipLaunchKernelGGL((linear_lean_kernel<T, TO, 64, 64, 1>), g64, dim3(256), 0, s, x, w, a.bias, res, y, m, n, k, act,
-                           (const T *)a.x2, a.k1);
+                           (const T *)a.x2, a.k1, LnHead{}, a.li.stat);
         break;
     case GemmForm::TILED128:
         hipLaunchKernelGGL((linear_tiled_kernel<T, TO, 128, 128, 2, CONV>), g128, dim3(256), 0, s, x, w, a.bias, res, y, m, n, k, act, a.cg);
@@ -1567,10 +1667,31 @@
 
 using namespace tramba;
 
+static bool plan_emits_rowstat(const GemmPlan &p, int dtype, int out_dtype, long m, int n)
+{
+    if (out_dtype != dtype || dtype == TRAMBA_F32) return false;
+    if (tramba_tune_get(TRAMBA_TUNE_GEMM_TILE) == 0 && ws_ncw(m, 2 * n, n) && ws_rule(m, 2 * n, n, GEMM_LN)) return false;
+    switch (p.form) {
+    case GemmForm::PC3: case GemmForm::PC4: case GemmForm::DMA2: case GemmForm::DMA3: case GemmForm::DMA4: case GemmForm::LEAN:
+        return true;
+    default:
+        return false;
+    }
+}
+
 extern "C" int tramba_linear_cl(const void *x, const void *w, const float *bias, const void *residual,
                                 void *y, int64_t m, int n, int k, int act, int dtype, int out_dtype,
                                 void *stream)
 {
+    return tramba_linear_rowstat_cl(x, w, bias, residual, y, m, n, k, act, dtype, out_dtype, nullptr, nullptr, stream);
+}
+
+extern "C" int tramba_linear_rowstat_cl(const void *x, const void *w, const float *bias, const void *residual,
+                                        void *y, int64_t m, int n, int k, int act, int dtype, int out_dtype,
+                                        float *rowstat_out, int *emitted, void *stream)
+{
+    if (emitted) *emitted = 0;
+    TRAMBA_CHECK(!rowstat_out || (emitted && ((size_t)rowstat_out & 7) == 0), "linear_cl: rowstat_out needs `emitted` and 8-byte alignment");
     TRAMBA_CHECK(x && w && y, "linear_cl: null tensor");
     TRAMBA_CHECK(m > 0 && n > 0 && k > 0, "linear_cl: empty shape");
     TRAMBA_CHECK(out_dtype == dtype || out_dtype == TRAMBA_F32, "linear_cl: out dtype must be dtype or f32");
@@ -1586,8 +1707,13 @@
     const bool tiled = vec && dtype != TRAMBA_F32 && aligned16(y) && (residual == nullptr || aligned16(residual)) &&
                        (m + 63) / 64 <= 65535;
     if (tiled) {
-        launch_gemm16(gemm_plan(GEMM_PLAIN, m, n, k, act, out_dtype == dtype), GemmArgs{x, w, bias, residual, y, m, n, k, act},
-                      dtype, out_dtype, s);
+        const GemmPlan p = gemm_plan(GEMM_PLAIN, m, n, k, act, out_dtype == dtype);
+        GemmArgs a{x, w, bias, residual, y, m, n, k, act};
+        if (rowstat_out && plan_emits_rowstat(p, dtype, out_dtype, m, n)) {
+            a.li.stat = reinterpret_cast<float2 *>(rowstat_out);
+            *emitted = 1;
+        }
+        launch_gemm16(p, a, dtype, out_dtype, s);
         TRAMBA_LAUNCH_CHECK();
         return TRAMBA_OK;
     }
@@ -1622,6 +1748,16 @@
                                    const void *residual, void *y, int64_t m, int n, int k, float eps, int act, int dtype,
                                    int out_dtype, void *stream)
 {
+    return tramba_linear_ln_rowstat_cl(x, w_folded, colsum, bias, residual, y, m, n, k, eps, act, dtype, out_dtype, nullptr, 0,
+                                       stream);
+}
+
+extern "C" int tramba_linear_ln_rowstat_cl(const void *x, const void *w_folded, const float *colsum, const float *bias,
+                                           const void *residual, void *y, int64_t m, int n, int k, float eps, int act,
+                                           int dtype, int out_dtype, const float *rowstat_in, int p, void *stream)
+{
+    TRAMBA_CHECK(!rowstat_in || (p > 0 && p == k / 64 && ((size_t)rowstat_in & 7) == 0),
+                 "linear_ln_cl: rowstat_in holds %d partials per row, K = %d needs K / 64 (8-byte aligned)", p, k);
     TRAMBA_CHECK(x && w_folded && colsum && y, "linear_ln_cl: null tensor");
     TRAMBA_CHECK(m > 0 && n > 0 && k > 0, "linear_ln_cl: empty shape");
     TRAMBA_CHECK(dtype == TRAMBA_BF16 || dtype == TRAMBA_F16, "linear_ln_cl: 16-bit activations only");
@@ -1633,8 +1769,8 @@
     hipStream_t s = (hipStream_t)stream;
     ProfScope prof(TRAMBA_PROF_GEMM, s, 2.0 * (double)m * n * k);
     GemmArgs a{x, w_folded, bias, residual, y, m, n, k, act};
-    a.li = LnIn{colsum, eps};
-    launch_gemm16<true>(gemm_plan(GEMM_LN, m, n, k, act, out_dtype == dtype), a, dtype, out_dtype, s);
+    a.li = LnIn{colsum, eps, const_cast<float2 *>(reinterpret_cast<const float2 *>(rowstat_in))};
+    launch_gemm16<true>(gemm_plan(GEMM_LN, m, n, k, act, out_dtype == dtype, true, rowstat_in != nullptr), a, dtype, out_dtype, s);
     TRAMBA_LAUNCH_CHECK();
     return TRAMBA_OK;
 }
@@ -1643,6 +1779,15 @@
                                  const void *residual, void *y, int64_t m, int n, int k, int act, int dtype,
                                  int out_dtype, void *stream)
 {
+    return tramba_linear2_rowstat_cl(x1, x2, k1, w, bias, residual, y, m, n, k, act, dtype, out_dtype, nullptr, nullptr, stream);
+}
+
+extern "C" int tramba_linear2_rowstat_cl(const void *x1, const void *x2, int k1, const void *w, const float *bias,
+                                         const void *residual, void *y, int64_t m, int n, int k, int act, int dtype,
+                                         int out_dtype, float *rowstat_out, int *emitted, void *stream)
+{
+    if (emitted) *emitted = 0;
+    TRAMBA_CHECK(!rowstat_out || (emitted && ((size_t)rowstat_out & 7) == 0), "linear2_cl: rowstat_out needs `emitted` and 8-byte alignment");
     TRAMBA_CHECK(x1 && x2 && w && y, "linear2_cl: null tensor");
     TRAMBA_CHECK(m > 0 && n > 0 && k > 0 && k1 > 0 && k1 < k, "linear2_cl: empty shape");
     TRAMBA_CHECK(dtype == TRAMBA_BF16 || dtype == TRAMBA_F16, "linear2_cl: 16-bit dtypes only");
@@ -1656,7 +1801,12 @@
     GemmArgs a{x1, w, bias, residual, y, m, n, k, act};
     a.x2 = x2;
     a.k1 = k1;
-    launch_gemm16(gemm_plan(GEMM_TWO_SRC, m, n, k, act, out_dtype == dtype), a, dtype, out_dtype, s);
+    const GemmPlan p = gemm_plan(GEMM_TWO_SRC, m, n, k, act, out_dtype == dtype);
+    if (rowstat_out && plan_emits_rowstat(p, dtype, out_dtype, m, n)) {
+        a.li.stat = reinterpret_cast<float2 *>(rowstat_out);
+        *emitted = 1;
+    }
+    launch_gemm16(p, a, dtype, out_dtype, s);
     TRAMBA_LAUNCH_CHECK();
     return TRAMBA_OK;
 }
diff --git a/tramba_amd/hip.py b/tramba_amd/hip.py
--- a/tramba_amd/hip.py
+++ b/tramba_amd/hip.py
@@ -108,6 +108,11 @@
     "tramba_linear_dual_cl": (c_int, [c_vp] * 5 + [c_i64, c_int, c_int, c_int, c_int, c_vp]),
     "tramba_linear_ln_cl": (c_int, [c_vp] * 6 + [c_i64, c_int, c_int, c_f, c_int, c_int, c_int, c_vp]),
     "tramba_linear2_cl": (c_int, [c_vp, c_vp, c_int] + [c_vp] * 4 + [c_i64, c_int, c_int, c_int, c_int, c_int, c_vp]),
+    "tramba_linear_rowstat_cl": (c_int, [c_vp] * 5 + [c_i64, c_int, c_int, c_int, c_int, c_int, c_vp,
+                                                      ctypes.POINTER(c_int), c_vp]),
+    "tramba_linear2_rowstat_cl": (c_int, [c_vp, c_vp, c_int] + [c_vp] * 4 + [c_i64, c_int, c_int, c_int, c_int, c_int, c_vp,
+                                                                             ctypes.POINTER(c_int), c_vp]),
+    "tramba_linear_ln_rowstat_cl": (c_int, [c_vp] * 6 + [c_i64, c_int, c_int, c_f, c_int, c_int, c_int, c_vp, c_int, c_vp]),
     "tramba_wgrad_workspace": (ctypes.c_size_t, [c_i64, c_int, c_int, c_int, c_int]),
     "tramba_wgrad_cl": (c_int, [c_vp] * 4 + [ctypes.c_size_t, c_i64, c_int, c_int, c_int, c_int, c_i64, c_i64, c_int, c_i64,
                                              c_i64, c_int, c_int, c_int, c_vp]),
@@ -1338,16 +1343,45 @@
                              f"{residual.numel()}")
 
 
-def linear_cl(x, w, bias=None, residual=None, act=ACT_NONE, out_dtype=None):
+def _rowstat_extra(rowstat, dtype, out_dtype, m, n):
+    if not rowstat or out_dtype != dtype or dtype == torch.float32:
+        return 0
+    return (-(m * n)) % 8 + m * ((n + 63) // 64) * 4
+
+
+def _rowstat_split(buf, shape, m, n):
+    off = (m * n + 7) // 8 * 8
+    return buf[:m * n].view(shape), buf[off:].view(torch.float32).view(m, (n + 63) // 64, 2)
+
+
+def rowstat_for(x, k):
+    tag = getattr(x, "_tramba_rowstat", None)
+    if tag is None:
+        return None
+    slab, version = tag
+    if version != x._version or k % 64 or slab.shape != (x.numel() // k, k // 64, 2) or slab.device != x.device:
+        return None
+    return slab
+
+
+def linear_cl(x, w, bias=None, residual=None, act=ACT_NONE, out_dtype=None, rowstat=False):
     _dev(x, w, bias, residual)
     k = x.shape[-1]
     n = w.shape[0]
     m = x.numel() // k
     out_dtype = x.dtype if out_dtype is None else out_dtype
-    y = torch.empty(x.shape[:-1] + (n,), dtype=out_dtype, device=x.device)
+    extra = _rowstat_extra(rowstat, x.dtype, out_dtype, m, n)
+    y = torch.empty((m * n + extra,) if extra else x.shape[:-1] + (n,), dtype=out_dtype, device=x.device)
     if w.dtype != x.dtype or w.shape[1] != k:
         raise TrambaHipError("linear_cl: weight dtype/shape mismatch")
     _check_epilogue("linear_cl", bias, residual, x.dtype, m, n)
+    if extra:
+        (y, slab), emitted = _rowstat_split(y, x.shape[:-1] + (n,), m, n), c_int(0)
+        _check(lib().tramba_linear_rowstat_cl(_ptr(x), _ptr(w), _ptr(bias), _ptr(residual), _ptr(y), m, n, k, act, dt(x),
+                                              dt(y), _ptr(slab), ctypes.byref(emitted), _stream()), "linear_cl")
+        if emitted.value:
+            y._tramba_rowstat = (slab, y._version)
+        return y
     _check(lib().tramba_linear_cl(_ptr(x), _ptr(w), _ptr(bias), _ptr(residual), _ptr(y), m, n, k, act, dt(x),
                                   dt(y), _stream()), "linear_cl")
     return y
@@ -1468,7 +1502,7 @@
     return y_pre, y_act
 
 
-def linear_ln_cl(x, w_folded, colsum, bias, eps, residual=None, act=ACT_NONE, out_dtype=None):
+def linear_ln_cl(x, w_folded, colsum, bias, eps, residual=None, act=ACT_NONE, out_dtype=None, rowstat=None):
     _dev(x, w_folded, colsum, bias, residual)
     k = x.shape[-1]
     n = w_folded.shape[0]
@@ -1478,12 +1512,21 @@
     _check_epilogue("linear_ln_cl", bias, residual, x.dtype, m, n)
     out_dtype = x.dtype if out_dtype is None else out_dtype
     y = torch.empty(x.shape[:-1] + (n,), dtype=out_dtype, device=x.device)
+    if rowstat is not None:
+        if (rowstat.dtype != torch.float32 or rowstat.shape != (m, k // 64, 2) or k % 64 or not rowstat.is_contiguous()
+                or rowstat.device != x.device):
+            raise TrambaHipError(f"linear_ln_cl: rowstat must be a contiguous f32 ({m}, {k // 64}, 2) slab, got "
+                                 f"{rowstat.dtype} {tuple(rowstat.shape)}")
+        _check(lib().tramba_linear_ln_rowstat_cl(_ptr(x), _ptr(w_folded), _ptr(colsum), _ptr(bias), _ptr(residual), _ptr(y),
+                                                 m, n, k, float(eps), act, dt(x), dt(y), _ptr(rowstat), k // 64, _stream()),
+               "linear_ln_cl")
+        return y
     _check(lib().tramba_linear_ln_cl(_ptr(x), _ptr(w_folded), _ptr(colsum), _ptr(bias), _ptr(residual), _ptr(y), m, n, k,
                                      float(eps), act, dt(x), dt(y), _stream()), "linear_ln_cl")
     return y
 
 
-def linear2_cl(x1, x2, w, bias=None, residual=None, act=ACT_NONE, out_dtype=None):
+def linear2_cl(x1, x2, w, bias=None, residual=None, act=ACT_NONE, out_dtype=None, rowstat=False):
     _dev(x1, x2, w, bias, residual)
     k1, k2 = x1.shape[-1], x2.shape[-1]
     n = w.shape[0]
@@ -1492,7 +1535,16 @@
         raise TrambaHipError("linear2_cl: operand shapes / dtypes do not match")
     _check_epilogue("linear2_cl", bias, residual, x1.dtype, m, n)
     out_dtype = x1.dtype if out_dtype is None else out_dtype
-    y = torch.empty(x1.shape[:-1] + (n,), dtype=out_dtype, device=x1.device)
+    extra = _rowstat_extra(rowstat, x1.dtype, out_dtype, m, n)
+    y = torch.empty((m * n + extra,) if extra else x1.shape[:-1] + (n,), dtype=out_dtype, device=x1.device)
+    if extra:
+        (y, slab), emitted = _rowstat_split(y, x1.shape[:-1] + (n,), m, n), c_int(0)
+        _check(lib().tramba_linear2_rowstat_cl(_ptr(x1), _ptr(x2), k1, _ptr(w), _ptr(bias), _ptr(residual), _ptr(y), m, n,
+                                               k1 + k2, act, dt(x1), dt(y), _ptr(slab), ctypes.byref(emitted), _stream()),
+               "linear2_cl")
+        if emitted.value:
+            y._tramba_rowstat = (slab, y._version)
+        return y
     _check(lib().tramba_linear2_cl(_ptr(x1), _ptr(x2), k1, _ptr(w), _ptr(bias), _ptr(residual), _ptr(y), m, n, k1 + k2,
                                    act, dt(x1), dt(y), _stream()), "linear2_cl")
     return y
diff --git a/tramba_amd/modules.py b/tramba_amd/modules.py
--- a/tramba_amd/modules.py
+++ b/tramba_amd/modules.py
@@ -11,7 +11,7 @@
 
 
 
-FOLD_LAYERNORM = True
+FOLD_LAYERNORM, ROW_STATS = True, True
 
 
 def to_cl(x: torch.Tensor) -> torch.Tensor:
@@ -538,7 +538,7 @@
     def _forward_cl(self, x, act=hip.ACT_NONE, residual=None, out_dtype=None, gelu_in=False, gelu_ready=None):
         if _infer(x, self.weight):
             w = self.weight if self.weight.dtype == x.dtype else self.weight.to(x.dtype)
-            return hip.linear_cl(F.gelu(x) if gelu_in else x, w.detach(), _f32(self.bias), residual, act, out_dtype)
+            return hip.linear_cl(F.gelu(x) if gelu_in else x, w.detach(), _f32(self.bias), residual, act, out_dtype, _want_rs(residual, act))
         if gelu_in:
             y = _act_torch(_GeluLinearTrainCL.apply(x, self.weight, self.bias, gelu_ready), act)
         else:
@@ -559,7 +559,7 @@
                 and self.weight.shape[0] % 8 == 0):
             wf, cs, tb = _cache(self).get(("lnfold", x.dtype, id(norm)), (self.weight, self.bias, norm.weight, norm.bias),
                                           lambda: _fold_layernorm(self, norm, x.dtype))
-            return hip.linear_ln_cl(x, wf, cs, tb, norm.eps, residual, act, out_dtype)
+            return hip.linear_ln_cl(x, wf, cs, tb, norm.eps, residual, act, out_dtype, hip.rowstat_for(x, k) if ROW_STATS else None)
         return self._forward_cl(norm._forward_cl(x), act=act, residual=residual, out_dtype=out_dtype)
 
     def _forward_cat_cl(self, x1, x2, act=hip.ACT_NONE, residual=None, out_dtype=None):
@@ -1089,6 +1089,10 @@
     return _AddLayerNormCL.apply(v, None, None, norm.weight, norm.bias, norm.eps, act, True)
 
 
+def _want_rs(residual, act):
+    return ROW_STATS and FOLD_LAYERNORM and residual is not None and act == hip.ACT_NONE
+
+
 _dw_pack_store = {}
 _dw_plans = None
 
```

Result: faster. 884.4 img/s (median of 6 runs) (+1.0%).
